# asarigun/mma

Hardware: AMD Instinct MI355X
Metric: aggregated edges/sec (fwd+bwd) MultiMaskConv (higher is better)
Workload: dtype f32

## Files before the change

include/mma_amd.h:

```cpp
#ifndef MMA_AMD_H
#define MMA_AMD_H

#include <stdint.h>

#ifdef __cplusplus
extern "C" {
#endif

#define MMA_ABI_VERSION 36
#define MMA_MAX_K 8

enum {
  MMA_KIND_SUM = 0,
  MMA_KIND_MEAN = 1,
  MMA_KIND_MAX = 2,
  MMA_KIND_MIN = 3,
  MMA_KIND_SOFTMAX = 4,
  MMA_KIND_SOFTMIN = 5
};
enum { MMA_ACT_SIGMOID = 0, MMA_ACT_RAW = 1 };

enum { MMA_DROP_NONE = 0, MMA_DROP_HASH = 1, MMA_DROP_EXPLICIT = 2 };

int mma_abi_version(void);
const char* mma_last_error(void);
const char* mma_build_stamp(void);

int mma_nc_fused_fwd(
    const float* x, int64_t ldx,
    const float* P, int64_t ldp,
    const float* Q, int64_t ldq,
    const int32_t* rowptr,
    const int32_t* col,
    const int32_t* items, int64_t n_items,
    int64_t n_wave_items,
    const int32_t* hubs, int64_t n_hubs,
    float* partial, int64_t n_slots,
    float* m,
    float* m_sum, int64_t ldms,
    float* T, uint8_t* sel, int64_t ldt,
    float* crow, int64_t ldc,
    int64_t N, int64_t E, int32_t H, int32_t K,
    const uint8_t* kind_host, const uint8_t* act_host,
    int32_t drop_mode, uint32_t drop_thr, uint64_t seed,
    const uint64_t* seed_dev,
    int64_t drop_edge_base,
    const uint8_t* keep,
    int32_t* sync,
    void* stream);

int mma_nc_bwd_node(
    const float* g, int64_t g_kstride, int64_t ldgr,
    const uint8_t* sel, const float* T, int64_t ldt, const int32_t* rowptr,
    float* gs, int64_t ldgs,
    const float* crow, int64_t ldc,
    float* gP, int64_t ldgp, float* gxs, int64_t ldgx,
    float* row_max,
    int64_t N, int32_t H, int32_t K, const uint8_t* kind_host, void* stream);
int64_t mma_nc_crow_floats(int32_t H, int32_t K, const uint8_t* kind_host);

int mma_nc_fused_bwd(
    const float* x, int64_t ldx, const float* P, int64_t ldp, const float* Q, int64_t ldq,
    const float* gs, int64_t ldg,
    const float* g, int64_t ldgg,
    const float* crow, int64_t ldc,
    const uint8_t* kind_host,
    const float* gxs, int64_t ldgx,
    const float* T, int64_t ldt,
    float* gP, int64_t ldgp, int64_t n_targets,
    const int32_t* t_col, const int32_t* t_eid,
    const int32_t* items, int64_t n_items, int64_t n_wave_items, const int32_t* hubs, int64_t n_hubs,
    float* partial, int64_t n_slots,
    float* gQ, int64_t ldgq, float* gx, int64_t ldgxo,
    float* row_max,
    int64_t N, int64_t E, int32_t H, int32_t K,
    const uint8_t* act_host,
    int32_t drop_mode, uint32_t drop_thr, uint64_t seed, const uint64_t* seed_dev, int64_t drop_edge_base, const uint8_t* keep,
    int32_t* sync,
    void* stream);

int mma_csr_spmm(
    const int32_t* rowptr, const int32_t* col, const float* val,
    const float* B, int64_t ldb, int64_t rows_per_block, int32_t K,
    const float* bias, float* out, int64_t ldo,
    int64_t n_rows, int32_t C, void* stream);
int mma_csr_spmm_rm(
    const int32_t* rowptr, const int32_t* col, const float* val,
    const float* B, int64_t ldb, int64_t rows_per_block, int32_t K,
    const float* bias, float* out, int64_t ldo,
    int64_t n_rows, int32_t C, float* row_max, void* stream);

int mma_csr_spmm_items(
    const int32_t* col, const float* val, const float* B, int64_t ldb, const float* bias, float* out, int64_t ldo,
    const int32_t* items, int64_t n_items,
    int64_t n_wave_items,
    const int32_t* hubs, int64_t n_hubs, float* partial, int64_t n_slots,
    int32_t C, void* stream);

int mma_split_bf16x3(const float* in, int64_t n, void* out_3n_bf16, void* stream);
int mma_gemm_bf16x3(const float* A, int64_t lda, const void* Bt3, float* C, int64_t ldc,
                    int64_t M, int32_t N, int32_t K, int32_t accumulate , void* stream);
int mma_row_absmax(const float* A, int64_t lda, int64_t M, int32_t cols, float* out, void* stream);
int mma_split_f16x2(const float* w, int64_t stride_k, int64_t stride_n, int32_t K, int32_t N, void* bt2, float* col_unscale,
                    int32_t plain_lo, void* stream);
int mma_gemm_f16x2(const float* A, int64_t lda, const void* Bt2, const float* col_unscale, float* C, int64_t ldc,
                   float* a_row_max,
                   int64_t M, int32_t N, void* stream);
int mma_gemm_f16x2_k(const float* A, int64_t lda, const void* Bt2, const float* col_unscale, float* C, int64_t ldc,
                     float* a_row_max, int64_t M, int32_t N, int32_t K, void* stream);
int mma_gemm_f16x2_k256(const float* A, int64_t lda, const float* row_max, const void* Bt2, const float* col_unscale, float* C,
                        int64_t ldc, int64_t M, int32_t N, void* stream);
int64_t mma_pack_f16x2_k256_bytes(int64_t M);
int mma_pack_f16x2_k256(const float* A, int64_t lda, int64_t M, void* Ap, int32_t* sce, float* row_max, void* stream);
int mma_gemm_f16x2_k256p(const void* Ap, const int32_t* sce, const void* Bt2, const float* col_unscale, float* C, int64_t ldc,
                         int64_t M, int32_t N, void* stream);
int mma_gemm_f16x2_n128(const float* A, int64_t lda, const float* row_max, const void* Bt2, const float* col_unscale,
                        float* C, int64_t ldc, int64_t M, int32_t K, int32_t accumulate, void* stream);
int mma_gemm_f16x2_nlp(const float* A, int64_t lda, const float* row_max, const void* Bt2, const float* col_unscale,
                       float* C, int64_t ldc, int64_t M, int32_t N, int32_t K, int32_t accumulate, void* stream);
int64_t mma_gemm_bf16x3_tn_workspace_floats(int64_t M, int32_t KA, int32_t NC);
int mma_gemm_bf16x3_tn(const float* X, int64_t ldx, const float* G, int64_t ldg, float* C, float* ws, int64_t ws_floats,
                       int64_t M, int32_t KA, int32_t NC, void* stream);
int64_t mma_gemm_bf16x3_tn_batched_workspace_floats(int64_t M, int32_t KA, int32_t NC, int32_t B);
int mma_gemm_bf16x3_tn_batched(const float* X, int64_t ldx, int64_t xb, const float* G, int64_t ldg, int64_t gb, float* C, float* ws,
                               int64_t ws_floats, int64_t M, int32_t KA, int32_t NC, int32_t B, void* stream);
int64_t mma_gemm_f16x2_tn_workspace_floats(int64_t M, int32_t KA, int32_t NC);
int mma_gemm_f16x2_tn(const float* X, int64_t ldx, const float* G, int64_t ldg, const float* x_row_max, const float* g_row_max,
                      float* C, float* ws, int64_t ws_floats, int64_t M, int32_t KA, int32_t NC, void* stream);

int mma_pack_rows(const float* src, int64_t lds, const int32_t* idx, int64_t n_idx,
                  float* dst, int64_t ldd, int32_t width, void* stream);
int mma_unpack_add_rows(const float* src, int64_t lds, const int32_t* idx, int64_t n_idx,
                        float* dst, int64_t ldd, int32_t width, void* stream);
int mma_unpack_add_rows_csr(const float* src, int64_t lds, const int32_t* rows, const int32_t* segptr, const int32_t* pos,
                            int64_t n_rows, float* dst, int64_t ldd, int32_t width, void* stream);

int64_t mma_col_sum_workspace_floats(int64_t R, int32_t C);
int mma_col_sum(const float* g, int64_t ldg, int64_t R, int32_t C, float* out, float* ws, int64_t ws_floats,
                void* stream);

int64_t mma_tower_linear_bwd_blocks(int64_t N);
int mma_tower_linear_bwd(const float* gy, const float* a, const float* W, float* ga, float* part, int64_t n_blocks,
                         int64_t N, int32_t T, int32_t O, int32_t C, void* stream);

int64_t mma_tower_post_kfp(int32_t KF);
int mma_tower_post_weights(const float* Wo, int32_t T, int32_t O, int32_t S, int32_t KF, float* Wa, float* Wb, void* stream);
int mma_skinny_linear_weights(const float* W, int32_t O, int32_t K, float* Wa, float* Wb, void* stream);
int mma_tower_post_gw_reduce(const float* part, int64_t n_chunks, int32_t T, int32_t S, int32_t O, int32_t KF, float* gWo, void* stream);
int mma_tower_post_fits(int32_t KF, int32_t S);
int mma_tower_post_pre(const int32_t* rowptr, float* pre, int64_t N, int32_t S, const uint8_t* scaler_host, float avg_log, float avg_lin,
                       void* stream);
int mma_tower_post_fwd(const float* agg, int64_t lda, const float* pre, const float* Wa, float* y, int64_t ldy,
                       int64_t N, int32_t T, int32_t KF, int32_t S, int32_t O, const uint8_t* scaler_host, float avg_log, float avg_lin,
                       void* stream);
int mma_tower_post_bwd(const float* gy, int64_t ldg, const float* pre, const float* Wb, float* gagg, int64_t lda,
                       float* gys, int64_t ldgs,
                       int64_t N, int32_t T, int32_t KF, int32_t S, int32_t O,
                       const uint8_t* scaler_host, float avg_log, float avg_lin, void* stream);
int64_t mma_tower_post_gw_chunks(int64_t N, int32_t T);
int mma_tower_post_gw(const float* gy, int64_t ldg, const float* agg, int64_t lda,
                      const float* pre,
                      float* part, int64_t n_chunks,
// ... 84 lines not shown
```

mma_amd/_abi.py:

```python
ABI_VERSION = 36
FUNCTIONS = {
    "mma_abi_version": ("int", []),
    "mma_last_error": ("const char*", []),
    "mma_build_stamp": ("const char*", []),
    "mma_nc_fused_fwd": ("int", [("T", "T", "x"), ("i", "i64", "ldx"), ("T", "T", "P"), ("i", "i64", "ldp"), ("T", "T", "Q"), ("i", "i64", "ldq"), ("T", "T", "rowptr"), ("T", "T", "col"), ("T", "T", "items"), ("i", "i64", "n_items"), ("i", "i64", "n_wave_items"), ("T", "T", "hubs"), ("i", "i64", "n_hubs"), ("T", "T", "partial"), ("i", "i64", "n_slots"), ("T", "T", "m"), ("T", "T", "m_sum"), ("i", "i64", "ldms"), ("T", "T", "T"), ("T", "T", "sel"), ("i", "i64", "ldt"), ("T", "T", "crow"), ("i", "i64", "ldc"), ("i", "i64", "N"), ("i", "i64", "E"), ("i", "i32", "H"), ("i", "i32", "K"), ("H", "H", "kind_host"), ("H", "H", "act_host"), ("i", "i32", "drop_mode"), ("i", "u32", "drop_thr"), ("i", "u64", "seed"), ("T", "T", "seed_dev"), ("i", "i64", "drop_edge_base"), ("T", "T", "keep"), ("T", "T", "sync"), ("S", "S", "stream")]),
    "mma_nc_bwd_node": ("int", [("T", "T", "g"), ("i", "i64", "g_kstride"), ("i", "i64", "ldgr"), ("T", "T", "sel"), ("T", "T", "T"), ("i", "i64", "ldt"), ("T", "T", "rowptr"), ("T", "T", "gs"), ("i", "i64", "ldgs"), ("T", "T", "crow"), ("i", "i64", "ldc"), ("T", "T", "gP"), ("i", "i64", "ldgp"), ("T", "T", "gxs"), ("i", "i64", "ldgx"), ("T", "T", "row_max"), ("i", "i64", "N"), ("i", "i32", "H"), ("i", "i32", "K"), ("H", "H", "kind_host"), ("S", "S", "stream")]),
    "mma_nc_crow_floats": ("int64_t", [("i", "i32", "H"), ("i", "i32", "K"), ("H", "H", "kind_host")]),
    "mma_nc_fused_bwd": ("int", [("T", "T", "x"), ("i", "i64", "ldx"), ("T", "T", "P"), ("i", "i64", "ldp"), ("T", "T", "Q"), ("i", "i64", "ldq"), ("T", "T", "gs"), ("i", "i64", "ldg"), ("T", "T", "g"), ("i", "i64", "ldgg"), ("T", "T", "crow"), ("i", "i64", "ldc"), ("H", "H", "kind_host"), ("T", "T", "gxs"), ("i", "i64", "ldgx"), ("T", "T", "T"), ("i", "i64", "ldt"), ("T", "T", "gP"), ("i", "i64", "ldgp"), ("i", "i64", "n_targets"), ("T", "T", "t_col"), ("T", "T", "t_eid"), ("T", "T", "items"), ("i", "i64", "n_items"), ("i", "i64", "n_wave_items"), ("T", "T", "hubs"), ("i", "i64", "n_hubs"), ("T", "T", "partial"), ("i", "i64", "n_slots"), ("T", "T", "gQ"), ("i", "i64", "ldgq"), ("T", "T", "gx"), ("i", "i64", "ldgxo"), ("T", "T", "row_max"), ("i", "i64", "N"), ("i", "i64", "E"), ("i", "i32", "H"), ("i", "i32", "K"), ("H", "H", "act_host"), ("i", "i32", "drop_mode"), ("i", "u32", "drop_thr"), ("i", "u64", "seed"), ("T", "T", "seed_dev"), ("i", "i64", "drop_edge_base"), ("T", "T", "keep"), ("T", "T", "sync"), ("S", "S", "stream")]),
    "mma_csr_spmm": ("int", [("T", "T", "rowptr"), ("T", "T", "col"), ("T", "T", "val"), ("T", "T", "B"), ("i", "i64", "ldb"), ("i", "i64", "rows_per_block"), ("i", "i32", "K"), ("T", "T", "bias"), ("T", "T", "out"), ("i", "i64", "ldo"), ("i", "i64", "n_rows"), ("i", "i32", "C"), ("S", "S", "stream")]),
    "mma_csr_spmm_rm": ("int", [("T", "T", "rowptr"), ("T", "T", "col"), ("T", "T", "val"), ("T", "T", "B"), ("i", "i64", "ldb"), ("i", "i64", "rows_per_block"), ("i", "i32", "K"), ("T", "T", "bias"), ("T", "T", "out"), ("i", "i64", "ldo"), ("i", "i64", "n_rows"), ("i", "i32", "C"), ("T", "T", "row_max"), ("S", "S", "stream")]),
    "mma_csr_spmm_items": ("int", [("T", "T", "col"), ("T", "T", "val"), ("T", "T", "B"), ("i", "i64", "ldb"), ("T", "T", "bias"), ("T", "T", "out"), ("i", "i64", "ldo"), ("T", "T", "items"), ("i", "i64", "n_items"), ("i", "i64", "n_wave_items"), ("T", "T", "hubs"), ("i", "i64", "n_hubs"), ("T", "T", "partial"), ("i", "i64", "n_slots"), ("i", "i32", "C"), ("S", "S", "stream")]),
    "mma_split_bf16x3": ("int", [("T", "T", "in"), ("i", "i64", "n"), ("T", "T", "out_3n_bf16"), ("S", "S", "stream")]),
    "mma_gemm_bf16x3": ("int", [("T", "T", "A"), ("i", "i64", "lda"), ("T", "T", "Bt3"), ("T", "T", "C"), ("i", "i64", "ldc"), ("i", "i64", "M"), ("i", "i32", "N"), ("i", "i32", "K"), ("i", "i32", "accumulate"), ("S", "S", "stream")]),
    "mma_row_absmax": ("int", [("T", "T", "A"), ("i", "i64", "lda"), ("i", "i64", "M"), ("i", "i32", "cols"), ("T", "T", "out"), ("S", "S", "stream")]),
    "mma_split_f16x2": ("int", [("T", "T", "w"), ("i", "i64", "stride_k"), ("i", "i64", "stride_n"), ("i", "i32", "K"), ("i", "i32", "N"), ("T", "T", "bt2"), ("T", "T", "col_unscale"), ("i", "i32", "plain_lo"), ("S", "S", "stream")]),
    "mma_gemm_f16x2": ("int", [("T", "T", "A"), ("i", "i64", "lda"), ("T", "T", "Bt2"), ("T", "T", "col_unscale"), ("T", "T", "C"), ("i", "i64", "ldc"), ("T", "T", "a_row_max"), ("i", "i64", "M"), ("i", "i32", "N"), ("S", "S", "stream")]),
    "mma_gemm_f16x2_k": ("int", [("T", "T", "A"), ("i", "i64", "lda"), ("T", "T", "Bt2"), ("T", "T", "col_unscale"), ("T", "T", "C"), ("i", "i64", "ldc"), ("T", "T", "a_row_max"), ("i", "i64", "M"), ("i", "i32", "N"), ("i", "i32", "K"), ("S", "S", "stream")]),
    "mma_gemm_f16x2_k256": ("int", [("T", "T", "A"), ("i", "i64", "lda"), ("T", "T", "row_max"), ("T", "T", "Bt2"), ("T", "T", "col_unscale"), ("T", "T", "C"), ("i", "i64", "ldc"), ("i", "i64", "M"), ("i", "i32", "N"), ("S", "S", "stream")]),
    "mma_pack_f16x2_k256_bytes": ("int64_t", [("i", "i64", "M")]),
    "mma_pack_f16x2_k256": ("int", [("T", "T", "A"), ("i", "i64", "lda"), ("i", "i64", "M"), ("T", "T", "Ap"), ("T", "T", "sce"), ("T", "T", "row_max"), ("S", "S", "stream")]),
    "mma_gemm_f16x2_k256p": ("int", [("T", "T", "Ap"), ("T", "T", "sce"), ("T", "T", "Bt2"), ("T", "T", "col_unscale"), ("T", "T", "C"), ("i", "i64", "ldc"), ("i", "i64", "M"), ("i", "i32", "N"), ("S", "S", "stream")]),
    "mma_gemm_f16x2_n128": ("int", [("T", "T", "A"), ("i", "i64", "lda"), ("T", "T", "row_max"), ("T", "T", "Bt2"), ("T", "T", "col_unscale"), ("T", "T", "C"), ("i", "i64", "ldc"), ("i", "i64", "M"), ("i", "i32", "K"), ("i", "i32", "accumulate"), ("S", "S", "stream")]),
    "mma_gemm_f16x2_nlp": ("int", [("T", "T", "A"), ("i", "i64", "lda"), ("T", "T", "row_max"), ("T", "T", "Bt2"), ("T", "T", "col_unscale"), ("T", "T", "C"), ("i", "i64", "ldc"), ("i", "i64", "M"), ("i", "i32", "N"), ("i", "i32", "K"), ("i", "i32", "accumulate"), ("S", "S", "stream")]),
    "mma_gemm_bf16x3_tn_workspace_floats": ("int64_t", [("i", "i64", "M"), ("i", "i32", "KA"), ("i", "i32", "NC")]),
    "mma_gemm_bf16x3_tn": ("int", [("T", "T", "X"), ("i", "i64", "ldx"), ("T", "T", "G"), ("i", "i64", "ldg"), ("T", "T", "C"), ("T", "T", "ws"), ("i", "i64", "ws_floats"), ("i", "i64", "M"), ("i", "i32", "KA"), ("i", "i32", "NC"), ("S", "S", "stream")]),
    "mma_gemm_bf16x3_tn_batched_workspace_floats": ("int64_t", [("i", "i64", "M"), ("i", "i32", "KA"), ("i", "i32", "NC"), ("i", "i32", "B")]),
    "mma_gemm_bf16x3_tn_batched": ("int", [("T", "T", "X"), ("i", "i64", "ldx"), ("i", "i64", "xb"), ("T", "T", "G"), ("i", "i64", "ldg"), ("i", "i64", "gb"), ("T", "T", "C"), ("T", "T", "ws"), ("i", "i64", "ws_floats"), ("i", "i64", "M"), ("i", "i32", "KA"), ("i", "i32", "NC"), ("i", "i32", "B"), ("S", "S", "stream")]),
    "mma_gemm_f16x2_tn_workspace_floats": ("int64_t", [("i", "i64", "M"), ("i", "i32", "KA"), ("i", "i32", "NC")]),
    "mma_gemm_f16x2_tn": ("int", [("T", "T", "X"), ("i", "i64", "ldx"), ("T", "T", "G"), ("i", "i64", "ldg"), ("T", "T", "x_row_max"), ("T", "T", "g_row_max"), ("T", "T", "C"), ("T", "T", "ws"), ("i", "i64", "ws_floats"), ("i", "i64", "M"), ("i", "i32", "KA"), ("i", "i32", "NC"), ("S", "S", "stream")]),
    "mma_pack_rows": ("int", [("T", "T", "src"), ("i", "i64", "lds"), ("T", "T", "idx"), ("i", "i64", "n_idx"), ("T", "T", "dst"), ("i", "i64", "ldd"), ("i", "i32", "width"), ("S", "S", "stream")]),
    "mma_unpack_add_rows": ("int", [("T", "T", "src"), ("i", "i64", "lds"), ("T", "T", "idx"), ("i", "i64", "n_idx"), ("T", "T", "dst"), ("i", "i64", "ldd"), ("i", "i32", "width"), ("S", "S", "stream")]),
    "mma_unpack_add_rows_csr": ("int", [("T", "T", "src"), ("i", "i64", "lds"), ("T", "T", "rows"), ("T", "T", "segptr"), ("T", "T", "pos"), ("i", "i64", "n_rows"), ("T", "T", "dst"), ("i", "i64", "ldd"), ("i", "i32", "width"), ("S", "S", "stream")]),
    "mma_col_sum_workspace_floats": ("int64_t", [("i", "i64", "R"), ("i", "i32", "C")]),
    "mma_col_sum": ("int", [("T", "T", "g"), ("i", "i64", "ldg"), ("i", "i64", "R"), ("i", "i32", "C"), ("T", "T", "out"), ("T", "T", "ws"), ("i", "i64", "ws_floats"), ("S", "S", "stream")]),
    "mma_tower_linear_bwd_blocks": ("int64_t", [("i", "i64", "N")]),
    "mma_tower_linear_bwd": ("int", [("T", "T", "gy"), ("T", "T", "a"), ("T", "T", "W"), ("T", "T", "ga"), ("T", "T", "part"), ("i", "i64", "n_blocks"), ("i", "i64", "N"), ("i", "i32", "T"), ("i", "i32", "O"), ("i", "i32", "C"), ("S", "S", "stream")]),
    "mma_tower_post_kfp": ("int64_t", [("i", "i32", "KF")]),
    "mma_tower_post_weights": ("int", [("T", "T", "Wo"), ("i", "i32", "T"), ("i", "i32", "O"), ("i", "i32", "S"), ("i", "i32", "KF"), ("T", "T", "Wa"), ("T", "T", "Wb"), ("S", "S", "stream")]),
    "mma_skinny_linear_weights": ("int", [("T", "T", "W"), ("i", "i32", "O"), ("i", "i32", "K"), ("T", "T", "Wa"), ("T", "T", "Wb"), ("S", "S", "stream")]),
    "mma_tower_post_gw_reduce": ("int", [("T", "T", "part"), ("i", "i64", "n_chunks"), ("i", "i32", "T"), ("i", "i32", "S"), ("i", "i32", "O"), ("i", "i32", "KF"), ("T", "T", "gWo"), ("S", "S", "stream")]),
    "mma_tower_post_fits": ("int", [("i", "i32", "KF"), ("i", "i32", "S")]),
    "mma_tower_post_pre": ("int", [("T", "T", "rowptr"), ("T", "T", "pre"), ("i", "i64", "N"), ("i", "i32", "S"), ("H", "H", "scaler_host"), ("f", "f32", "avg_log"), ("f", "f32", "avg_lin"), ("S", "S", "stream")]),
    "mma_tower_post_fwd": ("int", [("T", "T", "agg"), ("i", "i64", "lda"), ("T", "T", "pre"), ("T", "T", "Wa"), ("T", "T", "y"), ("i", "i64", "ldy"), ("i", "i64", "N"), ("i", "i32", "T"), ("i", "i32", "KF"), ("i", "i32", "S"), ("i", "i32", "O"), ("H", "H", "scaler_host"), ("f", "f32", "avg_log"), ("f", "f32", "avg_lin"), ("S", "S", "stream")]),
    "mma_tower_post_bwd": ("int", [("T", "T", "gy"), ("i", "i64", "ldg"), ("T", "T", "pre"), ("T", "T", "Wb"), ("T", "T", "gagg"), ("i", "i64", "lda"), ("T", "T", "gys"), ("i", "i64", "ldgs"), ("i", "i64", "N"), ("i", "i32", "T"), ("i", "i32", "KF"), ("i", "i32", "S"), ("i", "i32", "O"), ("H", "H", "scaler_host"), ("f", "f32", "avg_log"), ("f", "f32", "avg_lin"), ("S", "S", "stream")]),
    "mma_tower_post_gw_chunks": ("int64_t", [("i", "i64", "N"), ("i", "i32", "T")]),
    "mma_tower_post_gw": ("int", [("T", "T", "gy"), ("i", "i64", "ldg"), ("T", "T", "agg"), ("i", "i64", "lda"), ("T", "T", "pre"), ("T", "T", "part"), ("i", "i64", "n_chunks"), ("i", "i64", "N"), ("i", "i32", "T"), ("i", "i32", "KF"), ("i", "i32", "S"), ("i", "i32", "O"), ("H", "H", "scaler_host"), ("f", "f32", "avg_log"), ("f", "f32", "avg_lin"), ("S", "S", "stream")]),
    "mma_skinny_linear_fwd": ("int", [("T", "T", "x"), ("i", "i64", "ldx"), ("T", "T", "Wa"), ("T", "T", "bias"), ("T", "T", "addend"), ("i", "i64", "ldadd"), ("T", "T", "y"), ("i", "i64", "ldy"), ("i", "i64", "N"), ("i", "i32", "K"), ("i", "i32", "O"), ("S", "S", "stream")]),
    "mma_skinny_linear_bwd_dx": ("int", [("T", "T", "gy"), ("i", "i64", "ldg"), ("T", "T", "Wb"), ("T", "T", "gx"), ("i", "i64", "ldx"), ("i", "i64", "N"), ("i", "i32", "K"), ("i", "i32", "O"), ("S", "S", "stream")]),
    "mma_skinny_linear_gw_part": ("int64_t", [("i", "i64", "N"), ("i", "i32", "K"), ("i", "i32", "O")]),
    "mma_skinny_linear_gw": ("int", [("T", "T", "gy"), ("i", "i64", "ldg"), ("T", "T", "x"), ("i", "i64", "ldx"), ("T", "T", "part"), ("i", "i64", "n_part"), ("T", "T", "gw"), ("T", "T", "gb"), ("i", "i64", "N"), ("i", "i32", "K"), ("i", "i32", "O"), ("S", "S", "stream")]),
    "mma_logsoftmax_nll_fwd": ("int", [("T", "T", "x"), ("i", "i64", "ldx"), ("T", "T", "idx"), ("T", "T", "labels"), ("i", "i64", "n_idx"), ("T", "T", "logp"), ("i", "i64", "ldo"), ("T", "T", "loss"), ("i", "i64", "N"), ("i", "i32", "C"), ("S", "S", "stream")]),
    "mma_logsoftmax_nll_bwd": ("int", [("T", "T", "logp"), ("i", "i64", "ldo"), ("T", "T", "idx"), ("T", "T", "labels"), ("i", "i64", "n_idx"), ("T", "T", "gloss"), ("T", "T", "gx"), ("i", "i64", "ldg"), ("i", "i64", "N"), ("i", "i32", "C"), ("S", "S", "stream")]),
    "mma_masked_bn_relu_fwd": ("int", [("T", "T", "x"), ("i", "i64", "ldx"), ("T", "T", "n_valid"), ("T", "T", "gamma"), ("T", "T", "beta"), ("T", "T", "y"), ("i", "i64", "ldy"), ("T", "T", "mean_out"), ("T", "T", "rstd_out"), ("T", "T", "running_mean"), ("T", "T", "running_var"), ("T", "T", "n_tracked"), ("f", "f32", "momentum"), ("f", "f32", "eps"), ("i", "i64", "N"), ("i", "i32", "C"), ("i", "i32", "relu"), ("S", "S", "stream")]),
    "mma_masked_bn_relu_bwd": ("int", [("T", "T", "gy"), ("i", "i64", "ldg"), ("T", "T", "y"), ("i", "i64", "ldy"), ("T", "T", "x"), ("i", "i64", "ldx"), ("T", "T", "mean"), ("T", "T", "rstd"), ("T", "T", "gamma"), ("T", "T", "n_valid"), ("T", "T", "gx"), ("i", "i64", "ldgx"), ("T", "T", "ggamma"), ("T", "T", "gbeta"), ("i", "i64", "N"), ("i", "i32", "C"), ("i", "i32", "relu"), ("S", "S", "stream")]),
    "mma_pad_rows": ("int", [("T", "T", "x"), ("i", "i64", "ldx"), ("i", "i64", "M"), ("i", "i32", "fin"), ("T", "T", "col"), ("T", "T", "row_index"), ("T", "T", "out"), ("i", "i64", "ldo"), ("i", "i32", "width"), ("i", "i64", "M_out"), ("S", "S", "stream")]),
    "mma_pack_blocks": ("int", [("T", "T", "table"), ("i", "i64", "n_blocks"), ("T", "T", "a_base"), ("T", "T", "b0"), ("T", "T", "b1"), ("T", "T", "b2"), ("T", "T", "b3"), ("T", "T", "b4"), ("T", "T", "b5"), ("T", "T", "b6"), ("T", "T", "b7"), ("i", "i32", "unpack"), ("S", "S", "stream")]),
    "mma_edge_fold_fwd": ("int", [("T", "T", "We"), ("i", "i64", "ldw"), ("T", "T", "Wenc"), ("T", "T", "benc"), ("T", "T", "wz"), ("T", "T", "bz"), ("i", "i64", "TF"), ("i", "i32", "F"), ("i", "i32", "ED"), ("S", "S", "stream")]),
    "mma_edge_fold_bwd": ("int", [("T", "T", "We"), ("i", "i64", "ldw"), ("T", "T", "Wenc"), ("T", "T", "benc"), ("T", "T", "gwz"), ("T", "T", "gbz"), ("T", "T", "gWe"), ("T", "T", "gWenc"), ("T", "T", "gbenc"), ("i", "i64", "TF"), ("i", "i32", "F"), ("i", "i32", "ED"), ("S", "S", "stream")]),
    "mma_seed_advance": ("int", [("T", "T", "seeds"), ("i", "i32", "n"), ("S", "S", "stream")]),
    "mma_l1_loss_fwd": ("int", [("T", "T", "pred"), ("T", "T", "target"), ("i", "i64", "n"), ("T", "T", "loss"), ("S", "S", "stream")]),
    "mma_l1_loss_bwd": ("int", [("T", "T", "pred"), ("T", "T", "target"), ("i", "i64", "n"), ("T", "T", "gloss"), ("T", "T", "gpred"), ("S", "S", "stream")]),
    "mma_adam_table_bytes": ("int64_t", [("i", "i64", "n_tensors"), ("i", "i64", "total_chunks")]),
    "mma_adam_chunks": ("int64_t", [("i", "i64", "n_elements")]),
    "mma_adam_step": ("int", [("T", "T", "table"), ("i", "i64", "n_tensors"), ("i", "i64", "total_chunks"), ("T", "T", "step"), ("f", "f64", "lr"), ("f", "f64", "beta1"), ("f", "f64", "beta2"), ("f", "f32", "eps"), ("f", "f32", "weight_decay"), ("S", "S", "stream")]),
    "mma_adam_max_grads_by_value": ("int64_t", []),
    "mma_adam_step_grads": ("int", [("T", "T", "table"), ("i", "i64", "n_tensors"), ("i", "i64", "total_chunks"), ("T", "T", "step"), ("f", "f64", "lr"), ("f", "f64", "beta1"), ("f", "f64", "beta2"), ("f", "f32", "eps"), ("f", "f32", "weight_decay"), ("H", "H", "grad_ptrs_host"), ("S", "S", "stream")]),
    "mma_csr_workspace_bytes": ("int64_t", [("i", "i64", "E"), ("i", "i64", "N")]),
    "mma_gr_long_nodes_len": ("int64_t", [("i", "i64", "E")]),
    "mma_build_csr": ("int", [("T", "T", "key"), ("T", "T", "other"), ("i", "i64", "E"), ("i", "i64", "N"), ("T", "T", "rowptr"), ("T", "T", "perm"), ("T", "T", "other_sorted"), ("T", "T", "long_nodes"), ("T", "T", "workspace"), ("i", "i64", "workspace_bytes"), ("S", "S", "stream")]),
    "mma_gr_arg_side_rows": ("int64_t", [("i", "i64", "E")]),
    "mma_gr_fused_fwd": ("int", [("T", "T", "rowptr"), ("T", "T", "src"), ("T", "T", "perm"), ("T", "T", "U"), ("T", "T", "V"), ("i", "i64", "lduv"), ("T", "T", "Z"), ("i", "i64", "ldz"), ("i", "i32", "by_pos"), ("T", "T", "z_index"), ("T", "T", "inputs"), ("i", "i64", "ldi"), ("T", "T", "out"), ("T", "T", "amin8"), ("T", "T", "amax8"), ("T", "T", "amin_side"), ("T", "T", "amax_side"), ("T", "T", "mean"), ("T", "T", "var"), ("i", "i64", "ldsave"), ("T", "T", "long_nodes"), ("i", "i64", "N"), ("i", "i64", "E"), ("i", "i32", "T"), ("i", "i32", "F"), ("H", "H", "aggr_host"), ("i", "i32", "K"), ("H", "H", "scaler_host"), ("i", "i32", "S"), ("f", "f32", "avg_log"), ("f", "f32", "avg_lin"), ("i", "i32", "drop_mode"), ("i", "u32", "drop_thr"), ("i", "u64", "seed"), ("T", "T", "seed_dev"), ("S", "S", "stream")]),
    "mma_gr_fused_bwd": ("int", [("T", "T", "rowptr"), ("T", "T", "src"), ("T", "T", "perm"), ("T", "T", "U"), ("T", "T", "V"), ("i", "i64", "lduv"), ("T", "T", "Z"), ("i", "i64", "ldz"), ("i", "i32", "by_pos"), ("T", "T", "z_index"), ("T", "T", "inputs"), ("i", "i64", "ldi"), ("T", "T", "gout"), ("T", "T", "amin8"), ("T", "T", "amax8"), ("T", "T", "amin_side"), ("T", "T", "amax_side"), ("T", "T", "mean"), ("T", "T", "var"), ("i", "i64", "ldsave"), ("T", "T", "long_nodes"), ("T", "T", "gmsg"), ("i", "i64", "ldg"), ("T", "T", "gU"), ("i", "i64", "ldgu"), ("T", "T", "gmsg_row_max"), ("T", "T", "gu_row_max"), ("i", "i64", "N"), ("i", "i64", "E"), ("i", "i32", "T"), ("i", "i32", "F"), ("H", "H", "aggr_host"), ("i", "i32", "K"), ("H", "H", "scaler_host"), ("i", "i32", "S"), ("f", "f32", "avg_log"), ("f", "f32", "avg_lin"), ("i", "i32", "drop_mode"), ("i", "u32", "drop_thr"), ("i", "u64", "seed"), ("T", "T", "seed_dev"), ("S", "S", "stream")]),
}
```

mma_amd/csrc/nc_fused.hip:

```cpp
#include <cstdlib>
#include "common.h"

#ifndef NC_FWD_UNROLL
#define NC_FWD_UNROLL(K) ((K) >= 3 ? 1 : 2)
#endif
#ifndef NC_BWD_UNROLL
#define NC_BWD_UNROLL(K) ((K) >= 3 ? 1 : 2)
#endif
#ifndef MMA_MIN_WAVES
#define MMA_MIN_WAVES 2
#endif
namespace mma {

struct NcFwdParams {
  const float* x; int64_t ldx;
  const float* P; int64_t ldp; const float* Q; int64_t ldq;
  const int32_t* rowptr; const int32_t* col;
  const int4* items; int64_t n_items;
  float* partial; int64_t pstride;
  float* m; int64_t m_kstride;
  float* msum; int64_t ldms;
  float* T; uint8_t* sel; int64_t ldt;
  float* crow; int64_t ldc; uint32_t sel_slots;
  int H, HQ, K_total, k_base, lpr_log;
// ... 306 lines not shown
    default: fs = tf == 255u ? __builtin_nanf("") : 1.f; fx = 0.f; break;
  }
}

template <int VEC>
__global__ __launch_bounds__(kBlock) void nc_bwd_node_kernel(const NcBwdNodeParams p) {
  const int per_row = (p.H + VEC - 1) / VEC;
  const int64_t total = p.N * per_row;
  for (int64_t idx = (int64_t)blockIdx.x * blockDim.x + threadIdx.x; idx < total; idx += (int64_t)gridDim.x * blockDim.x) {
    const int64_t node = idx / per_row;
    const int c = (int)(idx % per_row) * VEC;
    const float deg = (float)max(p.rowptr[node + 1] - p.rowptr[node], 1);
    const float inv_deg = 1.f / deg;
    Vec<VEC> gk[MMA_MAX_K], tk[MMA_MAX_K];
    uint32_t ck[MMA_MAX_K];
    const bool shared_g = p.g_kstride == 0;
#pragma unroll
    for (int k = 0; k < MMA_MAX_K; ++k) {
      if (k < p.K) {
        const size_t o = (size_t)node * p.ldt + (size_t)k * p.H + c;
        if (k == 0 || !shared_g) gk[k] = ldv_nt<VEC>(p.g + (size_t)k * p.g_kstride + (size_t)node * p.ldgr + c);
        tk[k] = ldv_nt<VEC>(p.T + o);
        if (p.crow) {
          ck[k] = sel_slot_of(p.sel_slots, k) != 0xFu
              ? ldb<VEC>(reinterpret_cast<const uint8_t*>(p.crow + (size_t)node * p.ldc + 4 + (size_t)sel_slot_of(p.sel_slots, k) * p.HQ) + c) : 0u;
        } else {
          ck[k] = ldb_nt<VEC>(p.sel + o);
        }
      }
    }
    Vec<VEC> gx = vzero<VEC>();
    float mxp = 0.f;
#pragma unroll
    for (int k = 0; k < MMA_MAX_K; ++k) {
      if (k < p.K) {
        const int kind = kind_of(p.kinds, k);
        const Vec<VEC> g = shared_g ? gk[0] : gk[k];
        const Vec<VEC> t = tk[k];
        const uint32_t codes = ck[k];
        Vec<VEC> gsv, gpv;
#pragma unroll
        for (int i = 0; i < VEC; ++i) {
          uint32_t tf = (codes >> (8 * i)) & 0xFFu;
          if (!p.crow) tf = tf == 1u ? 2u : (tf == 2u ? 1u : (tf == 3u ? 255u : 0u));
          float fs, fx;
          combine_grad_tf(kind, tf, inv_deg, fs, fx);
          gsv.v[i] = g.v[i] * fs;
          gpv.v[i] = gsv.v[i] * t.v[i];
          gx.v[i] = fmaf(g.v[i], fx, gx.v[i]);
          mxp = fmaxf(mxp, fabsf(gpv.v[i]));
        }
        if (p.gs) stv<VEC>(p.gs + (size_t)node * p.ldgs + (size_t)k * p.H + c, gsv);
        stv_nt<VEC>(p.gP + (size_t)node * p.ldgp + (size_t)k * p.H + c, gpv);
      }
    }
    stv_nt<VEC>(p.gxs + (size_t)node * p.ldgx + c, gx);
    if (p.rowmax) {
      if ((per_row & (per_row - 1)) == 0 && per_row <= kWave) {
        for (int off = per_row >> 1; off > 0; off >>= 1) mxp = fmaxf(mxp, __shfl_xor(mxp, off, kWave));
        if ((idx & (per_row - 1)) == 0 && mxp > 0.f) atomicMax(p.rowmax + node, __float_as_uint(mxp));
      } else if (mxp > 0.f) {
        atomicMax(p.rowmax + node, __float_as_uint(mxp));
      }
    }
  }
}

struct NcBwdParams {
  const float* x; int64_t ldx;
  const float* P; int64_t ldp; const float* Q; int64_t ldq;
  const float* gs; int64_t ldg; const float* gxs; int64_t ldgx;
  const float* g; int64_t ldgg; const float* crow; int64_t ldc; uint32_t sel_slots; uint32_t kinds;
  const float* T; int64_t ldt; float* gP; int64_t ldgp; int64_t n_targets;
  const int32_t* t_col; const int32_t* t_eid;
  const int4* items; int64_t n_items;
  float* partial; int64_t pstride;
  float* gQ; int64_t ldgq; float* gx; int64_t ldgxo;
  int H, HQ, K_total, k_base, lpr_log;
  uint32_t acts;
  DropParams drop;
  int first_pass;
  uint32_t* rowmax;
  const int4* hubs; int64_t n_hubs; unsigned* sync; unsigned n_slots;
};

template <int VEC>
__device__ __forceinline__ Vec<VEC> nc_bwd_epilogue(const NcBwdParams& p, int node, int c, int k0, int nk, float& mx) {
  const Vec<VEC> g = ldv_nt<VEC>(p.g + row_off(node, p.ldgg) + c);
  const float* crow = p.crow + row_off(node, p.ldc);
  const float inv_deg = crow[0];
  Vec<VEC> gxd = vzero<VEC>();
  Vec<VEC> tk[MMA_MAX_K]; uint32_t ck[MMA_MAX_K];
#pragma unroll
  for (int k = 0; k < MMA_MAX_K; ++k) {
    if (k < nk) {
      tk[k] = ldv_nt<VEC>(p.T + row_off(node, p.ldt) + (size_t)(k0 + k) * p.H + c);
      const uint32_t sslot = sel_slot_of(p.sel_slots, k0 + k);
      ck[k] = sslot != 0xFu ? ldb<VEC>(reinterpret_cast<const uint8_t*>(crow + 4 + (size_t)sslot * p.HQ) + c) : 0u;
    }
  }
#pragma unroll
  for (int k = 0; k < MMA_MAX_K; ++k) {
    if (k < nk) {
      const int kind = kind_of(p.kinds, k0 + k);
      Vec<VEC> gpv;
#pragma unroll
      for (int i = 0; i < VEC; ++i) {
        float fs, fx;
        combine_grad_tf(kind, (ck[k] >> (8 * i)) & 0xFFu, inv_deg, fs, fx);
        gpv.v[i] = (g.v[i] * fs) * tk[k].v[i];
        gxd.v[i] = fmaf(g.v[i], fx, gxd.v[i]);
        mx = fmaxf(mx, fabsf(gpv.v[i]));
      }
      stv_nt<VEC>(p.gP + row_off(node, p.ldgp) + (size_t)(k0 + k) * p.H + c, gpv);
    }
  }
  return gxd;
}

template <int VEC>
__device__ __forceinline__ void nc_bwd_finalize_body(const NcBwdParams& p, const int4* hubs, int64_t n_hubs, const int64_t first, const int64_t step);

template <int K, int VEC, int DM, bool SHARED, bool MULTI, bool EPI, bool ONE = false>
__device__ __forceinline__ void nc_bwd_body(const NcBwdParams& p, const int bx, const int nbx) {
  constexpr bool DROP = DM != MMA_DROP_NONE;
  const DropParams dp = (DM == MMA_DROP_HASH || DM == MMA_DROP_HASH16) ? drop_resolve(p.drop) : p.drop;
  uint32_t mult[K], mult2[K];
#pragma unroll
  for (int k = 0; k < K; ++k) { mult[k] = drop_mask_mult(p.k_base + k); mult2[k] = drop_mask_mult2(p.k_base + k); }
  constexpr int U = NC_BWD_UNROLL(K);
  const int lane = threadIdx.x & (kWave - 1);
  const int lpr = 1 << p.lpr_log;
  const int G = MULTI ? lpr : kWave;
  const int epg = G >> p.lpr_log;
  const int gpw = kWave / G;
  const int grp = MULTI ? lane / G : 0;
  const int gl = lane & (G - 1);
  const int gbase = grp * G;
  const int sub = gl >> p.lpr_log;
  const int c = ((int)blockIdx.y * lpr + (lane & (lpr - 1))) * VEC;
  const bool fvalid = c < p.H;
  const int cc = fvalid ? c : 0;
  const int waves_per_block = kBlock / kWave;
  const int64_t stride = (int64_t)nbx * waves_per_block;
  const int64_t n_witems = (p.n_items + gpw - 1) / gpw;

  for (int64_t it0 = (int64_t)bx * waves_per_block + (threadIdx.x >> 6); it0 < n_witems; it0 += stride) {
    int node, ebeg, eend, slot;
    bool ivalid = true;
    if (MULTI) {
      const int64_t idx = it0 * gpw + grp;
      ivalid = idx < p.n_items;
      const int4 item = p.items[ivalid ? idx : 0];
      node = item.x; ebeg = item.y; eend = ivalid ? item.z : item.y; slot = item.w;
    } else {
      const int4 item = p.items[__builtin_amdgcn_readfirstlane((int)it0)];
      node = __builtin_amdgcn_readfirstlane(item.x);
      ebeg = __builtin_amdgcn_readfirstlane(item.y);
      eend = __builtin_amdgcn_readfirstlane(item.z);
      slot = __builtin_amdgcn_readfirstlane(item.w);
    }
    const int len = eend - ebeg;
    int maxlen = len;
    if (MULTI) {
      for (int off = G; off < kWave; off <<= 1) maxlen = max(maxlen, __shfl_xor(maxlen, off, kWave));
      maxlen = __builtin_amdgcn_readfirstlane(maxlen);
    }

    const Vec<VEC> xj = ldv_nt<VEC>(p.x + row_off(node, p.ldx) + cc);
    Vec<VEC> qk[K], aq[K];
    Vec<VEC> ax = vzero<VEC>();
#pragma unroll
    for (int k = 0; k < K; ++k) {
      qk[k] = ldv_nt<VEC>(p.Q + row_off(node, p.ldq) + (size_t)(p.k_base + k) * p.H + cc);
      aq[k] = vzero<VEC>();
    }

    for (int base = 0; base < maxlen; base += G) {
      const int cnt = min(G, max(len - base, 0));
      const int ucnt = min(G, maxlen - base);
      const int myi = (gl < cnt) ? p.t_col[ebeg + base + gl] : ((gl == 0 && len > 0) ? p.t_col[ebeg] : 0);
      const int mye = (DROP && gl < cnt) ? p.t_eid[ebeg + base + gl] : 0;
      for (int t0 = 0; t0 < ucnt; t0 += U * epg) {
        int tt[U]; bool ev[U]; uint32_t eid[U]; Vec<VEC> gv[U][SHARED ? 1 : K]; Vec<VEC> pv[U][K];
        uint32_t codes[U][K]; float idg[U];
#pragma unroll
        for (int u = 0; u < U; ++u) {
          tt[u] = t0 + u * epg + sub;
          ev[u] = tt[u] < cnt;
          const int tl = min(tt[u], max(cnt - 1, 0));
          const int ii = __shfl(myi, gbase + (tl & (G - 1)), kWave);
          eid[u] = DROP ? (uint32_t)__shfl(mye, gbase + (tl & (G - 1)), kWave) : 0u;
          if (SHARED) {
            gv[u][0] = ldv<VEC>(p.g + row_off(ii, p.ldgg) + cc);
            const float* crow = p.crow + row_off(ii, p.ldc);
            idg[u] = crow[0];
#pragma unroll
            for (int k = 0; k < K; ++k) {
              const uint32_t sslot = sel_slot_of(p.sel_slots, p.k_base + k);
              codes[u][k] = (sslot != 0xFu) ? ldb<VEC>(reinterpret_cast<const uint8_t*>(crow + 4 + (size_t)sslot * p.HQ) + cc)
                                             : 0x02020202u;
            }
          }
          const float* prow = p.P + row_off(ii, p.ldp) + cc;
          const float* grow = SHARED ? nullptr : p.gs + row_off(ii, p.ldg) + cc;
#pragma unroll
          for (int k = 0; k < K; ++k) {
            const size_t o = (size_t)(p.k_base + k) * p.H;
            if (!SHARED) gv[u][k] = ldv<VEC>(grow + o);
            pv[u][k] = ldv<VEC>(prow + o);
          }
        }
#pragma unroll
        for (int u = 0; u < U; ++u) {
          const bool live = ev[u];
#pragma unroll
          for (int kk = 0; kk < (SHARED ? 1 : K); ++kk)
#pragma unroll
            for (int i = 0; i < VEC; ++i) gv[u][kk].v[i] = live ? gv[u][kk].v[i] : 0.f;
          const uint32_t hw = (DM == MMA_DROP_HASH || DM == MMA_DROP_HASH16) ? drop_base_word(dp, eid[u], cc >> 2) : 0u;
#pragma unroll
          for (int k = 0; k < K; ++k) {
            const bool raw = (p.acts >> (p.k_base + k)) & 1u;
            const int kind = SHARED ? kind_of(p.kinds, p.k_base + k) : 0;
            const float kscale = 0.5f * (kind == MMA_KIND_MEAN ? idg[u] : 1.f);
            float f[VEC];
            if (DM == MMA_DROP_HASH) {
              drop_unpack<VEC>(dp, drop_mask_word(hw, k == 0 ? p.k_base : 1, mult[k]), cc, f);
            } else if (DM == MMA_DROP_HASH16) {
              drop_unpack16<VEC>(dp, drop_mask_word(hw, k == 0 ? p.k_base : 1, mult[k]), drop_low_word(hw, mult2[k]), cc, f);
            } else if (DM == MMA_DROP_EXPLICIT) {
              drop_explicit<VEC>(dp, eid[u], p.k_base + k, cc, p.H, f);
            } else {
#pragma unroll
              for (int i = 0; i < VEC; ++i) f[i] = 1.f;
            }
#pragma unroll
            for (int i = 0; i < VEC; ++i) {
              const float z = pv[u][k].v[i] + qk[k].v[i];
              float a, da;
              if (raw) { a = z; da = 1.f; }
              else { a = sigmoid_fast(z); da = a - a * a; }
              float gsv;
              if (SHARED) {
                const uint32_t tf = (codes[u][k] >> (8 * i)) & 0xFFu;
                float cf = (float)tf;
                if (kind >= MMA_KIND_SOFTMAX && tf == 255u) cf = __builtin_nanf("");
                gsv = gv[u][0].v[i] * (cf * kscale);
              } else {
                gsv = gv[u][k].v[i];
              }
              const float w = f[i] * gsv;
              aq[k].v[i] = fmaf(da, w, aq[k].v[i]);
              ax.v[i] = fmaf(a, w, ax.v[i]);
            }
          }
        }
      }
    }

    const bool writer = sub == 0 && fvalid && ivalid;
    const bool tgt = EPI && writer && slot < 0 && (int64_t)node < p.n_targets;
    Vec<VEC> gxd = vzero<VEC>();
    float mxp = 0.f;
    if (EPI) { if (tgt) gxd = nc_bwd_epilogue<VEC>(p, node, c, p.k_base, K, mxp); }

    for (int off = G / 2; off >= lpr; off >>= 1) {
#pragma unroll
      for (int i = 0; i < VEC; ++i) {
        ax.v[i] += __shfl_xor(ax.v[i], off, kWave);
#pragma unroll
        for (int k = 0; k < K; ++k) aq[k].v[i] += __shfl_xor(aq[k].v[i], off, kWave);
      }
    }
    if (len == 0) {
      ax = vzero<VEC>();
#pragma unroll
      for (int k = 0; k < K; ++k) aq[k] = vzero<VEC>();
    }

    if (p.rowmax) {
      float mxq = mxp;
      if (writer && slot < 0) {
#pragma unroll
        for (int k = 0; k < K; ++k)
#pragma unroll
          for (int i = 0; i < VEC; ++i) mxq = fmaxf(mxq, fabsf(xj.v[i] * aq[k].v[i]));
      }
      for (int off = lpr >> 1; off > 0; off >>= 1) mxq = fmaxf(mxq, __shfl_xor(mxq, off, kWave));
      if (sub == 0 && (lane & (lpr - 1)) == 0 && ivalid && slot < 0 && mxq > 0.f) atomicMax(p.rowmax + node, __float_as_uint(mxq));
    }
    if (writer) {
      if (slot < 0) {
#pragma unroll
        for (int k = 0; k < K; ++k) {
          Vec<VEC> o;
#pragma unroll
          for (int i = 0; i < VEC; ++i) o.v[i] = xj.v[i] * aq[k].v[i];
          stv_nt<VEC>(p.gQ + row_off(node, p.ldgq) + (size_t)(p.k_base + k) * p.H + c, o);
        }
        Vec<VEC> g0;
        if (EPI) {
          g0 = gxd;
          if (!p.first_pass) {
            const Vec<VEC> prev = ldv<VEC>(p.gx + row_off(node, p.ldgxo) + c);
#pragma unroll
            for (int i = 0; i < VEC; ++i) g0.v[i] += prev.v[i];
          }
        } else {
          g0 = p.first_pass ? ldv_nt<VEC>(p.gxs + row_off(node, p.ldgx) + c) : ldv<VEC>(p.gx + row_off(node, p.ldgxo) + c);
        }
        Vec<VEC> o;
#pragma unroll
        for (int i = 0; i < VEC; ++i) o.v[i] = g0.v[i] + ax.v[i];
        stv_nt<VEC>(p.gx + row_off(node, p.ldgxo) + c, o);
      } else {
        float* ps = p.partial + (size_t)slot * p.pstride;
#pragma unroll
        for (int k = 0; k < K; ++k) stv<VEC>(ps + (size_t)(p.k_base + k) * p.H + c, aq[k]);
        float* px = ps + (size_t)p.K_total * p.H + c;
        if (p.first_pass) stv<VEC>(px, ax);
        else {
          const Vec<VEC> prev = ldv<VEC>(px);
          Vec<VEC> o;
#pragma unroll
          for (int i = 0; i < VEC; ++i) o.v[i] = prev.v[i] + ax.v[i];
          stv<VEC>(px, o);
        }
      }
    }
    if (ONE) {
      const bool wrote = ivalid && slot >= 0;
      if (__builtin_amdgcn_ballot_w64(wrote) != 0) {
        __builtin_amdgcn_fence(__ATOMIC_RELEASE, "agent");
        unsigned ticket = 0u;
        if (wrote && gl == 0) ticket = atomicAdd(p.sync, 1u) + 1u;
        if (__builtin_amdgcn_ballot_w64(ticket == p.n_slots) != 0) {
          __builtin_amdgcn_fence(__ATOMIC_ACQUIRE, "agent");
          nc_bwd_finalize_body<VEC>(p, p.hubs, p.n_hubs, lane, kWave);
          if (lane == 0) *p.sync = 0u;
        }
      }
    }
  }
}

template <int K, int VEC, int DM, bool SHARED, bool MULTI, bool EPI>
__global__ __launch_bounds__(kBlock, (K <= 4 ? MMA_MIN_WAVES : 1)) void nc_bwd_kernel(const NcBwdParams p) {
  nc_bwd_body<K, VEC, DM, SHARED, MULTI, EPI>(p, (int)blockIdx.x, (int)gridDim.x);
}

template <int VEC>
__device__ __forceinline__ void nc_bwd_finalize_body(const NcBwdParams& p, const int4* hubs, int64_t n_hubs, const int64_t first, const int64_t step) {
  const int per_row = (p.H + VEC - 1) / VEC;
  const bool epi = p.T != nullptr;
  const int64_t total = n_hubs * (p.K_total + 1) * per_row;
  for (int64_t idx = first; idx < total; idx += step) {
    const int c = (int)(idx % per_row) * VEC;
    const int k = (int)((idx / per_row) % (p.K_total + 1));
    const int4 hub = hubs[idx / ((int64_t)per_row * (p.K_total + 1))];
    Vec<VEC> s = vzero<VEC>();
    constexpr int kAhead = 8;
    for (int sl0 = hub.y; sl0 < hub.z; sl0 += kAhead) {
      Vec<VEC> a[kAhead];
#pragma unroll
      for (int u = 0; u < kAhead; ++u) a[u] = ldv<VEC>(p.partial + (size_t)min(sl0 + u, hub.z - 1) * p.pstride + (size_t)k * p.H + c);
#pragma unroll
      for (int u = 0; u < kAhead; ++u) {
        if (sl0 + u < hub.z) {
#pragma unroll
          for (int i = 0; i < VEC; ++i) s.v[i] += a[u].v[i];
        }
      }
    }
    const int node = hub.x;
    const bool tgt = epi && (int64_t)node < p.n_targets;
    Vec<VEC> o;
    if (k < p.K_total) {
      const Vec<VEC> xj = ldv<VEC>(p.x + (size_t)node * p.ldx + c);
      float mxq = 0.f;
      if (tgt) nc_bwd_epilogue<VEC>(p, node, c, k, 1, mxq);
#pragma unroll
      for (int i = 0; i < VEC; ++i) o.v[i] = xj.v[i] * s.v[i];
      stv_nt<VEC>(p.gQ + (size_t)node * p.ldgq + (size_t)k * p.H + c, o);
      if (p.rowmax) {
#pragma unroll
        for (int i = 0; i < VEC; ++i) mxq = fmaxf(mxq, fabsf(o.v[i]));
        if (mxq > 0.f) atomicMax(p.rowmax + node, __float_as_uint(mxq));
      }
    } else {
      Vec<VEC> g0 = vzero<VEC>();
      if (tgt) {
        const Vec<VEC> g = ldv<VEC>(p.g + row_off(node, p.ldgg) + c);
        const float* crow = p.crow + row_off(node, p.ldc);
        const float inv_deg = crow[0];
        for (int kk = 0; kk < p.K_total; ++kk) {
          const uint32_t sslot = sel_slot_of(p.sel_slots, kk);
          const uint32_t ck = sslot != 0xFu ? ldb<VEC>(reinterpret_cast<const uint8_t*>(crow + 4 + (size_t)sslot * p.HQ) + c) : 0u;
#pragma unroll
          for (int i = 0; i < VEC; ++i) {
            float fs, fx;
            combine_grad_tf(kind_of(p.kinds, kk), (ck >> (8 * i)) & 0xFFu, inv_deg, fs, fx);
            g0.v[i] = fmaf(g.v[i], fx, g0.v[i]);
          }
        }
      } else if (!epi) {
        g0 = ldv<VEC>(p.gxs + (size_t)node * p.ldgx + c);
      }
#pragma unroll
      for (int i = 0; i < VEC; ++i) o.v[i] = g0.v[i] + s.v[i];
      stv<VEC>(p.gx + (size_t)node * p.ldgxo + c, o);
    }
  }
}
template <int VEC>
__global__ __launch_bounds__(kBlock) void nc_bwd_finalize_kernel(const NcBwdParams p, const int4* hubs, int64_t n_hubs) {
  nc_bwd_finalize_body<VEC>(p, hubs, n_hubs, (int64_t)blockIdx.x * blockDim.x + threadIdx.x, (int64_t)gridDim.x * blockDim.x);
}

template <int K, int VEC, int DM, bool EPI>
__global__ __launch_bounds__(kBlock, (K <= 4 ? MMA_MIN_WAVES : 1)) void nc_bwd_small_kernel(const NcBwdParams p, const NcSmallPlan sp) {
  if ((int)blockIdx.x < sp.blocks_a) {
    NcBwdParams q = p;
    q.n_items = sp.n_wave_items;
    nc_bwd_body<K, VEC, DM, true, false, EPI, true>(q, (int)blockIdx.x, sp.blocks_a);
  } else {
    NcBwdParams q = p;
    q.items = p.items + sp.n_wave_items; q.n_items = p.n_items - sp.n_wave_items;
    nc_bwd_body<K, VEC, DM, true, true, EPI, true>(q, (int)blockIdx.x - sp.blocks_a, (int)gridDim.x - sp.blocks_a);
  }
}

static bool aligned16(const void* p) { return (reinterpret_cast<uintptr_t>(p) & 15u) == 0; }

static int pack_codes(const uint8_t* kind_host, const uint8_t* act_host, int K, uint32_t* kinds, uint32_t* acts) {
  *kinds = 0; *acts = 0;
  for (int k = 0; k < K; ++k) {
    if (kind_host) {
      if (kind_host[k] > MMA_KIND_SOFTMIN) return fail(1, "kind[%d]=%d is not an MMA_KIND_* code", k, (int)kind_host[k]);
      *kinds |= (uint32_t)kind_host[k] << (4 * k);
    }
    if (act_host) {
      if (act_host[k] > MMA_ACT_RAW) return fail(1, "act[%d]=%d is not an MMA_ACT_* code", k, (int)act_host[k]);
      *acts |= (uint32_t)act_host[k] << k;
    }
  }
  return 0;
}

static int64_t fill_sel_slots(const uint8_t* kind_host, int K, int H, uint32_t* slots) {
  int n = 0;
  *slots = 0xFFFFFFFFu;
  for (int k = 0; k < K; ++k)
    if (kind_host[k] >= MMA_KIND_MAX) { *slots = (*slots & ~(0xFu << (4 * k))) | ((uint32_t)n << (4 * k)); ++n; }
  return ((4 + (int64_t)n * (((int64_t)H + 3) / 4)) + 3) & ~(int64_t)3;
}

static int make_drop(int32_t mode, uint32_t thr, uint64_t seed, const uint64_t* seed_dev, int64_t edge_base, const uint8_t* keep,
                     int64_t E, DropParams* d) {
  d->seed_dev = seed_dev;
  MMA_REQUIRE(edge_base >= 0 && edge_base + E < (1LL << 32), "drop_edge_base %lld out of range", (long long)edge_base);
  d->edge_base = (uint32_t)edge_base;
  MMA_REQUIRE(mode >= MMA_DROP_NONE && mode <= MMA_DROP_EXPLICIT, "drop_mode %d unknown", mode);
  MMA_REQUIRE(mode == MMA_DROP_NONE || thr < 65536, "drop_thr %u out of range (0..65535: P(drop) = thr / 65536)", thr);
  MMA_REQUIRE(mode != MMA_DROP_EXPLICIT || keep != nullptr, "drop_mode EXPLICIT needs a keep mask");
  drop_set_threshold(d, mode, thr);
  d->seed_lo = (uint32_t)seed; d->seed_hi = (uint32_t)(seed >> 32); d->keep = keep; d->E = E;
  return 0;
}

struct Geometry { int vec, lpr_log, chunks; };
static Geometry geometry(int H, bool vec4_ok) {
  Geometry g;
  g.vec = vec4_ok ? 4 : 1;
  const int per_row = (H + g.vec - 1) / g.vec;
  g.lpr_log = min(ilog2_ceil(per_row), 6);
  g.chunks = (per_row + (1 << g.lpr_log) - 1) >> g.lpr_log;
  return g;
}

static dim3 item_grid(int64_t n_items, int chunks, int items_per_wave = 1) {
  const int64_t per_block = (int64_t)(kBlock / kWave) * items_per_wave;
  int64_t blocks = (n_items + per_block - 1) / per_block;
  if (blocks > kMaxGrid) blocks = kMaxGrid;
  if (blocks < 1) blocks = 1;
  return dim3((unsigned)blocks, (unsigned)chunks, 1);
}

template <int K, int VEC, bool MULTI>
static void launch_fwd(const NcFwdParams& p, dim3 grid, bool save, int dm, hipStream_t st) {
#define MMA_FWD(SAVE, DM) hipLaunchKernelGGL((nc_fwd_kernel<K, VEC, SAVE, DM, MULTI>), grid, dim3(kBlock), 0, st, p)
  if (save) {
    if (dm == MMA_DROP_HASH) MMA_FWD(true, MMA_DROP_HASH); else if (dm == MMA_DROP_HASH16) MMA_FWD(true, MMA_DROP_HASH16); else if (dm == MMA_DROP_EXPLICIT) MMA_FWD(true, MMA_DROP_EXPLICIT); else MMA_FWD(true, MMA_DROP_NONE);
  } else {
    if (dm == MMA_DROP_HASH) MMA_FWD(false, MMA_DROP_HASH); else if (dm == MMA_DROP_HASH16) MMA_FWD(false, MMA_DROP_HASH16); else if (dm == MMA_DROP_EXPLICIT) MMA_FWD(false, MMA_DROP_EXPLICIT); else MMA_FWD(false, MMA_DROP_NONE);
  }
#undef MMA_FWD
}
template <int VEC, bool MULTI>
static void launch_fwd_k(int Ks, const NcFwdParams& p, dim3 grid, bool save, int dm, hipStream_t st) {
  switch (Ks) {
    case 1: launch_fwd<1, VEC, MULTI>(p, grid, save, dm, st); break;
    case 2: launch_fwd<2, VEC, MULTI>(p, grid, save, dm, st); break;
    case 3: launch_fwd<3, VEC, MULTI>(p, grid, save, dm, st); break;
    case 4: launch_fwd<4, VEC, MULTI>(p, grid, save, dm, st); break;
    default: launch_fwd<8, VEC, MULTI>(p, grid, save, dm, st); break;
  }
}
template <int K, int VEC, bool MULTI>
static void launch_bwd(const NcBwdParams& p, dim3 grid, int dm, hipStream_t st) {
  const bool shared = p.gs == nullptr;
  const bool epi = p.T != nullptr;
#define MMA_BWD(DM, SHARED, EPI) hipLaunchKernelGGL((nc_bwd_kernel<K, VEC, DM, SHARED, MULTI, EPI>), grid, dim3(kBlock), 0, st, p)
#define MMA_BWD_DM(SHARED, EPI) \
  do { if (dm == MMA_DROP_HASH) MMA_BWD(MMA_DROP_HASH, SHARED, EPI); else if (dm == MMA_DROP_HASH16) MMA_BWD(MMA_DROP_HASH16, SHARED, EPI); else if (dm == MMA_DROP_EXPLICIT) MMA_BWD(MMA_DROP_EXPLICIT, SHARED, EPI); \
       else MMA_BWD(MMA_DROP_NONE, SHARED, EPI); } while (0)
  if (shared) { if (epi) MMA_BWD_DM(true, true); else MMA_BWD_DM(true, false); }
  else MMA_BWD_DM(false, false);
#undef MMA_BWD_DM
#undef MMA_BWD
}
template <int VEC, bool MULTI>
static void launch_bwd_k(int Ks, const NcBwdParams& p, dim3 grid, int dm, hipStream_t st) {
  switch (Ks) {
    case 1: launch_bwd<1, VEC, MULTI>(p, grid, dm, st); break;
    case 2: launch_bwd<2, VEC, MULTI>(p, grid, dm, st); break;
    case 3: launch_bwd<3, VEC, MULTI>(p, grid, dm, st); break;
    case 4: launch_bwd<4, VEC, MULTI>(p, grid, dm, st); break;
    default: launch_bwd<8, VEC, MULTI>(p, grid, dm, st); break;
  }
}

template <int K>
static void launch_fwd_small(const NcFwdParams& p, const NcSmallPlan& sp, dim3 grid, bool save, int dm, hipStream_t st) {
#define MMA_FWD_S(SAVE, DM) hipLaunchKernelGGL((nc_fwd_small_kernel<K, 4, SAVE, DM>), grid, dim3(kBlock), 0, st, p, sp)
  if (save) { if (dm == MMA_DROP_HASH) MMA_FWD_S(true, MMA_DROP_HASH); else if (dm == MMA_DROP_HASH16) MMA_FWD_S(true, MMA_DROP_HASH16); else MMA_FWD_S(true, MMA_DROP_NONE); }
  else { if (dm == MMA_DROP_HASH) MMA_FWD_S(false, MMA_DROP_HASH); else if (dm == MMA_DROP_HASH16) MMA_FWD_S(false, MMA_DROP_HASH16); else MMA_FWD_S(false, MMA_DROP_NONE); }
#undef MMA_FWD_S
}
template <int K>
static void launch_bwd_small(const NcBwdParams& p, const NcSmallPlan& sp, dim3 grid, int dm, hipStream_t st) {
  const bool epi = p.T != nullptr;
#define MMA_BWD_S(DM, EPI) hipLaunchKernelGGL((nc_bwd_small_kernel<K, 4, DM, EPI>), grid, dim3(kBlock), 0, st, p, sp)
  if (epi) { if (dm == MMA_DROP_HASH) MMA_BWD_S(MMA_DROP_HASH, true); else if (dm == MMA_DROP_HASH16) MMA_BWD_S(MMA_DROP_HASH16, true); else MMA_BWD_S(MMA_DROP_NONE, true); }
  else { if (dm == MMA_DROP_HASH) MMA_BWD_S(MMA_DROP_HASH, false); else if (dm == MMA_DROP_HASH16) MMA_BWD_S(MMA_DROP_HASH16, false); else MMA_BWD_S(MMA_DROP_NONE, false); }
#undef MMA_BWD_S
}
static bool small_plan(int32_t* sync, int K, const Geometry& g, int dm, int64_t n_items, int64_t n_wave_items, int64_t n_hubs, int64_t n_slots,
                       int64_t finalize_elems, NcSmallPlan* sp, dim3* grid) {
  const bool one_slice = K <= 4 || K == 8;
  if (!sync || !one_slice || g.vec != 4 || g.chunks != 1 || dm == MMA_DROP_EXPLICIT || finalize_elems > 4096 || n_slots >= (1LL << 31)) return false;
  const int64_t n_group = n_items - n_wave_items;
  if (n_hubs == 0 && (n_wave_items == 0 || n_group == 0)) return false;
  const int ipw = kWave >> g.lpr_log;
  const unsigned ba = n_wave_items > 0 ? item_grid(n_wave_items, 1, 1).x : 0u;
  const unsigned bb = n_group > 0 ? item_grid(n_group, 1, ipw).x : 0u;
  *sp = NcSmallPlan{n_wave_items, (int)ba};
  *grid = dim3(ba + bb, 1, 1);
  return true;
}

static int next_slice(int remaining) { return remaining >= 8 ? 8 : (remaining >= 4 ? 4 : remaining); }

static int64_t elementwise_grid(int64_t total) {
  int64_t b = (total + kBlock - 1) / kBlock;
  return b < 1 ? 1 : (b > kMaxGrid * 4 ? kMaxGrid * 4 : b);
}

}

using namespace mma;

extern "C" int mma_nc_fused_fwd(
    const float* x, int64_t ldx, const float* P, int64_t ldp, const float* Q, int64_t ldq,
    const int32_t* rowptr, const int32_t* col,
    const int32_t* items, int64_t n_items, int64_t n_wave_items, const int32_t* hubs, int64_t n_hubs,
    float* partial, int64_t n_slots, float* m, float* m_sum, int64_t ldms, float* T, uint8_t* sel, int64_t ldt,
    float* crow, int64_t ldc,
    int64_t N, int64_t E, int32_t H, int32_t K, const uint8_t* kind_host, const uint8_t* act_host,
    int32_t drop_mode, uint32_t drop_thr, uint64_t seed, const uint64_t* seed_dev, int64_t drop_edge_base, const uint8_t* keep,
    int32_t* sync, void* stream) {
  MMA_REQUIRE(N >= 0 && E >= 0 && N < (1LL << 31) && E < (1LL << 31), "N=%lld E=%lld out of int32 range", (long long)N, (long long)E);
  MMA_REQUIRE(H >= 1 && K >= 1 && K <= MMA_MAX_K, "H=%d K=%d unsupported (1<=K<=%d)", H, K, MMA_MAX_K);
  MMA_REQUIRE(ldx >= H && ldp >= (int64_t)K * H && ldq >= (int64_t)K * H, "row pitch too small: ldx=%lld ldp=%lld ldq=%lld",
              (long long)ldx, (long long)ldp, (long long)ldq);
  MMA_REQUIRE(T != nullptr || (sel == nullptr && crow == nullptr), "sel / crow are saved next to T: give T too");
  MMA_REQUIRE(T == nullptr || sel != nullptr || crow != nullptr, "T needs the selection state beside it: sel (N,K*H), crow (N,ldc), or both");
  MMA_REQUIRE(T == nullptr || ldt >= (int64_t)K * H, "ldt=%lld too small", (long long)ldt);
  MMA_REQUIRE(ldx < (1LL << 31) && ldp < (1LL << 31) && ldq < (1LL << 31) && ldt < (1LL << 31) && ldc < (1LL << 31), "row pitch out of range");
  MMA_REQUIRE(n_items >= 0 && n_hubs >= 0 && n_slots >= 0 && n_items < (1LL << 31) && n_wave_items >= 0, "negative or oversize item counts");
  MMA_REQUIRE(n_slots == 0 || (partial != nullptr && hubs != nullptr && n_hubs > 0), "hub slots without partial/hubs buffers");
  if (N == 0 || n_items == 0) return 0;
  MMA_REQUIRE(x && P && Q && rowptr && items && kind_host && act_host, "NULL argument");
  MMA_REQUIRE(m != nullptr || m_sum != nullptr, "give m (K,N,H), m_sum (N,H), or both");
  MMA_REQUIRE(m_sum == nullptr || ldms >= H, "ldms=%lld too small", (long long)ldms);
  MMA_REQUIRE(E == 0 || col != nullptr, "NULL col");
  MMA_REQUIRE(aligned16(items) && (hubs == nullptr || aligned16(hubs)), "items/hubs must be 16-byte aligned int32 quadruples");
  uint32_t kinds, acts;
  if (int rc = pack_codes(kind_host, act_host, K, &kinds, &acts)) return rc;
  NcFwdParams p{};
  if (int rc = make_drop(drop_mode, drop_thr, seed, seed_dev, drop_edge_base, keep, E, &p.drop)) return rc;
  const int dm = (drop_mode == MMA_DROP_HASH && drop_thr == 0) ? MMA_DROP_NONE : p.drop.mode;
  const bool save = T != nullptr;
  if (crow) {
    const int64_t crow_len = fill_sel_slots(kind_host, K, H, &p.sel_slots);
    MMA_REQUIRE(ldc >= crow_len && ldc % 4 == 0 && aligned16(crow), "crow needs a 16-byte aligned pitch >= %lld floats (mma_nc_crow_floats)",
                (long long)crow_len);
  }
  const bool v4 = (H % 4 == 0) && (ldx % 4 == 0) && (ldp % 4 == 0) && (ldq % 4 == 0) && (!save || ldt % 4 == 0) && aligned16(x) &&
                  aligned16(P) && aligned16(Q) && (!m || aligned16(m)) && (!m_sum || (aligned16(m_sum) && ldms % 4 == 0)) &&
                  (!save || (aligned16(T) && (!sel || aligned16(sel)))) && (partial == nullptr || aligned16(partial));
  const Geometry g = geometry(H, v4);
  p.x = x; p.ldx = ldx; p.P = P; p.ldp = ldp; p.Q = Q; p.ldq = ldq; p.rowptr = rowptr; p.col = col;
  static const bool ablate_p = getenv("MMA_NC_ABLATE_P") && atoi(getenv("MMA_NC_ABLATE_P")) != 0;
  if (ablate_p) p.ldp = 0;
  p.items = reinterpret_cast<const int4*>(items); p.n_items = n_items;
  p.partial = partial; p.pstride = 2LL * K * H;
  p.m = m; p.m_kstride = N * (int64_t)H; p.msum = m_sum; p.ldms = ldms; p.T = T; p.sel = sel; p.ldt = ldt;
  p.crow = crow; p.ldc = ldc;
  p.H = H; p.HQ = (H + 3) / 4; p.K_total = K; p.lpr_log = g.lpr_log; p.kinds = kinds; p.acts = acts;
  hipStream_t st = static_cast<hipStream_t>(stream);
  const int ipw = kWave >> g.lpr_log;
  if (ipw == 1 || n_wave_items > n_items) n_wave_items = n_items;
  const int4* all_items = p.items;
  {
    NcSmallPlan sp; dim3 sgrid;
    if (small_plan(sync, K, g, dm, n_items, n_wave_items, n_hubs, n_slots, n_hubs * ((H + 3) / 4), &sp, &sgrid)) {
      p.k_base = 0;
      p.hubs = reinterpret_cast<const int4*>(hubs); p.n_hubs = n_hubs; p.sync = reinterpret_cast<unsigned*>(sync); p.n_slots = (unsigned)n_slots;
      switch (K) {
        case 1: launch_fwd_small<1>(p, sp, sgrid, save, dm, st); break;
        case 2: launch_fwd_small<2>(p, sp, sgrid, save, dm, st); break;
        case 3: launch_fwd_small<3>(p, sp, sgrid, save, dm, st); break;
        case 4: launch_fwd_small<4>(p, sp, sgrid, save, dm, st); break;
        default: launch_fwd_small<8>(p, sp, sgrid, save, dm, st); break;
      }
      return check_launch("nc_fwd_small_kernel");
    }
  }
  for (int part = 0; part < 2; ++part) {
    const int64_t cnt = part == 0 ? n_wave_items : n_items - n_wave_items;
    if (cnt <= 0) continue;
    p.items = all_items + (part == 0 ? 0 : n_wave_items);
    p.n_items = cnt;
    const dim3 grid = item_grid(cnt, g.chunks, part == 0 ? 1 : ipw);
    for (int k0 = 0; k0 < K;) {
      const int ks = next_slice(K - k0);
      p.k_base = k0;
      if (g.vec == 4) { if (part == 0) launch_fwd_k<4, false>(ks, p, grid, save, dm, st); else launch_fwd_k<4, true>(ks, p, grid, save, dm, st); }
      else { if (part == 0) launch_fwd_k<1, false>(ks, p, grid, save, dm, st); else launch_fwd_k<1, true>(ks, p, grid, save, dm, st); }
      k0 += ks;
    }
  }
  if (int rc = check_launch("nc_fwd_kernel")) return rc;
  if (n_hubs > 0) {
    const int per_row = (H + g.vec - 1) / g.vec;
    const dim3 fg((unsigned)elementwise_grid(n_hubs * per_row));
    const int4* hb = reinterpret_cast<const int4*>(hubs);
    if (g.vec == 4) {
      if (save) hipLaunchKernelGGL((nc_fwd_finalize_kernel<4, true>), fg, dim3(kBlock), 0, st, p, hb, n_hubs);
      else hipLaunchKernelGGL((nc_fwd_finalize_kernel<4, false>), fg, dim3(kBlock), 0, st, p, hb, n_hubs);
    } else {
      if (save) hipLaunchKernelGGL((nc_fwd_finalize_kernel<1, true>), fg, dim3(kBlock), 0, st, p, hb, n_hubs);
      else hipLaunchKernelGGL((nc_fwd_finalize_kernel<1, false>), fg, dim3(kBlock), 0, st, p, hb, n_hubs);
    }
    if (int rc = check_launch("nc_fwd_finalize_kernel")) return rc;
  }
  return 0;
}

extern "C" int64_t mma_nc_crow_floats(int32_t H, int32_t K, const uint8_t* kind_host) {
  if (H < 1 || K < 1 || K > MMA_MAX_K || !kind_host) return -1;
  for (int k = 0; k < K; ++k) if (kind_host[k] > MMA_KIND_SOFTMIN) return -1;
  uint32_t slots;
  return fill_sel_slots(kind_host, K, H, &slots);
}

extern "C" int mma_nc_bwd_node(
    const float* g, int64_t g_kstride, int64_t ldgr, const uint8_t* sel, const float* T, int64_t ldt, const int32_t* rowptr,
    float* gs, int64_t ldgs, const float* crow, int64_t ldc, float* gP, int64_t ldgp, float* gxs, int64_t ldgx, float* row_max,
    int64_t N, int32_t H, int32_t K, const uint8_t* kind_host, void* stream) {
  MMA_REQUIRE(N >= 0 && N < (1LL << 31) && H >= 1 && K >= 1 && K <= MMA_MAX_K, "N=%lld H=%d K=%d unsupported", (long long)N, H, K);
  MMA_REQUIRE(ldt >= (int64_t)K * H && (!gs || ldgs >= (int64_t)K * H) && ldgp >= (int64_t)K * H && ldgx >= H && ldgr >= H &&
              g_kstride >= 0, "row pitch too small");
  if (N == 0) return 0;
  MMA_REQUIRE(g && (sel || crow) && T && rowptr && gP && gxs && kind_host, "NULL argument (the selection state is sel or crow)");
  uint32_t kinds, acts;
  if (int rc = pack_codes(kind_host, nullptr, K, &kinds, &acts)) return rc;
  NcBwdNodeParams p{g, g_kstride, ldgr, sel, T, ldt, rowptr, gs, ldgs, gP, ldgp, gxs, ldgx, N, H, K, kinds};
  p.rowmax = reinterpret_cast<uint32_t*>(row_max);
  p.crow = crow; p.ldc = ldc; p.HQ = (H + 3) / 4;
  const int64_t crow_len = fill_sel_slots(kind_host, K, H, &p.sel_slots);
  MMA_REQUIRE(!crow || (ldc >= crow_len && ldc % 4 == 0 && aligned16(crow)),
              "crow needs a 16-byte aligned pitch >= %lld floats (mma_nc_crow_floats)", (long long)crow_len);
  const bool v4 = (H % 4 == 0) && (ldt % 4 == 0) && (!gs || ldgs % 4 == 0) && (ldgp % 4 == 0) && (ldgx % 4 == 0) &&
                  (ldgr % 4 == 0) && (g_kstride % 4 == 0) && aligned16(g) && (crow || aligned16(sel)) &&
                  aligned16(T) && (!gs || aligned16(gs)) && aligned16(gP) && aligned16(gxs);
  hipStream_t st = static_cast<hipStream_t>(stream);
  const int per_row = v4 ? H / 4 : H;
  int64_t nblk = (N * per_row + kBlock - 1) / kBlock;
  if (nblk > (1LL << 30)) nblk = 1LL << 30;
  const dim3 grid((unsigned)nblk);
  if (v4) hipLaunchKernelGGL((nc_bwd_node_kernel<4>), grid, dim3(kBlock), 0, st, p);
  else hipLaunchKernelGGL((nc_bwd_node_kernel<1>), grid, dim3(kBlock), 0, st, p);
  return check_launch("nc_bwd_node_kernel");
}

extern "C" int mma_nc_fused_bwd(
    const float* x, int64_t ldx, const float* P, int64_t ldp, const float* Q, int64_t ldq,
    const float* gs, int64_t ldg, const float* g, int64_t ldgg, const float* crow, int64_t ldc, const uint8_t* kind_host,
    const float* gxs, int64_t ldgx, const float* T, int64_t ldt, float* gP, int64_t ldgp, int64_t n_targets,
    const int32_t* t_col, const int32_t* t_eid,
    const int32_t* items, int64_t n_items, int64_t n_wave_items, const int32_t* hubs, int64_t n_hubs,
    float* partial, int64_t n_slots, float* gQ, int64_t ldgq, float* gx, int64_t ldgxo, float* row_max,
    int64_t N, int64_t E, int32_t H, int32_t K, const uint8_t* act_host,
    int32_t drop_mode, uint32_t drop_thr, uint64_t seed, const uint64_t* seed_dev, int64_t drop_edge_base, const uint8_t* keep,
    int32_t* sync, void* stream) {
  MMA_REQUIRE(N >= 0 && E >= 0 && N < (1LL << 31) && E < (1LL << 31), "N=%lld E=%lld out of int32 range", (long long)N, (long long)E);
  MMA_REQUIRE(H >= 1 && K >= 1 && K <= MMA_MAX_K, "H=%d K=%d unsupported (1<=K<=%d)", H, K, MMA_MAX_K);
  MMA_REQUIRE(ldx >= H && ldp >= (int64_t)K * H && ldq >= (int64_t)K * H && (!gs || ldg >= (int64_t)K * H) && ldgq >= (int64_t)K * H &&
              ldgxo >= H, "row pitch too small");
  MMA_REQUIRE(ldx < (1LL << 31) && ldp < (1LL << 31) && ldq < (1LL << 31) && ldg < (1LL << 31) && ldgg < (1LL << 31) && ldc < (1LL << 31) &&
              ldt < (1LL << 31) && ldgp < (1LL << 31) && ldgq < (1LL << 31) && ldgx < (1LL << 31) && ldgxo < (1LL << 31), "row pitch out of range");
  MMA_REQUIRE(n_items >= 0 && n_hubs >= 0 && n_slots >= 0 && n_items < (1LL << 31) && n_wave_items >= 0, "negative or oversize item counts");
  MMA_REQUIRE(n_slots == 0 || (partial != nullptr && hubs != nullptr && n_hubs > 0), "hub slots without partial/hubs buffers");
  if (N == 0 || n_items == 0) return 0;
  const bool shared = gs == nullptr;
  const bool epi = T != nullptr;
  MMA_REQUIRE(!shared || (g && crow && kind_host && ldgg >= H),
              "give gs (n_targets,K*H), or the shared-gradient form: g (n_targets,H), the code rows crow K1 wrote, and kinds");
  MMA_REQUIRE(!epi || (shared && gP && ldt >= (int64_t)K * H && ldgp >= (int64_t)K * H && n_targets >= 0 && n_targets <= N),
              "the fused node-level epilogue (T given) needs the shared-gradient form, gP and 0 <= n_targets <= N");
  MMA_REQUIRE(epi || (gxs && ldgx >= H), "gxs (N,H) from mma_nc_bwd_node is needed unless the epilogue is fused (T given)");
  MMA_REQUIRE(x && P && Q && items && gQ && gx && act_host, "NULL argument");
  MMA_REQUIRE(E == 0 || (t_col != nullptr && t_eid != nullptr), "NULL transposed CSR");
  MMA_REQUIRE(aligned16(items) && (hubs == nullptr || aligned16(hubs)), "items/hubs must be 16-byte aligned int32 quadruples");
  uint32_t kinds, acts;
  if (int rc = pack_codes(shared ? kind_host : nullptr, act_host, K, &kinds, &acts)) return rc;
  NcBwdParams p{};
  if (int rc = make_drop(drop_mode, drop_thr, seed, seed_dev, drop_edge_base, keep, E, &p.drop)) return rc;
  const int dm = (drop_mode == MMA_DROP_HASH && drop_thr == 0) ? MMA_DROP_NONE : p.drop.mode;
  const bool v4 = (H % 4 == 0) && (ldx % 4 == 0) && (ldp % 4 == 0) && (ldq % 4 == 0) && (epi || (ldgx % 4 == 0 && aligned16(gxs))) && (ldgq % 4 == 0) &&
                  (shared ? (ldgg % 4 == 0 && aligned16(g) && ldc % 4 == 0 && aligned16(crow)) : (ldg % 4 == 0 && aligned16(gs))) &&
                  (!epi || (ldt % 4 == 0 && aligned16(T) && ldgp % 4 == 0 && aligned16(gP))) &&
                  (ldgxo % 4 == 0) && aligned16(x) && aligned16(P) && aligned16(Q) &&
                  aligned16(gQ) && aligned16(gx) && (partial == nullptr || aligned16(partial));
  const Geometry geo = geometry(H, v4);
  p.x = x; p.ldx = ldx; p.P = P; p.ldp = ldp; p.Q = Q; p.ldq = ldq; p.gs = gs; p.ldg = ldg; p.gxs = gxs; p.ldgx = ldgx;
  p.g = g; p.ldgg = ldgg; p.crow = crow; p.ldc = ldc; p.kinds = kinds;
  p.T = T; p.ldt = ldt; p.gP = gP; p.ldgp = ldgp; p.n_targets = n_targets;
  if (shared) {
    const int64_t crow_len = fill_sel_slots(kind_host, K, H, &p.sel_slots);
    MMA_REQUIRE(ldc >= crow_len, "ldc=%lld < %lld", (long long)ldc, (long long)crow_len);
  }
  p.t_col = t_col; p.t_eid = t_eid; p.items = reinterpret_cast<const int4*>(items); p.n_items = n_items;
  p.partial = partial; p.pstride = (int64_t)(K + 1) * H; p.gQ = gQ; p.ldgq = ldgq; p.gx = gx; p.ldgxo = ldgxo;
  p.rowmax = reinterpret_cast<uint32_t*>(row_max);
  p.H = H; p.HQ = (H + 3) / 4; p.K_total = K; p.lpr_log = geo.lpr_log; p.acts = acts;
  hipStream_t st = static_cast<hipStream_t>(stream);
  const int ipw = kWave >> geo.lpr_log;
  if (ipw == 1 || n_wave_items > n_items) n_wave_items = n_items;
  const int4* all_items = p.items;
  {
    NcSmallPlan sp; dim3 sgrid;
    if (shared && small_plan(sync, K, geo, dm, n_items, n_wave_items, n_hubs, n_slots, n_hubs * (K + 1) * ((H + 3) / 4), &sp, &sgrid)) {
      p.k_base = 0; p.first_pass = 1;
      p.hubs = reinterpret_cast<const int4*>(hubs); p.n_hubs = n_hubs; p.sync = reinterpret_cast<unsigned*>(sync); p.n_slots = (unsigned)n_slots;
      switch (K) {
        case 1: launch_bwd_small<1>(p, sp, sgrid, dm, st); break;
        case 2: launch_bwd_small<2>(p, sp, sgrid, dm, st); break;
        case 3: launch_bwd_small<3>(p, sp, sgrid, dm, st); break;
        case 4: launch_bwd_small<4>(p, sp, sgrid, dm, st); break;
        default: launch_bwd_small<8>(p, sp, sgrid, dm, st); break;
      }
      return check_launch("nc_bwd_small_kernel");
    }
  }
  for (int part = 0; part < 2; ++part) {
    const int64_t cnt = part == 0 ? n_wave_items : n_items - n_wave_items;
    if (cnt <= 0) continue;
    p.items = all_items + (part == 0 ? 0 : n_wave_items);
    p.n_items = cnt;
    const dim3 grid = item_grid(cnt, geo.chunks, part == 0 ? 1 : ipw);
    for (int k0 = 0; k0 < K;) {
      const int ks = next_slice(K - k0);
      p.k_base = k0; p.first_pass = (k0 == 0);
      if (geo.vec == 4) { if (part == 0) launch_bwd_k<4, false>(ks, p, grid, dm, st); else launch_bwd_k<4, true>(ks, p, grid, dm, st); }
      else { if (part == 0) launch_bwd_k<1, false>(ks, p, grid, dm, st); else launch_bwd_k<1, true>(ks, p, grid, dm, st); }
      k0 += ks;
    }
  }
  if (int rc = check_launch("nc_bwd_kernel")) return rc;
  if (n_hubs > 0) {
    const int per_row = (H + geo.vec - 1) / geo.vec;
    const dim3 fg((unsigned)elementwise_grid(n_hubs * (K + 1) * per_row));
    const int4* hb = reinterpret_cast<const int4*>(hubs);
    if (geo.vec == 4) hipLaunchKernelGGL((nc_bwd_finalize_kernel<4>), fg, dim3(kBlock), 0, st, p, hb, n_hubs);
    else hipLaunchKernelGGL((nc_bwd_finalize_kernel<1>), fg, dim3(kBlock), 0, st, p, hb, n_hubs);
    if (int rc = check_launch("nc_bwd_finalize_kernel")) return rc;
  }
  return 0;
}
```

mma_amd/csrc/torch_ops.cpp:

```cpp
#include <torch/library.h>
#include <ATen/ATen.h>
#include <c10/hip/HIPStream.h>
#include <array>
#include <optional>
#include "../../include/mma_amd.h"

namespace {
using OptT = std::optional<at::Tensor>;
template <typename T> T* dptr(const OptT& t) { return t.has_value() && t->defined() ? static_cast<T*>(t->data_ptr()) : nullptr; }
struct Codes { std::array<uint8_t, 1024> v{}; bool has = false; };
Codes codes(const std::optional<at::IntArrayRef>& a, int64_t expected, const char* what) {
  Codes c;
  if (a.has_value()) {
    TORCH_CHECK(a->size() <= c.v.size(), "mma_amd: ", what, " is too long");
    TORCH_CHECK(expected < 0 || static_cast<int64_t>(a->size()) == expected, "mma_amd: ", what, " has ", a->size(),
                " entries, the call says ", expected);
    for (size_t i = 0; i < a->size(); ++i) c.v[i] = static_cast<uint8_t>((*a)[i]);
    c.has = true;
  }
  return c;
}
void check(int rc, const char* name) { TORCH_CHECK(rc == 0, name, " failed (code ", rc, "): ", mma_last_error()); }
void* stream() { return c10::hip::device_count() > 0 ? static_cast<void*>(c10::hip::getCurrentHIPStream().stream()) : nullptr; }

void op_mma_nc_fused_fwd(const OptT& x, int64_t ldx, const OptT& P, int64_t ldp, const OptT& Q, int64_t ldq, const OptT& rowptr, const OptT& col, const OptT& items, int64_t n_items, int64_t n_wave_items, const OptT& hubs, int64_t n_hubs, const OptT& partial, int64_t n_slots, const OptT& m, const OptT& m_sum, int64_t ldms, const OptT& T, const OptT& sel, int64_t ldt, const OptT& crow, int64_t ldc, int64_t N, int64_t E, int64_t H, int64_t K, std::optional<at::IntArrayRef> kind_host, std::optional<at::IntArrayRef> act_host, int64_t drop_mode, int64_t drop_thr, int64_t seed, const OptT& seed_dev, int64_t drop_edge_base, const OptT& keep, const OptT& sync) {
  const Codes c_kind_host = codes(kind_host, static_cast<int64_t>(K), "kind_host");
  const Codes c_act_host = codes(act_host, static_cast<int64_t>(K), "act_host");
  check(mma_nc_fused_fwd(dptr<float>(x), static_cast<int64_t>(ldx), dptr<float>(P), static_cast<int64_t>(ldp), dptr<float>(Q), static_cast<int64_t>(ldq), dptr<int32_t>(rowptr), dptr<int32_t>(col), dptr<int32_t>(items), static_cast<int64_t>(n_items), static_cast<int64_t>(n_wave_items), dptr<int32_t>(hubs), static_cast<int64_t>(n_hubs), dptr<float>(partial), static_cast<int64_t>(n_slots), dptr<float>(m), dptr<float>(m_sum), static_cast<int64_t>(ldms), dptr<float>(T), dptr<uint8_t>(sel), static_cast<int64_t>(ldt), dptr<float>(crow), static_cast<int64_t>(ldc), static_cast<int64_t>(N), static_cast<int64_t>(E), static_cast<int32_t>(H), static_cast<int32_t>(K), (c_kind_host.has ? c_kind_host.v.data() : nullptr), (c_act_host.has ? c_act_host.v.data() : nullptr), static_cast<int32_t>(drop_mode), static_cast<uint32_t>(drop_thr), static_cast<uint64_t>(seed), dptr<uint64_t>(seed_dev), static_cast<int64_t>(drop_edge_base), dptr<uint8_t>(keep), dptr<int32_t>(sync), stream()), "mma_nc_fused_fwd");
}

void op_mma_nc_bwd_node(const OptT& g, int64_t g_kstride, int64_t ldgr, const OptT& sel, const OptT& T, int64_t ldt, const OptT& rowptr, const OptT& gs, int64_t ldgs, const OptT& crow, int64_t ldc, const OptT& gP, int64_t ldgp, const OptT& gxs, int64_t ldgx, const OptT& row_max, int64_t N, int64_t H, int64_t K, std::optional<at::IntArrayRef> kind_host) {
  const Codes c_kind_host = codes(kind_host, static_cast<int64_t>(K), "kind_host");
  check(mma_nc_bwd_node(dptr<float>(g), static_cast<int64_t>(g_kstride), static_cast<int64_t>(ldgr), dptr<uint8_t>(sel), dptr<float>(T), static_cast<int64_t>(ldt), dptr<int32_t>(rowptr), dptr<float>(gs), static_cast<int64_t>(ldgs), dptr<float>(crow), static_cast<int64_t>(ldc), dptr<float>(gP), static_cast<int64_t>(ldgp), dptr<float>(gxs), static_cast<int64_t>(ldgx), dptr<float>(row_max), static_cast<int64_t>(N), static_cast<int32_t>(H), static_cast<int32_t>(K), (c_kind_host.has ? c_kind_host.v.data() : nullptr), stream()), "mma_nc_bwd_node");
}

void op_mma_nc_fused_bwd(const OptT& x, int64_t ldx, const OptT& P, int64_t ldp, const OptT& Q, int64_t ldq, const OptT& gs, int64_t ldg, const OptT& g, int64_t ldgg, const OptT& crow, int64_t ldc, std::optional<at::IntArrayRef> kind_host, const OptT& gxs, int64_t ldgx, const OptT& T, int64_t ldt, const OptT& gP, int64_t ldgp, int64_t n_targets, const OptT& t_col, const OptT& t_eid, const OptT& items, int64_t n_items, int64_t n_wave_items, const OptT& hubs, int64_t n_hubs, const OptT& partial, int64_t n_slots, const OptT& gQ, int64_t ldgq, const OptT& gx, int64_t ldgxo, const OptT& row_max, int64_t N, int64_t E, int64_t H, int64_t K, std::optional<at::IntArrayRef> act_host, int64_t drop_mode, int64_t drop_thr, int64_t seed, const OptT& seed_dev, int64_t drop_edge_base, const OptT& keep, const OptT& sync) {
  const Codes c_kind_host = codes(kind_host, static_cast<int64_t>(K), "kind_host");
  const Codes c_act_host = codes(act_host, static_cast<int64_t>(K), "act_host");
  check(mma_nc_fused_bwd(dptr<float>(x), static_cast<int64_t>(ldx), dptr<float>(P), static_cast<int64_t>(ldp), dptr<float>(Q), static_cast<int64_t>(ldq), dptr<float>(gs), static_cast<int64_t>(ldg), dptr<float>(g), static_cast<int64_t>(ldgg), dptr<float>(crow), static_cast<int64_t>(ldc), (c_kind_host.has ? c_kind_host.v.data() : nullptr), dptr<float>(gxs), static_cast<int64_t>(ldgx), dptr<float>(T), static_cast<int64_t>(ldt), dptr<float>(gP), static_cast<int64_t>(ldgp), static_cast<int64_t>(n_targets), dptr<int32_t>(t_col), dptr<int32_t>(t_eid), dptr<int32_t>(items), static_cast<int64_t>(n_items), static_cast<int64_t>(n_wave_items), dptr<int32_t>(hubs), static_cast<int64_t>(n_hubs), dptr<float>(partial), static_cast<int64_t>(n_slots), dptr<float>(gQ), static_cast<int64_t>(ldgq), dptr<float>(gx), static_cast<int64_t>(ldgxo), dptr<float>(row_max), static_cast<int64_t>(N), static_cast<int64_t>(E), static_cast<int32_t>(H), static_cast<int32_t>(K), (c_act_host.has ? c_act_host.v.data() : nullptr), static_cast<int32_t>(drop_mode), static_cast<uint32_t>(drop_thr), static_cast<uint64_t>(seed), dptr<uint64_t>(seed_dev), static_cast<int64_t>(drop_edge_base), dptr<uint8_t>(keep), dptr<int32_t>(sync), stream()), "mma_nc_fused_bwd");
}

void op_mma_csr_spmm(const OptT& rowptr, const OptT& col, const OptT& val, const OptT& B, int64_t ldb, int64_t rows_per_block, int64_t K, const OptT& bias, const OptT& out, int64_t ldo, int64_t n_rows, int64_t C) {
  check(mma_csr_spmm(dptr<int32_t>(rowptr), dptr<int32_t>(col), dptr<float>(val), dptr<float>(B), static_cast<int64_t>(ldb), static_cast<int64_t>(rows_per_block), static_cast<int32_t>(K), dptr<float>(bias), dptr<float>(out), static_cast<int64_t>(ldo), static_cast<int64_t>(n_rows), static_cast<int32_t>(C), stream()), "mma_csr_spmm");
}

void op_mma_csr_spmm_rm(const OptT& rowptr, const OptT& col, const OptT& val, const OptT& B, int64_t ldb, int64_t rows_per_block, int64_t K, const OptT& bias, const OptT& out, int64_t ldo, int64_t n_rows, int64_t C, const OptT& row_max) {
  check(mma_csr_spmm_rm(dptr<int32_t>(rowptr), dptr<int32_t>(col), dptr<float>(val), dptr<float>(B), static_cast<int64_t>(ldb), static_cast<int64_t>(rows_per_block), static_cast<int32_t>(K), dptr<float>(bias), dptr<float>(out), static_cast<int64_t>(ldo), static_cast<int64_t>(n_rows), static_cast<int32_t>(C), dptr<float>(row_max), stream()), "mma_csr_spmm_rm");
}

void op_mma_csr_spmm_items(const OptT& col, const OptT& val, const OptT& B, int64_t ldb, const OptT& bias, const OptT& out, int64_t ldo, const OptT& items, int64_t n_items, int64_t n_wave_items, const OptT& hubs, int64_t n_hubs, const OptT& partial, int64_t n_slots, int64_t C) {
  check(mma_csr_spmm_items(dptr<int32_t>(col), dptr<float>(val), dptr<float>(B), static_cast<int64_t>(ldb), dptr<float>(bias), dptr<float>(out), static_cast<int64_t>(ldo), dptr<int32_t>(items), static_cast<int64_t>(n_items), static_cast<int64_t>(n_wave_items), dptr<int32_t>(hubs), static_cast<int64_t>(n_hubs), dptr<float>(partial), static_cast<int64_t>(n_slots), static_cast<int32_t>(C), stream()), "mma_csr_spmm_items");
}

void op_mma_split_bf16x3(const OptT& in_, int64_t n, const OptT& out_3n_bf16) {
  check(mma_split_bf16x3(dptr<float>(in_), static_cast<int64_t>(n), dptr<void>(out_3n_bf16), stream()), "mma_split_bf16x3");
}

void op_mma_gemm_bf16x3(const OptT& A, int64_t lda, const OptT& Bt3, const OptT& C, int64_t ldc, int64_t M, int64_t N, int64_t K, int64_t accumulate) {
  check(mma_gemm_bf16x3(dptr<float>(A), static_cast<int64_t>(lda), dptr<void>(Bt3), dptr<float>(C), static_cast<int64_t>(ldc), static_cast<int64_t>(M), static_cast<int32_t>(N), static_cast<int32_t>(K), static_cast<int32_t>(accumulate), stream()), "mma_gemm_bf16x3");
}

void op_mma_row_absmax(const OptT& A, int64_t lda, int64_t M, int64_t cols, const OptT& out) {
  check(mma_row_absmax(dptr<float>(A), static_cast<int64_t>(lda), static_cast<int64_t>(M), static_cast<int32_t>(cols), dptr<float>(out), stream()), "mma_row_absmax");
}

void op_mma_split_f16x2(const OptT& w, int64_t stride_k, int64_t stride_n, int64_t K, int64_t N, const OptT& bt2, const OptT& col_unscale, int64_t plain_lo) {
  check(mma_split_f16x2(dptr<float>(w), static_cast<int64_t>(stride_k), static_cast<int64_t>(stride_n), static_cast<int32_t>(K), static_cast<int32_t>(N), dptr<void>(bt2), dptr<float>(col_unscale), static_cast<int32_t>(plain_lo), stream()), "mma_split_f16x2");
}

void op_mma_gemm_f16x2(const OptT& A, int64_t lda, const OptT& Bt2, const OptT& col_unscale, const OptT& C, int64_t ldc, const OptT& a_row_max, int64_t M, int64_t N) {
  check(mma_gemm_f16x2(dptr<float>(A), static_cast<int64_t>(lda), dptr<void>(Bt2), dptr<float>(col_unscale), dptr<float>(C), static_cast<int64_t>(ldc), dptr<float>(a_row_max), static_cast<int64_t>(M), static_cast<int32_t>(N), stream()), "mma_gemm_f16x2");
}

void op_mma_gemm_f16x2_k(const OptT& A, int64_t lda, const OptT& Bt2, const OptT& col_unscale, const OptT& C, int64_t ldc, const OptT& a_row_max, int64_t M, int64_t N, int64_t K) {
  check(mma_gemm_f16x2_k(dptr<float>(A), static_cast<int64_t>(lda), dptr<void>(Bt2), dptr<float>(col_unscale), dptr<float>(C), static_cast<int64_t>(ldc), dptr<float>(a_row_max), static_cast<int64_t>(M), static_cast<int32_t>(N), static_cast<int32_t>(K), stream()), "mma_gemm_f16x2_k");
}

void op_mma_gemm_f16x2_k256(const OptT& A, int64_t lda, const OptT& row_max, const OptT& Bt2, const OptT& col_unscale, const OptT& C, int64_t ldc, int64_t M, int64_t N) {
  check(mma_gemm_f16x2_k256(dptr<float>(A), static_cast<int64_t>(lda), dptr<float>(row_max), dptr<void>(Bt2), dptr<float>(col_unscale), dptr<float>(C), static_cast<int64_t>(ldc), static_cast<int64_t>(M), static_cast<int32_t>(N), stream()), "mma_gemm_f16x2_k256");
}

void op_mma_pack_f16x2_k256(const OptT& A, int64_t lda, int64_t M, const OptT& Ap, const OptT& sce, const OptT& row_max) {
  check(mma_pack_f16x2_k256(dptr<float>(A), static_cast<int64_t>(lda), static_cast<int64_t>(M), dptr<void>(Ap), dptr<int32_t>(sce), dptr<float>(row_max), stream()), "mma_pack_f16x2_k256");
}

void op_mma_gemm_f16x2_k256p(const OptT& Ap, const OptT& sce, const OptT& Bt2, const OptT& col_unscale, const OptT& C, int64_t ldc, int64_t M, int64_t N) {
  check(mma_gemm_f16x2_k256p(dptr<void>(Ap), dptr<int32_t>(sce), dptr<void>(Bt2), dptr<float>(col_unscale), dptr<float>(C), static_cast<int64_t>(ldc), static_cast<int64_t>(M), static_cast<int32_t>(N), stream()), "mma_gemm_f16x2_k256p");
}

void op_mma_gemm_f16x2_n128(const OptT& A, int64_t lda, const OptT& row_max, const OptT& Bt2, const OptT& col_unscale, const OptT& C, int64_t ldc, int64_t M, int64_t K, int64_t accumulate) {
  check(mma_gemm_f16x2_n128(dptr<float>(A), static_cast<int64_t>(lda), dptr<float>(row_max), dptr<void>(Bt2), dptr<float>(col_unscale), dptr<float>(C), static_cast<int64_t>(ldc), static_cast<int64_t>(M), static_cast<int32_t>(K), static_cast<int32_t>(accumulate), stream()), "mma_gemm_f16x2_n128");
}

void op_mma_gemm_f16x2_nlp(const OptT& A, int64_t lda, const OptT& row_max, const OptT& Bt2, const OptT& col_unscale, const OptT& C, int64_t ldc, int64_t M, int64_t N, int64_t K, int64_t accumulate) {
  check(mma_gemm_f16x2_nlp(dptr<float>(A), static_cast<int64_t>(lda), dptr<float>(row_max), dptr<void>(Bt2), dptr<float>(col_unscale), dptr<float>(C), static_cast<int64_t>(ldc), static_cast<int64_t>(M), static_cast<int32_t>(N), static_cast<int32_t>(K), static_cast<int32_t>(accumulate), stream()), "mma_gemm_f16x2_nlp");
}

void op_mma_gemm_bf16x3_tn(const OptT& X, int64_t ldx, const OptT& G, int64_t ldg, const OptT& C, const OptT& ws, int64_t ws_floats, int64_t M, int64_t KA, int64_t NC) {
  check(mma_gemm_bf16x3_tn(dptr<float>(X), static_cast<int64_t>(ldx), dptr<float>(G), static_cast<int64_t>(ldg), dptr<float>(C), dptr<float>(ws), static_cast<int64_t>(ws_floats), static_cast<int64_t>(M), static_cast<int32_t>(KA), static_cast<int32_t>(NC), stream()), "mma_gemm_bf16x3_tn");
}

void op_mma_gemm_bf16x3_tn_batched(const OptT& X, int64_t ldx, int64_t xb, const OptT& G, int64_t ldg, int64_t gb, const OptT& C, const OptT& ws, int64_t ws_floats, int64_t M, int64_t KA, int64_t NC, int64_t B) {
  check(mma_gemm_bf16x3_tn_batched(dptr<float>(X), static_cast<int64_t>(ldx), static_cast<int64_t>(xb), dptr<float>(G), static_cast<int64_t>(ldg), static_cast<int64_t>(gb), dptr<float>(C), dptr<float>(ws), static_cast<int64_t>(ws_floats), static_cast<int64_t>(M), static_cast<int32_t>(KA), static_cast<int32_t>(NC), static_cast<int32_t>(B), stream()), "mma_gemm_bf16x3_tn_batched");
}

void op_mma_gemm_f16x2_tn(const OptT& X, int64_t ldx, const OptT& G, int64_t ldg, const OptT& x_row_max, const OptT& g_row_max, const OptT& C, const OptT& ws, int64_t ws_floats, int64_t M, int64_t KA, int64_t NC) {
  check(mma_gemm_f16x2_tn(dptr<float>(X), static_cast<int64_t>(ldx), dptr<float>(G), static_cast<int64_t>(ldg), dptr<float>(x_row_max), dptr<float>(g_row_max), dptr<float>(C), dptr<float>(ws), static_cast<int64_t>(ws_floats), static_cast<int64_t>(M), static_cast<int32_t>(KA), static_cast<int32_t>(NC), stream()), "mma_gemm_f16x2_tn");
}

void op_mma_pack_rows(const OptT& src, int64_t lds, const OptT& idx, int64_t n_idx, const OptT& dst, int64_t ldd, int64_t width) {
  check(mma_pack_rows(dptr<float>(src), static_cast<int64_t>(lds), dptr<int32_t>(idx), static_cast<int64_t>(n_idx), dptr<float>(dst), static_cast<int64_t>(ldd), static_cast<int32_t>(width), stream()), "mma_pack_rows");
}

void op_mma_unpack_add_rows(const OptT& src, int64_t lds, const OptT& idx, int64_t n_idx, const OptT& dst, int64_t ldd, int64_t width) {
  check(mma_unpack_add_rows(dptr<float>(src), static_cast<int64_t>(lds), dptr<int32_t>(idx), static_cast<int64_t>(n_idx), dptr<float>(dst), static_cast<int64_t>(ldd), static_cast<int32_t>(width), stream()), "mma_unpack_add_rows");
}

void op_mma_unpack_add_rows_csr(const OptT& src, int64_t lds, const OptT& rows, const OptT& segptr, const OptT& pos, int64_t n_rows, const OptT& dst, int64_t ldd, int64_t width) {
  check(mma_unpack_add_rows_csr(dptr<float>(src), static_cast<int64_t>(lds), dptr<int32_t>(rows), dptr<int32_t>(segptr), dptr<int32_t>(pos), static_cast<int64_t>(n_rows), dptr<float>(dst), static_cast<int64_t>(ldd), static_cast<int32_t>(width), stream()), "mma_unpack_add_rows_csr");
}

void op_mma_col_sum(const OptT& g, int64_t ldg, int64_t R, int64_t C, const OptT& out, const OptT& ws, int64_t ws_floats) {
  check(mma_col_sum(dptr<float>(g), static_cast<int64_t>(ldg), static_cast<int64_t>(R), static_cast<int32_t>(C), dptr<float>(out), dptr<float>(ws), static_cast<int64_t>(ws_floats), stream()), "mma_col_sum");
}
// ... 41 lines not shown
void op_mma_skinny_linear_bwd_dx(const OptT& gy, int64_t ldg, const OptT& Wb, const OptT& gx, int64_t ldx, int64_t N, int64_t K, int64_t O) {
  check(mma_skinny_linear_bwd_dx(dptr<float>(gy), static_cast<int64_t>(ldg), dptr<float>(Wb), dptr<float>(gx), static_cast<int64_t>(ldx), static_cast<int64_t>(N), static_cast<int32_t>(K), static_cast<int32_t>(O), stream()), "mma_skinny_linear_bwd_dx");
}

void op_mma_skinny_linear_gw(const OptT& gy, int64_t ldg, const OptT& x, int64_t ldx, const OptT& part, int64_t n_part, const OptT& gw, const OptT& gb, int64_t N, int64_t K, int64_t O) {
  check(mma_skinny_linear_gw(dptr<float>(gy), static_cast<int64_t>(ldg), dptr<float>(x), static_cast<int64_t>(ldx), dptr<float>(part), static_cast<int64_t>(n_part), dptr<float>(gw), dptr<float>(gb), static_cast<int64_t>(N), static_cast<int32_t>(K), static_cast<int32_t>(O), stream()), "mma_skinny_linear_gw");
}

void op_mma_logsoftmax_nll_fwd(const OptT& x, int64_t ldx, const OptT& idx, const OptT& labels, int64_t n_idx, const OptT& logp, int64_t ldo, const OptT& loss, int64_t N, int64_t C) {
  check(mma_logsoftmax_nll_fwd(dptr<float>(x), static_cast<int64_t>(ldx), dptr<int64_t>(idx), dptr<int64_t>(labels), static_cast<int64_t>(n_idx), dptr<float>(logp), static_cast<int64_t>(ldo), dptr<float>(loss), static_cast<int64_t>(N), static_cast<int32_t>(C), stream()), "mma_logsoftmax_nll_fwd");
}

void op_mma_logsoftmax_nll_bwd(const OptT& logp, int64_t ldo, const OptT& idx, const OptT& labels, int64_t n_idx, const OptT& gloss, const OptT& gx, int64_t ldg, int64_t N, int64_t C) {
  check(mma_logsoftmax_nll_bwd(dptr<float>(logp), static_cast<int64_t>(ldo), dptr<int64_t>(idx), dptr<int64_t>(labels), static_cast<int64_t>(n_idx), dptr<float>(gloss), dptr<float>(gx), static_cast<int64_t>(ldg), static_cast<int64_t>(N), static_cast<int32_t>(C), stream()), "mma_logsoftmax_nll_bwd");
}

void op_mma_masked_bn_relu_fwd(const OptT& x, int64_t ldx, const OptT& n_valid, const OptT& gamma, const OptT& beta, const OptT& y, int64_t ldy, const OptT& mean_out, const OptT& rstd_out, const OptT& running_mean, const OptT& running_var, const OptT& n_tracked, double momentum, double eps, int64_t N, int64_t C, int64_t relu) {
  check(mma_masked_bn_relu_fwd(dptr<float>(x), static_cast<int64_t>(ldx), dptr<int64_t>(n_valid), dptr<float>(gamma), dptr<float>(beta), dptr<float>(y), static_cast<int64_t>(ldy), dptr<float>(mean_out), dptr<float>(rstd_out), dptr<float>(running_mean), dptr<float>(running_var), dptr<int64_t>(n_tracked), static_cast<float>(momentum), static_cast<float>(eps), static_cast<int64_t>(N), static_cast<int32_t>(C), static_cast<int32_t>(relu), stream()), "mma_masked_bn_relu_fwd");
}

void op_mma_masked_bn_relu_bwd(const OptT& gy, int64_t ldg, const OptT& y, int64_t ldy, const OptT& x, int64_t ldx, const OptT& mean, const OptT& rstd, const OptT& gamma, const OptT& n_valid, const OptT& gx, int64_t ldgx, const OptT& ggamma, const OptT& gbeta, int64_t N, int64_t C, int64_t relu) {
  check(mma_masked_bn_relu_bwd(dptr<float>(gy), static_cast<int64_t>(ldg), dptr<float>(y), static_cast<int64_t>(ldy), dptr<float>(x), static_cast<int64_t>(ldx), dptr<float>(mean), dptr<float>(rstd), dptr<float>(gamma), dptr<int64_t>(n_valid), dptr<float>(gx), static_cast<int64_t>(ldgx), dptr<float>(ggamma), dptr<float>(gbeta), static_cast<int64_t>(N), static_cast<int32_t>(C), static_cast<int32_t>(relu), stream()), "mma_masked_bn_relu_bwd");
}

void op_mma_pad_rows(const OptT& x, int64_t ldx, int64_t M, int64_t fin, const OptT& col, const OptT& row_index, const OptT& out, int64_t ldo, int64_t width, int64_t M_out) {
  check(mma_pad_rows(dptr<float>(x), static_cast<int64_t>(ldx), static_cast<int64_t>(M), static_cast<int32_t>(fin), dptr<float>(col), dptr<int32_t>(row_index), dptr<float>(out), static_cast<int64_t>(ldo), static_cast<int32_t>(width), static_cast<int64_t>(M_out), stream()), "mma_pad_rows");
}

void op_mma_pack_blocks(const OptT& table, int64_t n_blocks, const OptT& a_base, const OptT& b0, const OptT& b1, const OptT& b2, const OptT& b3, const OptT& b4, const OptT& b5, const OptT& b6, const OptT& b7, int64_t unpack) {
  check(mma_pack_blocks(dptr<int64_t>(table), static_cast<int64_t>(n_blocks), dptr<float>(a_base), dptr<float>(b0), dptr<float>(b1), dptr<float>(b2), dptr<float>(b3), dptr<float>(b4), dptr<float>(b5), dptr<float>(b6), dptr<float>(b7), static_cast<int32_t>(unpack), stream()), "mma_pack_blocks");
}

void op_mma_edge_fold_fwd(const OptT& We, int64_t ldw, const OptT& Wenc, const OptT& benc, const OptT& wz, const OptT& bz, int64_t TF, int64_t F, int64_t ED) {
  check(mma_edge_fold_fwd(dptr<float>(We), static_cast<int64_t>(ldw), dptr<float>(Wenc), dptr<float>(benc), dptr<float>(wz), dptr<float>(bz), static_cast<int64_t>(TF), static_cast<int32_t>(F), static_cast<int32_t>(ED), stream()), "mma_edge_fold_fwd");
}

void op_mma_edge_fold_bwd(const OptT& We, int64_t ldw, const OptT& Wenc, const OptT& benc, const OptT& gwz, const OptT& gbz, const OptT& gWe, const OptT& gWenc, const OptT& gbenc, int64_t TF, int64_t F, int64_t ED) {
  check(mma_edge_fold_bwd(dptr<float>(We), static_cast<int64_t>(ldw), dptr<float>(Wenc), dptr<float>(benc), dptr<float>(gwz), dptr<float>(gbz), dptr<float>(gWe), dptr<float>(gWenc), dptr<float>(gbenc), static_cast<int64_t>(TF), static_cast<int32_t>(F), static_cast<int32_t>(ED), stream()), "mma_edge_fold_bwd");
}

void op_mma_seed_advance(const OptT& seeds, int64_t n) {
  check(mma_seed_advance(dptr<uint64_t>(seeds), static_cast<int32_t>(n), stream()), "mma_seed_advance");
}

void op_mma_l1_loss_fwd(const OptT& pred, const OptT& target, int64_t n, const OptT& loss) {
  check(mma_l1_loss_fwd(dptr<float>(pred), dptr<float>(target), static_cast<int64_t>(n), dptr<float>(loss), stream()), "mma_l1_loss_fwd");
}

void op_mma_l1_loss_bwd(const OptT& pred, const OptT& target, int64_t n, const OptT& gloss, const OptT& gpred) {
  check(mma_l1_loss_bwd(dptr<float>(pred), dptr<float>(target), static_cast<int64_t>(n), dptr<float>(gloss), dptr<float>(gpred), stream()), "mma_l1_loss_bwd");
}

void op_mma_adam_step(const OptT& table, int64_t n_tensors, int64_t total_chunks, const OptT& step, double lr, double beta1, double beta2, double eps, double weight_decay) {
  check(mma_adam_step(dptr<void>(table), static_cast<int64_t>(n_tensors), static_cast<int64_t>(total_chunks), dptr<float>(step), lr, beta1, beta2, static_cast<float>(eps), static_cast<float>(weight_decay), stream()), "mma_adam_step");
}

void op_mma_adam_step_grads(const OptT& table, int64_t n_tensors, int64_t total_chunks, const OptT& step, double lr, double beta1, double beta2, double eps, double weight_decay, std::optional<at::IntArrayRef> grad_ptrs_host) {
  const Codes c_grad_ptrs_host = codes(grad_ptrs_host, static_cast<int64_t>(8 * n_tensors), "grad_ptrs_host");
  check(mma_adam_step_grads(dptr<void>(table), static_cast<int64_t>(n_tensors), static_cast<int64_t>(total_chunks), dptr<float>(step), lr, beta1, beta2, static_cast<float>(eps), static_cast<float>(weight_decay), (c_grad_ptrs_host.has ? c_grad_ptrs_host.v.data() : nullptr), stream()), "mma_adam_step_grads");
}

void op_mma_build_csr(const OptT& key, const OptT& other, int64_t E, int64_t N, const OptT& rowptr, const OptT& perm, const OptT& other_sorted, const OptT& long_nodes, const OptT& workspace, int64_t workspace_bytes) {
  check(mma_build_csr(dptr<int64_t>(key), dptr<int64_t>(other), static_cast<int64_t>(E), static_cast<int64_t>(N), dptr<int32_t>(rowptr), dptr<int32_t>(perm), dptr<int32_t>(other_sorted), dptr<int32_t>(long_nodes), dptr<void>(workspace), static_cast<int64_t>(workspace_bytes), stream()), "mma_build_csr");
}

void op_mma_gr_fused_fwd(const OptT& rowptr, const OptT& src, const OptT& perm, const OptT& U, const OptT& V, int64_t lduv, const OptT& Z, int64_t ldz, int64_t by_pos, const OptT& z_index, const OptT& inputs, int64_t ldi, const OptT& out, const OptT& amin8, const OptT& amax8, const OptT& amin_side, const OptT& amax_side, const OptT& mean, const OptT& var, int64_t ldsave, const OptT& long_nodes, int64_t N, int64_t E, int64_t T, int64_t F, std::optional<at::IntArrayRef> aggr_host, int64_t K, std::optional<at::IntArrayRef> scaler_host, int64_t S, double avg_log, double avg_lin, int64_t drop_mode, int64_t drop_thr, int64_t seed, const OptT& seed_dev) {
  const Codes c_aggr_host = codes(aggr_host, static_cast<int64_t>(K), "aggr_host");
  const Codes c_scaler_host = codes(scaler_host, static_cast<int64_t>(S), "scaler_host");
  check(mma_gr_fused_fwd(dptr<int32_t>(rowptr), dptr<int32_t>(src), dptr<int32_t>(perm), dptr<float>(U), dptr<float>(V), static_cast<int64_t>(lduv), dptr<float>(Z), static_cast<int64_t>(ldz), static_cast<int32_t>(by_pos), dptr<uint8_t>(z_index), dptr<float>(inputs), static_cast<int64_t>(ldi), dptr<float>(out), dptr<uint8_t>(amin8), dptr<uint8_t>(amax8), dptr<int32_t>(amin_side), dptr<int32_t>(amax_side), dptr<float>(mean), dptr<float>(var), static_cast<int64_t>(ldsave), dptr<int32_t>(long_nodes), static_cast<int64_t>(N), static_cast<int64_t>(E), static_cast<int32_t>(T), static_cast<int32_t>(F), (c_aggr_host.has ? c_aggr_host.v.data() : nullptr), static_cast<int32_t>(K), (c_scaler_host.has ? c_scaler_host.v.data() : nullptr), static_cast<int32_t>(S), static_cast<float>(avg_log), static_cast<float>(avg_lin), static_cast<int32_t>(drop_mode), static_cast<uint32_t>(drop_thr), static_cast<uint64_t>(seed), dptr<uint64_t>(seed_dev), stream()), "mma_gr_fused_fwd");
}

void op_mma_gr_fused_bwd(const OptT& rowptr, const OptT& src, const OptT& perm, const OptT& U, const OptT& V, int64_t lduv, const OptT& Z, int64_t ldz, int64_t by_pos, const OptT& z_index, const OptT& inputs, int64_t ldi, const OptT& gout, const OptT& amin8, const OptT& amax8, const OptT& amin_side, const OptT& amax_side, const OptT& mean, const OptT& var, int64_t ldsave, const OptT& long_nodes, const OptT& gmsg, int64_t ldg, const OptT& gU, int64_t ldgu, const OptT& gmsg_row_max, const OptT& gu_row_max, int64_t N, int64_t E, int64_t T, int64_t F, std::optional<at::IntArrayRef> aggr_host, int64_t K, std::optional<at::IntArrayRef> scaler_host, int64_t S, double avg_log, double avg_lin, int64_t drop_mode, int64_t drop_thr, int64_t seed, const OptT& seed_dev) {
  const Codes c_aggr_host = codes(aggr_host, static_cast<int64_t>(K), "aggr_host");
  const Codes c_scaler_host = codes(scaler_host, static_cast<int64_t>(S), "scaler_host");
  check(mma_gr_fused_bwd(dptr<int32_t>(rowptr), dptr<int32_t>(src), dptr<int32_t>(perm), dptr<float>(U), dptr<float>(V), static_cast<int64_t>(lduv), dptr<float>(Z), static_cast<int64_t>(ldz), static_cast<int32_t>(by_pos), dptr<uint8_t>(z_index), dptr<float>(inputs), static_cast<int64_t>(ldi), dptr<float>(gout), dptr<uint8_t>(amin8), dptr<uint8_t>(amax8), dptr<int32_t>(amin_side), dptr<int32_t>(amax_side), dptr<float>(mean), dptr<float>(var), static_cast<int64_t>(ldsave), dptr<int32_t>(long_nodes), dptr<float>(gmsg), static_cast<int64_t>(ldg), dptr<float>(gU), static_cast<int64_t>(ldgu), dptr<float>(gmsg_row_max), dptr<float>(gu_row_max), static_cast<int64_t>(N), static_cast<int64_t>(E), static_cast<int32_t>(T), static_cast<int32_t>(F), (c_aggr_host.has ? c_aggr_host.v.data() : nullptr), static_cast<int32_t>(K), (c_scaler_host.has ? c_scaler_host.v.data() : nullptr), static_cast<int32_t>(S), static_cast<float>(avg_log), static_cast<float>(avg_lin), static_cast<int32_t>(drop_mode), static_cast<uint32_t>(drop_thr), static_cast<uint64_t>(seed), dptr<uint64_t>(seed_dev), stream()), "mma_gr_fused_bwd");
}

}

TORCH_LIBRARY(mma_amd, m) {
  m.def("mma_nc_fused_fwd(Tensor? x, int ldx, Tensor? P, int ldp, Tensor? Q, int ldq, Tensor? rowptr, Tensor? col, Tensor? items, int n_items, int n_wave_items, Tensor? hubs, int n_hubs, Tensor(a!)? partial, int n_slots, Tensor(b!)? m, Tensor(c!)? m_sum, int ldms, Tensor(d!)? T, Tensor(e!)? sel, int ldt, Tensor(f!)? crow, int ldc, int N, int E, int H, int K, int[]? kind_host, int[]? act_host, int drop_mode, int drop_thr, int seed, Tensor? seed_dev, int drop_edge_base, Tensor? keep, Tensor(g!)? sync) -> ()");
  m.def("mma_nc_bwd_node(Tensor? g, int g_kstride, int ldgr, Tensor? sel, Tensor? T, int ldt, Tensor? rowptr, Tensor(a!)? gs, int ldgs, Tensor? crow, int ldc, Tensor(b!)? gP, int ldgp, Tensor(c!)? gxs, int ldgx, Tensor(d!)? row_max, int N, int H, int K, int[]? kind_host) -> ()");
  m.def("mma_nc_fused_bwd(Tensor? x, int ldx, Tensor? P, int ldp, Tensor? Q, int ldq, Tensor? gs, int ldg, Tensor? g, int ldgg, Tensor? crow, int ldc, int[]? kind_host, Tensor? gxs, int ldgx, Tensor? T, int ldt, Tensor(a!)? gP, int ldgp, int n_targets, Tensor? t_col, Tensor? t_eid, Tensor? items, int n_items, int n_wave_items, Tensor? hubs, int n_hubs, Tensor(b!)? partial, int n_slots, Tensor(c!)? gQ, int ldgq, Tensor(d!)? gx, int ldgxo, Tensor(e!)? row_max, int N, int E, int H, int K, int[]? act_host, int drop_mode, int drop_thr, int seed, Tensor? seed_dev, int drop_edge_base, Tensor? keep, Tensor(f!)? sync) -> ()");
  m.def("mma_csr_spmm(Tensor? rowptr, Tensor? col, Tensor? val, Tensor? B, int ldb, int rows_per_block, int K, Tensor? bias, Tensor(a!)? out, int ldo, int n_rows, int C) -> ()");
  m.def("mma_csr_spmm_rm(Tensor? rowptr, Tensor? col, Tensor? val, Tensor? B, int ldb, int rows_per_block, int K, Tensor? bias, Tensor(a!)? out, int ldo, int n_rows, int C, Tensor(b!)? row_max) -> ()");
  m.def("mma_csr_spmm_items(Tensor? col, Tensor? val, Tensor? B, int ldb, Tensor? bias, Tensor(a!)? out, int ldo, Tensor? items, int n_items, int n_wave_items, Tensor? hubs, int n_hubs, Tensor(b!)? partial, int n_slots, int C) -> ()");
  m.def("mma_split_bf16x3(Tensor? in_, int n, Tensor(a!)? out_3n_bf16) -> ()");
  m.def("mma_gemm_bf16x3(Tensor? A, int lda, Tensor? Bt3, Tensor(a!)? C, int ldc, int M, int N, int K, int accumulate) -> ()");
  m.def("mma_row_absmax(Tensor? A, int lda, int M, int cols, Tensor(a!)? out) -> ()");
  m.def("mma_split_f16x2(Tensor? w, int stride_k, int stride_n, int K, int N, Tensor(a!)? bt2, Tensor(b!)? col_unscale, int plain_lo) -> ()");
  m.def("mma_gemm_f16x2(Tensor? A, int lda, Tensor? Bt2, Tensor? col_unscale, Tensor(a!)? C, int ldc, Tensor(b!)? a_row_max, int M, int N) -> ()");
  m.def("mma_gemm_f16x2_k(Tensor? A, int lda, Tensor? Bt2, Tensor? col_unscale, Tensor(a!)? C, int ldc, Tensor(b!)? a_row_max, int M, int N, int K) -> ()");
  m.def("mma_gemm_f16x2_k256(Tensor? A, int lda, Tensor? row_max, Tensor? Bt2, Tensor? col_unscale, Tensor(a!)? C, int ldc, int M, int N) -> ()");
  m.def("mma_pack_f16x2_k256(Tensor? A, int lda, int M, Tensor(a!)? Ap, Tensor(b!)? sce, Tensor(c!)? row_max) -> ()");
  m.def("mma_gemm_f16x2_k256p(Tensor? Ap, Tensor? sce, Tensor? Bt2, Tensor? col_unscale, Tensor(a!)? C, int ldc, int M, int N) -> ()");
  m.def("mma_gemm_f16x2_n128(Tensor? A, int lda, Tensor? row_max, Tensor? Bt2, Tensor? col_unscale, Tensor(a!)? C, int ldc, int M, int K, int accumulate) -> ()");
  m.def("mma_gemm_f16x2_nlp(Tensor? A, int lda, Tensor? row_max, Tensor? Bt2, Tensor? col_unscale, Tensor(a!)? C, int ldc, int M, int N, int K, int accumulate) -> ()");
  m.def("mma_gemm_bf16x3_tn(Tensor? X, int ldx, Tensor? G, int ldg, Tensor(a!)? C, Tensor(b!)? ws, int ws_floats, int M, int KA, int NC) -> ()");
  m.def("mma_gemm_bf16x3_tn_batched(Tensor? X, int ldx, int xb, Tensor? G, int ldg, int gb, Tensor(a!)? C, Tensor(b!)? ws, int ws_floats, int M, int KA, int NC, int B) -> ()");
  m.def("mma_gemm_f16x2_tn(Tensor? X, int ldx, Tensor? G, int ldg, Tensor? x_row_max, Tensor? g_row_max, Tensor(a!)? C, Tensor(b!)? ws, int ws_floats, int M, int KA, int NC) -> ()");
  m.def("mma_pack_rows(Tensor? src, int lds, Tensor? idx, int n_idx, Tensor(a!)? dst, int ldd, int width) -> ()");
  m.def("mma_unpack_add_rows(Tensor? src, int lds, Tensor? idx, int n_idx, Tensor(a!)? dst, int ldd, int width) -> ()");
  m.def("mma_unpack_add_rows_csr(Tensor? src, int lds, Tensor? rows, Tensor? segptr, Tensor? pos, int n_rows, Tensor(a!)? dst, int ldd, int width) -> ()");
  m.def("mma_col_sum(Tensor? g, int ldg, int R, int C, Tensor(a!)? out, Tensor(b!)? ws, int ws_floats) -> ()");
  m.def("mma_tower_linear_bwd(Tensor? gy, Tensor? a, Tensor? W, Tensor(a!)? ga, Tensor(b!)? part, int n_blocks, int N, int T, int O, int C) -> ()");
  m.def("mma_tower_post_weights(Tensor? Wo, int T, int O, int S, int KF, Tensor(a!)? Wa, Tensor(b!)? Wb) -> ()");
  m.def("mma_skinny_linear_weights(Tensor? W, int O, int K, Tensor(a!)? Wa, Tensor(b!)? Wb) -> ()");
  m.def("mma_tower_post_gw_reduce(Tensor? part, int n_chunks, int T, int S, int O, int KF, Tensor(a!)? gWo) -> ()");
  m.def("mma_tower_post_pre(Tensor? rowptr, Tensor(a!)? pre, int N, int S, int[]? scaler_host, float avg_log, float avg_lin) -> ()");
  m.def("mma_tower_post_fwd(Tensor? agg, int lda, Tensor? pre, Tensor? Wa, Tensor(a!)? y, int ldy, int N, int T, int KF, int S, int O, int[]? scaler_host, float avg_log, float avg_lin) -> ()");
  m.def("mma_tower_post_bwd(Tensor? gy, int ldg, Tensor? pre, Tensor? Wb, Tensor(a!)? gagg, int lda, Tensor(b!)? gys, int ldgs, int N, int T, int KF, int S, int O, int[]? scaler_host, float avg_log, float avg_lin) -> ()");
  m.def("mma_tower_post_gw(Tensor? gy, int ldg, Tensor? agg, int lda, Tensor? pre, Tensor(a!)? part, int n_chunks, int N, int T, int KF, int S, int O, int[]? scaler_host, float avg_log, float avg_lin) -> ()");
  m.def("mma_skinny_linear_fwd(Tensor? x, int ldx, Tensor? Wa, Tensor? bias, Tensor? addend, int ldadd, Tensor(a!)? y, int ldy, int N, int K, int O) -> ()");
  m.def("mma_skinny_linear_bwd_dx(Tensor? gy, int ldg, Tensor? Wb, Tensor(a!)? gx, int ldx, int N, int K, int O) -> ()");
  m.def("mma_skinny_linear_gw(Tensor? gy, int ldg, Tensor? x, int ldx, Tensor(a!)? part, int n_part, Tensor(b!)? gw, Tensor(c!)? gb, int N, int K, int O) -> ()");
  m.def("mma_logsoftmax_nll_fwd(Tensor? x, int ldx, Tensor? idx, Tensor? labels, int n_idx, Tensor(a!)? logp, int ldo, Tensor(b!)? loss, int N, int C) -> ()");
  m.def("mma_logsoftmax_nll_bwd(Tensor? logp, int ldo, Tensor? idx, Tensor? labels, int n_idx, Tensor? gloss, Tensor(a!)? gx, int ldg, int N, int C) -> ()");
  m.def("mma_masked_bn_relu_fwd(Tensor? x, int ldx, Tensor? n_valid, Tensor? gamma, Tensor? beta, Tensor(a!)? y, int ldy, Tensor(b!)? mean_out, Tensor(c!)? rstd_out, Tensor(d!)? running_mean, Tensor(e!)? running_var, Tensor(f!)? n_tracked, float momentum, float eps, int N, int C, int relu) -> ()");
  m.def("mma_masked_bn_relu_bwd(Tensor? gy, int ldg, Tensor? y, int ldy, Tensor? x, int ldx, Tensor? mean, Tensor? rstd, Tensor? gamma, Tensor? n_valid, Tensor(a!)? gx, int ldgx, Tensor(b!)? ggamma, Tensor(c!)? gbeta, int N, int C, int relu) -> ()");
  m.def("mma_pad_rows(Tensor? x, int ldx, int M, int fin, Tensor? col, Tensor? row_index, Tensor(a!)? out, int ldo, int width, int M_out) -> ()");
  m.def("mma_pack_blocks(Tensor? table, int n_blocks, Tensor(a!)? a_base, Tensor(b!)? b0, Tensor(c!)? b1, Tensor(d!)? b2, Tensor(e!)? b3, Tensor(f!)? b4, Tensor(g!)? b5, Tensor(h!)? b6, Tensor(i!)? b7, int unpack) -> ()");
  m.def("mma_edge_fold_fwd(Tensor? We, int ldw, Tensor? Wenc, Tensor? benc, Tensor(a!)? wz, Tensor(b!)? bz, int TF, int F, int ED) -> ()");
  m.def("mma_edge_fold_bwd(Tensor? We, int ldw, Tensor? Wenc, Tensor? benc, Tensor? gwz, Tensor? gbz, Tensor(a!)? gWe, Tensor(b!)? gWenc, Tensor(c!)? gbenc, int TF, int F, int ED) -> ()");
  m.def("mma_seed_advance(Tensor(a!)? seeds, int n) -> ()");
  m.def("mma_l1_loss_fwd(Tensor? pred, Tensor? target, int n, Tensor(a!)? loss) -> ()");
  m.def("mma_l1_loss_bwd(Tensor? pred, Tensor? target, int n, Tensor? gloss, Tensor(a!)? gpred) -> ()");
  m.def("mma_adam_step(Tensor? table, int n_tensors, int total_chunks, Tensor(a!)? step, float lr, float beta1, float beta2, float eps, float weight_decay) -> ()");
  m.def("mma_adam_step_grads(Tensor? table, int n_tensors, int total_chunks, Tensor(a!)? step, float lr, float beta1, float beta2, float eps, float weight_decay, int[]? grad_ptrs_host) -> ()");
  m.def("mma_build_csr(Tensor? key, Tensor? other, int E, int N, Tensor(a!)? rowptr, Tensor(b!)? perm, Tensor(c!)? other_sorted, Tensor(d!)? long_nodes, Tensor(e!)? workspace, int workspace_bytes) -> ()");
  m.def("mma_gr_fused_fwd(Tensor? rowptr, Tensor? src, Tensor? perm, Tensor? U, Tensor? V, int lduv, Tensor? Z, int ldz, int by_pos, Tensor? z_index, Tensor? inputs, int ldi, Tensor(a!)? out, Tensor(b!)? amin8, Tensor(c!)? amax8, Tensor(d!)? amin_side, Tensor(e!)? amax_side, Tensor(f!)? mean, Tensor(g!)? var, int ldsave, Tensor? long_nodes, int N, int E, int T, int F, int[]? aggr_host, int K, int[]? scaler_host, int S, float avg_log, float avg_lin, int drop_mode, int drop_thr, int seed, Tensor? seed_dev) -> ()");
  m.def("mma_gr_fused_bwd(Tensor? rowptr, Tensor? src, Tensor? perm, Tensor? U, Tensor? V, int lduv, Tensor? Z, int ldz, int by_pos, Tensor? z_index, Tensor? inputs, int ldi, Tensor? gout, Tensor? amin8, Tensor? amax8, Tensor? amin_side, Tensor? amax_side, Tensor? mean, Tensor? var, int ldsave, Tensor? long_nodes, Tensor(a!)? gmsg, int ldg, Tensor(b!)? gU, int ldgu, Tensor(c!)? gmsg_row_max, Tensor(d!)? gu_row_max, int N, int E, int T, int F, int[]? aggr_host, int K, int[]? scaler_host, int S, float avg_log, float avg_lin, int drop_mode, int drop_thr, int seed, Tensor? seed_dev) -> ()");
}

TORCH_LIBRARY_IMPL(mma_amd, CompositeExplicitAutograd, m) {
  m.impl("mma_nc_fused_fwd", &op_mma_nc_fused_fwd);
  m.impl("mma_nc_bwd_node", &op_mma_nc_bwd_node);
  m.impl("mma_nc_fused_bwd", &op_mma_nc_fused_bwd);
  m.impl("mma_csr_spmm", &op_mma_csr_spmm);
  m.impl("mma_csr_spmm_rm", &op_mma_csr_spmm_rm);
  m.impl("mma_csr_spmm_items", &op_mma_csr_spmm_items);
  m.impl("mma_split_bf16x3", &op_mma_split_bf16x3);
  m.impl("mma_gemm_bf16x3", &op_mma_gemm_bf16x3);
  m.impl("mma_row_absmax", &op_mma_row_absmax);
  m.impl("mma_split_f16x2", &op_mma_split_f16x2);
  m.impl("mma_gemm_f16x2", &op_mma_gemm_f16x2);
  m.impl("mma_gemm_f16x2_k", &op_mma_gemm_f16x2_k);
  m.impl("mma_gemm_f16x2_k256", &op_mma_gemm_f16x2_k256);
  m.impl("mma_pack_f16x2_k256", &op_mma_pack_f16x2_k256);
  m.impl("mma_gemm_f16x2_k256p", &op_mma_gemm_f16x2_k256p);
  m.impl("mma_gemm_f16x2_n128", &op_mma_gemm_f16x2_n128);
  m.impl("mma_gemm_f16x2_nlp", &op_mma_gemm_f16x2_nlp);
  m.impl("mma_gemm_bf16x3_tn", &op_mma_gemm_bf16x3_tn);
  m.impl("mma_gemm_bf16x3_tn_batched", &op_mma_gemm_bf16x3_tn_batched);
  m.impl("mma_gemm_f16x2_tn", &op_mma_gemm_f16x2_tn);
  m.impl("mma_pack_rows", &op_mma_pack_rows);
  m.impl("mma_unpack_add_rows", &op_mma_unpack_add_rows);
  m.impl("mma_unpack_add_rows_csr", &op_mma_unpack_add_rows_csr);
  m.impl("mma_col_sum", &op_mma_col_sum);
  m.impl("mma_tower_linear_bwd", &op_mma_tower_linear_bwd);
  m.impl("mma_tower_post_weights", &op_mma_tower_post_weights);
  m.impl("mma_skinny_linear_weights", &op_mma_skinny_linear_weights);
  m.impl("mma_tower_post_gw_reduce", &op_mma_tower_post_gw_reduce);
  m.impl("mma_tower_post_pre", &op_mma_tower_post_pre);
  m.impl("mma_tower_post_fwd", &op_mma_tower_post_fwd);
  m.impl("mma_tower_post_bwd", &op_mma_tower_post_bwd);
  m.impl("mma_tower_post_gw", &op_mma_tower_post_gw);
  m.impl("mma_skinny_linear_fwd", &op_mma_skinny_linear_fwd);
  m.impl("mma_skinny_linear_bwd_dx", &op_mma_skinny_linear_bwd_dx);
  m.impl("mma_skinny_linear_gw", &op_mma_skinny_linear_gw);
  m.impl("mma_logsoftmax_nll_fwd", &op_mma_logsoftmax_nll_fwd);
  m.impl("mma_logsoftmax_nll_bwd", &op_mma_logsoftmax_nll_bwd);
  m.impl("mma_masked_bn_relu_fwd", &op_mma_masked_bn_relu_fwd);
  m.impl("mma_masked_bn_relu_bwd", &op_mma_masked_bn_relu_bwd);
  m.impl("mma_pad_rows", &op_mma_pad_rows);
  m.impl("mma_pack_blocks", &op_mma_pack_blocks);
  m.impl("mma_edge_fold_fwd", &op_mma_edge_fold_fwd);
  m.impl("mma_edge_fold_bwd", &op_mma_edge_fold_bwd);
  m.impl("mma_seed_advance", &op_mma_seed_advance);
  m.impl("mma_l1_loss_fwd", &op_mma_l1_loss_fwd);
  m.impl("mma_l1_loss_bwd", &op_mma_l1_loss_bwd);
  m.impl("mma_adam_step", &op_mma_adam_step);
  m.impl("mma_adam_step_grads", &op_mma_adam_step_grads);
  m.impl("mma_build_csr", &op_mma_build_csr);
  m.impl("mma_gr_fused_fwd", &op_mma_gr_fused_fwd);
  m.impl("mma_gr_fused_bwd", &op_mma_gr_fused_bwd);
}
```

mma_amd/functional.py:

```python


import torch

from . import _lib
from ._env import flag
from ._lib import call, host_codes, ptr, require_gpu, stream_ptr

SHARED_GRAD_BWD = True
FUSE_NODE_BWD = flag("MMA_FUSE_NODE_BWD")
TIMER = None


class _NoSpan:
    def __enter__(self):
        return self

    def __exit__(self, *a):
        return False


def _span(name, nbytes=0, flops=0, mfma=None):
    return TIMER.span(name, nbytes, flops, mfma) if TIMER is not None else _NoSpan()


KIND = {"sum": 0, "mean": 1, "max": 2, "min": 3, "softmax": 4, "softmin": 5}
ACT_SIGMOID, ACT_RAW = 0, 1
DROP_NONE, DROP_HASH, DROP_EXPLICIT = 0, 1, 2


class DropoutSpec:

    def __init__(self, p=0.0, seed=None, keep=None, seed_tensor=None):
        self.p = float(p)
        if not (0.0 <= self.p < 1.0):
            raise ValueError("dropout probability has to be in [0, 1), but got %r" % p)
        self.keep = keep
        self.seed_tensor = seed_tensor
        if keep is not None:
            self.mode, self.thr = DROP_EXPLICIT, int(round(self.p * 65536))
            if self.thr / 65536.0 != self.p:
                raise ValueError("explicit keep masks need p = i/65536 so that 1/(1-p) is reproduced exactly")
        elif self.p == 0.0:
            self.mode, self.thr = DROP_NONE, 0
        else:
            self.mode, self.thr = DROP_HASH, min(65535, max(1, int(round(self.p * 65536))))
        self.p_applied = self.thr / 65536.0 if self.mode != DROP_NONE else 0.0
        if seed is None:
            seed = int(torch.empty((), dtype=torch.int64).random_().item()) if (self.mode == DROP_HASH and seed_tensor is None) else 0
        self.seed = seed & 0xFFFFFFFFFFFFFFFF

    def args(self):
        return self.mode, self.thr, self.seed, ptr(self.seed_tensor), ptr(self.keep)


def crow_floats(H, kinds):
    return _lib.query("mma_nc_crow_floats", H, len(kinds), host_codes(kinds))


def nc_fwd_launch(x_src, P, Q, graph, kinds, acts, drop, reduce_k, save, shared=None):
    K = len(kinds)
    S, H = x_src.shape
    N = graph.N
    shared = (reduce_k and SHARED_GRAD_BWD) if shared is None else shared
    assert x_src.dtype == torch.float32 and P.dtype == torch.float32 and Q.dtype == torch.float32
    assert S == graph.n_src and P.shape == (N, K * H) and Q.shape == (S, K * H) and 1 <= K <= 8
    assert x_src.is_contiguous() and P.stride(1) == 1 and Q.stride(1) == 1
    dev = x_src.device
    m = None if reduce_k else torch.empty((K, N, H), device=dev, dtype=torch.float32)
    msum = torch.empty((N, H), device=dev, dtype=torch.float32) if reduce_k else None
    T = torch.empty((N, K * H), device=dev, dtype=torch.float32) if save else None
    sel = torch.empty((N, K * H), device=dev, dtype=torch.uint8) if save and not shared else None
    crow = None
    if save and shared:
        ldc = crow_floats(H, kinds)
        crow = (torch.zeros if H % 4 else torch.empty)((N, ldc), device=dev, dtype=torch.float32)
    partial = torch.empty((graph.n_slots, 2 * K * H), device=dev, dtype=torch.float32) if graph.n_slots else None
    if drop.keep is not None:
        assert drop.keep.dtype == torch.uint8 and drop.keep.is_contiguous() and drop.keep.is_cuda and \
            tuple(drop.keep.shape) == (K, graph.E, H), "explicit keep mask must be a contiguous (K,E,H) uint8 GPU tensor"
    mode, thr, seed, seed_dev, keep = drop.args()
    with _span("nc_fused_fwd"):
        call("mma_nc_fused_fwd", ptr(x_src), x_src.stride(0), ptr(P), P.stride(0), ptr(Q), Q.stride(0),
             ptr(graph.rowptr), ptr(graph.col), ptr(graph.items), graph.items.shape[0], graph.n_wave_items,
             ptr(graph.hubs) if graph.n_slots else None, graph.hubs.shape[0], ptr(partial), graph.n_slots,
             ptr(m), ptr(msum), H, ptr(T), ptr(sel), K * H, ptr(crow), crow.stride(0) if crow is not None else 0,
             N, graph.E, H, K, host_codes(kinds), host_codes(acts),
             mode, thr, seed, seed_dev, graph.edge_base, keep, ptr(graph.sync(0)), stream_ptr())
    return (msum if reduce_k else m), T, sel, crow


def nc_bwd_node_launch(g, reduce_k, sel, crow, T, graph, kinds, H, shared, gP=None, row_max=None):
    K, N, S = len(kinds), graph.N, graph.n_src
    dev = g.device
    gs = None if shared else torch.empty((N, K * H), device=dev, dtype=torch.float32)
    if gP is None:
        gP = torch.empty((N, K * H), device=dev, dtype=torch.float32)
    gxs = torch.empty((S, H), device=dev, dtype=torch.float32)
    if S > N:
        gxs[N:].zero_()
    with _span("nc_bwd_node"):
        call("mma_nc_bwd_node", ptr(g), 0 if reduce_k else N * H, H, ptr(sel), ptr(T), K * H, ptr(graph.rowptr),
             ptr(gs), K * H, ptr(crow), crow.stride(0) if crow is not None else 0, ptr(gP), gP.stride(0), ptr(gxs), H, ptr(row_max),
             N, H, K, host_codes(kinds), stream_ptr())
    return gs, gP, gxs


def nc_bwd_edges_launch(x_src, P, Q, gs, g, crow, gxs, graph, kinds, acts, drop, gQ, gx, partial, part=None, row_max=None, T=None, gP=None):
    K = len(acts)
    S, H = x_src.shape
    items, n_wave, hubs = part if part is not None else (graph.t_items, graph.t_n_wave_items, graph.t_hubs)
    shared = gs is None
    mode, thr, seed, seed_dev, keep = drop.args()
    with _span("nc_fused_bwd"):
        call("mma_nc_fused_bwd", ptr(x_src), x_src.stride(0), ptr(P), P.stride(0), ptr(Q), Q.stride(0),
             ptr(gs), K * H, ptr(g) if shared else None, g.stride(0) if shared else 0,
             ptr(crow) if shared else None, crow.stride(0) if shared else 0, host_codes(kinds) if shared else None,
             ptr(gxs), H, ptr(T), K * H if T is not None else 0, ptr(gP), gP.stride(0) if gP is not None else 0, graph.N,
             ptr(graph.t_col), ptr(graph.t_eid), ptr(items), items.shape[0], n_wave,
             ptr(hubs) if hubs.shape[0] else None, hubs.shape[0], ptr(partial), graph.t_n_slots if hubs.shape[0] else 0,
             ptr(gQ), gQ.stride(0), ptr(gx), H, ptr(row_max), S, graph.E, H, K, host_codes(acts), mode, thr, seed, seed_dev, graph.edge_base,
             keep, ptr(graph.sync(1)) if part is None else None, stream_ptr())


class _NCFused(torch.autograd.Function):

    @staticmethod
    def forward(ctx, x_src, P, Q, graph, kinds, acts, drop, reduce_k):
        require_gpu(x_src, P, Q)
        x_src = x_src.contiguous()
        if P.stride(1) != 1:
            P = P.contiguous()
        if Q.stride(1) != 1:
            Q = Q.contiguous()
        out, T, sel, crow = nc_fwd_launch(x_src, P, Q, graph, kinds, acts, drop, reduce_k, any(ctx.needs_input_grad[:3]))
        ctx.graph, ctx.kinds, ctx.acts, ctx.drop, ctx.reduce_k = graph, kinds, acts, drop, reduce_k
        ctx.save_for_backward(x_src, P, Q, T, sel, crow)
        return out

    @staticmethod
    def backward(ctx, g):
        graph, kinds, acts, drop, reduce_k = ctx.graph, ctx.kinds, ctx.acts, ctx.drop, ctx.reduce_k
        x_src, P, Q, T, sel, crow = ctx.saved_tensors
        shared = crow is not None
        K = len(kinds)
        H, S = x_src.shape[1], graph.n_src
        g = g.contiguous()
        dev = g.device
        gQ = torch.empty((S, K * H), device=dev, dtype=torch.float32)
        gx = torch.empty((S, H), device=dev, dtype=torch.float32)
        partial = (torch.empty((graph.t_n_slots, (K + 1) * H), device=dev, dtype=torch.float32)
                   if graph.t_n_slots else None)
        if shared and FUSE_NODE_BWD:
            gP = torch.empty((graph.N, K * H), device=dev, dtype=torch.float32)
            nc_bwd_edges_launch(x_src, P, Q, None, g, crow, None, graph, kinds, acts, drop, gQ, gx, partial, T=T, gP=gP)
        else:
            gs, gP, gxs = nc_bwd_node_launch(g, reduce_k, sel, crow, T, graph, kinds, H, shared)
            nc_bwd_edges_launch(x_src, P, Q, gs, g, crow, gxs, graph, kinds, acts, drop, gQ, gx, partial)
        return gx, gP, gQ, None, None, None, None, None


class _NCLocalLayer(torch.autograd.Function):

    @staticmethod
    def forward(ctx, x, wtop, wbot, graph, kinds, acts, drop):
        from .dense import mm_into
        require_gpu(x)
        x = x.contiguous()
        N, H = x.shape
        K = len(kinds)
        KH = K * H
        PQ = torch.empty((N, 2 * KH), device=x.device, dtype=torch.float32)
        ctx.cat_given = wbot is None
        wcat = wtop if ctx.cat_given else torch.cat([wtop, wbot], 1)
        need = any(ctx.needs_input_grad[:3])
        box = [] if need else None
        mm_into(x, wcat, PQ, row_max_box=box)
        msum, T, sel, crow = nc_fwd_launch(x, PQ[:, :KH], PQ[:, KH:], graph, kinds, acts, drop, True, need)
        ctx.graph, ctx.kinds, ctx.acts, ctx.drop = graph, kinds, acts, drop
        ctx.save_for_backward(x, PQ, T, sel, crow, wcat, box[0] if box else None)
        return msum

    @staticmethod
    def backward(ctx, g):
        from .dense import f16x2_n128_ok, rows_mm_add_, xt_g
        graph, kinds, acts, drop = ctx.graph, ctx.kinds, ctx.acts, ctx.drop
        x, PQ, T, sel, crow, wcat, x_row_max = ctx.saved_tensors
        N, H = x.shape
        K = len(kinds)
        KH = K * H
        g = g.contiguous()
        gPQ = torch.empty((N, 2 * KH), device=g.device, dtype=torch.float32)
        row_max = torch.zeros((N,), device=g.device, dtype=torch.float32) if f16x2_n128_ok(N, 2 * KH, H) and K <= 8 else None
        gx = torch.empty((N, H), device=g.device, dtype=torch.float32)
        partial = (torch.empty((graph.t_n_slots, (K + 1) * H), device=g.device, dtype=torch.float32)
                   if graph.t_n_slots else None)
        shared = crow is not None
        if shared and FUSE_NODE_BWD:
            nc_bwd_edges_launch(x, PQ[:, :KH], PQ[:, KH:], None, g, crow, None, graph, kinds, acts, drop, gPQ[:, KH:], gx, partial,
                                row_max=row_max, T=T, gP=gPQ[:, :KH])
        else:
            gs, gP, gxs = nc_bwd_node_launch(g, True, sel, crow, T, graph, kinds, H, shared, gP=gPQ[:, :KH], row_max=row_max)
            nc_bwd_edges_launch(x, PQ[:, :KH], PQ[:, KH:], gs, g, crow, gxs, graph, kinds, acts, drop, gPQ[:, KH:], gx, partial,
                                row_max=row_max)
        rows_mm_add_(gx, gPQ, wcat.t(), row_max)
        gw = xt_g(x, gPQ, x_row_max, row_max) if (ctx.needs_input_grad[1] or ctx.needs_input_grad[2]) else None
        if ctx.cat_given:
            return gx, gw, None, None, None, None, None
        return gx, (gw[:, :KH] if gw is not None else None), (gw[:, KH:] if gw is not None else None), None, None, None, None


def nc_local_layer(x, wtop, wbot, graph, kinds, acts, drop=None):
    assert graph.n_src == graph.N
    return _NCLocalLayer.apply(x, wtop, wbot, graph, tuple(kinds), tuple(acts), drop or DropoutSpec(0.0))


class DeviceSeeds:

    def __init__(self, n, device):
        if torch.cuda.is_current_stream_capturing():
            raise _lib.MMALibraryError("mma_amd: run one warm-up step before capturing a graph (the dropout seed states are drawn on the first step)")
        self.n = n
        self.buf = torch.empty(2 * n, dtype=torch.int64, device=device)
        self.buf.random_()
        self.seeds = self.buf[:n]
        self.device = self.buf.device

    def advance(self):
        call("mma_seed_advance", ptr(self.buf), self.n, stream_ptr())
        return self.seeds


class SeedSlot:

    def __init__(self, shared, i):
        self.shared, self.i, self.n, self.device = shared, i, 1, shared.device
        self.seeds = shared.seeds[i:i + 1]

    def advance(self):
        if self.i == 0:
            self.shared.advance()
        return self.seeds


class _MaskWeights(torch.autograd.Function):

    @staticmethod
    def forward(ctx, *masks):
        K = len(masks)
        H = masks[0].shape[1]
        ctx.shape = (K, H)
        return torch.cat([w[:H] for w in masks] + [w[H:] for w in masks], 1)

    @staticmethod
    def backward(ctx, g):
        K, H = ctx.shape
        gm = g.view(H, 2, K, H).permute(2, 1, 0, 3).reshape(K, 2 * H, H)
        return tuple(gm[k] for k in range(K))


def mask_weights(masks):
    return _MaskWeights.apply(*masks)


def nc_fused_aggregate(x, P, Q, graph, kinds, acts, drop=None, reduce_k=False):
    return _NCFused.apply(x, P, Q, graph, tuple(kinds), tuple(acts), drop or DropoutSpec(0.0), bool(reduce_k))


def _spmm_call(rowptr, col, val, items, hubs, n_slots, B, rows_per_block, K, bias, out, n_rows, C, n_wave_items=None):
    if K == 1 and items is not None:
        partial = torch.empty((n_slots, C), device=B.device, dtype=torch.float32) if n_slots else None
        call("mma_csr_spmm_items", ptr(col), ptr(val), ptr(B), B.stride(0), ptr(bias), ptr(out), C, ptr(items), items.shape[0],
             items.shape[0] if n_wave_items is None else n_wave_items,
             ptr(hubs) if n_slots else None, hubs.shape[0], ptr(partial), n_slots, C, stream_ptr())
    else:
        call("mma_csr_spmm", ptr(rowptr), ptr(col), ptr(val), ptr(B), B.stride(0), rows_per_block, K,
             ptr(bias), ptr(out), C, n_rows, C, stream_ptr())


class _CsrSpmm(torch.autograd.Function):

    @staticmethod
    def forward(ctx, B, bias, sg, K):
        require_gpu(B, bias)
        B = B.contiguous()
        rows_per_block = B.shape[0] // K
        assert B.shape[0] == K * rows_per_block and rows_per_block == sg.n_cols
        C = B.shape[1]
        out = torch.empty((sg.n_rows, C), device=B.device, dtype=torch.float32)
        with _span("csr_spmm_fwd", nbytes=K * sg.col.numel() * (8 + 4 * C) + sg.n_rows * (16 + 4 * C), flops=2 * K * sg.col.numel() * C):
            _spmm_call(sg.rowptr, sg.col, sg.val, sg.items, sg.hubs, sg.n_slots, B, rows_per_block, K, bias, out, sg.n_rows, C,
                       sg.n_wave_items)
# ... 325 lines not shown
```

mma_amd/layers.py:

```python
import math

import torch
from torch.nn.modules.module import Module

from . import functional as Fn
from .dense import mm
from ._lib import require_gpu
from .graph import DEFAULT_CHUNK, NCGraph, SpmmGraph
from .scalers import SCALERS, scaler_row_factor, true_degree_row_factor

_AGG = {
    "sum": ("sum", False), "sum2": ("sum", False), "sum3": ("sum", False), "sum4": ("sum", False),
    "mean": ("mean", False), "mean2": ("mean", False), "mean3": ("mean", True), "mean4": ("mean", False),
    "max": ("max", True), "max2": ("max", False), "max3": ("max", False), "max4": ("max", False),
    "min": ("min", True), "min2": ("min", False), "min3": ("min", False), "min4": ("min", False),
    "softmax": ("softmax", True), "softmin": ("softmin", True),
}
_UNUSABLE = ("std", "normalized_mean", "moment_3")
_MASK_NAMES = ["moment_3", "sum", "sum2", "sum3", "sum4", "mean", "mean2", "mean3", "mean4", "max", "max2", "max3",
               "max4", "min", "min2", "min3", "min4", "softmax", "softmin", "std", "normalized_mean"]


class GraphConvolution(Module):

# ... 65 lines not shown
                 weight_mean3, weight_mean4, weight_max, weight_max2, weight_max3, weight_max4, weight_min,
                 weight_min2, weight_min3, weight_min4, weight_softmax, weight_softmin, weight_std,
                 weight_normalized_mean]
        for name, w in zip(_MASK_NAMES, masks):
            setattr(self, "mask_" + name, w)

        self.all_aggregators = {name: getattr(self, "learnable_" + name) for name in _MASK_NAMES}
        self.AGGREGATORS = dict()
        for aggr in aggregator_list:
            self.AGGREGATORS[aggr] = self.all_aggregators[aggr]
        self.aggregator_names = list(self.AGGREGATORS)
        self.aggregators = [self.AGGREGATORS[a] for a in self.AGGREGATORS]
        self.scalers = [SCALERS[s] for s in SCALERS]
        self.num_aggregators = len(self.aggregators)

        self.reset_parameters()
        self.avg_d = avg_d
        self.self_loop = None

        self.strict_reference = bool(strict_reference)
        self.scaler_names = list(scalers) if scalers is not None else list(SCALERS)
        self.compound_scalers = bool(compound_scalers)
        if self.strict_reference and (scalers is not None or compound_scalers):
            raise ValueError("scalers / compound_scalers are extensions: pass strict_reference=False to use them")
        self._row_factor = None

        self._chunk = chunk
        self._graph = add_all if isinstance(add_all, NCGraph) else None
        self._sg = None
        self._sg_scaled = None
        self.drop_override = None
        self.graph_capturable = False
        self._seeds = None
        self._seed_buf = None

    def reset_parameters(self):
        stdv = 1. / math.sqrt(self.weight.size(0))
        self.weight.data.uniform_(-stdv, stdv)
        for name in _MASK_NAMES:
            w = getattr(self, "mask_" + name)
            s = 1. / math.sqrt(w.size(1))
            setattr(self, "mask_stdv_" + name, s)
            w.data.uniform_(-s, s)
        if self.bias is not None:
            self.bias.data.uniform_(-stdv, stdv)

    def graph(self, device):
        if self._graph is None or self._graph.device != device:
            self._graph = NCGraph.from_add_all(self.add_all, device, chunk=self._chunk, H=self.in_features)
        return self._graph

    def _scaler_factor(self, N, device):
        if self.strict_reference:
            return scaler_row_factor(N, device)
        if self._row_factor is None or self._row_factor[0] != device:
            g = self.graph(device)
            deg = (g.rowptr[1:] - g.rowptr[:-1])
            self._row_factor = (device, true_degree_row_factor(deg, self.scaler_names, self.compound_scalers, self.avg_d))
        return self._row_factor[1]

    def _codes(self, names):
        kinds, acts = [], []
        for n in names:
            if n in _UNUSABLE:
                raise NotImplementedError(
                    "aggregator %r is unusable in the reference (layers.py:731-851: learnable_std calls the full-graph "
                    "mean inside the node loop, normalized_mean/moment_3 raise NameError); not implemented" % n)
            kind, rawq = _AGG[n]
            kinds.append(Fn.KIND[kind])
            acts.append(Fn.ACT_RAW if (rawq and self.activation == "new_sigmoid") else Fn.ACT_SIGMOID)
        return kinds, acts

    def _drop(self, names, device=None):
        if self.drop_override is not None:
            return self.drop_override
        if self.graph_capturable and self.dropout > 0 and device is not None:
            n_groups = -(-len(names) // 8)
            if self._seeds is None or self._seeds.device != device or self._seeds.n != n_groups:
                self._seeds = Fn.DeviceSeeds(n_groups, device)
                self._seed_buf = self._seeds.seeds
            return Fn.DropoutSpec(self.dropout, seed_tensor=self._seeds.advance())
        return Fn.DropoutSpec(self.dropout)

    def _aggregate(self, names, input, drop=None, reduce_k=False):
        require_gpu(input)
        H = input.shape[1]
        kinds, acts = self._codes(names)
        masks = [getattr(self, "mask_" + n) for n in names]
        graph = self.graph(input.device)
        if reduce_k:
            return Fn.nc_local_layer(input, Fn.mask_weights(masks), None, graph, kinds, acts, drop or self._drop(names, input.device))
        wtop, wbot = torch.cat([w[:H] for w in masks], 1), torch.cat([w[H:] for w in masks], 1)
        return Fn.nc_fused_aggregate(input, mm(input, wtop), mm(input, wbot), graph, kinds, acts,
                                     drop or self._drop(names, input.device))

    def _aggregate_all(self, names, input, reduce_k=False):
        outs = []
        base = self._drop(names, input.device)
        for g0 in range(0, len(names), 8):
            grp = names[g0:g0 + 8]
            drop = base
            if base.keep is not None:
                drop = Fn.DropoutSpec(base.p, keep=base.keep[g0:g0 + 8].contiguous())
            elif g0 and base.seed_tensor is not None and base.seed_tensor.numel() > g0 // 8:
                drop = Fn.DropoutSpec(base.p, seed_tensor=base.seed_tensor[g0 // 8:])
            elif g0 and base.seed_tensor is None:
                drop = Fn.DropoutSpec(base.p, seed=base.seed + g0)
            outs.append(self._aggregate(grp, input, drop, reduce_k))
        if reduce_k:
            return outs[0] if len(outs) == 1 else torch.stack(outs).sum(0)
        return outs[0] if len(outs) == 1 else torch.cat(outs, 0)

    def forward(self, input, adj):
        N = input.shape[0]
        msum = self._aggregate_all(self.aggregator_names, input, reduce_k=True)
        if self._sg is None or self._sg[0] is not adj:
            self._sg = (adj, adj if isinstance(adj, SpmmGraph) else SpmmGraph.from_torch_sparse(adj, input.device))
        factor = self._scaler_factor(N, input.device)
        if self._sg_scaled is None or self._sg_scaled[0] is not self._sg[1] or self._sg_scaled[1] is not factor:
            self._sg_scaled = (self._sg[1], factor, self._sg[1].scaled_by_source(factor))
        return Fn.csr_spmm(mm(msum, self.weight), self.bias, self._sg_scaled[2], 1)

    def __repr__(self):
        return self.__class__.__name__ + ' (' + str(self.in_features) + ' -> ' + str(self.out_features) + ')'


def _make_learnable(name):
    def run(self, input):
        return self._aggregate([name], input)[0]
    if name.startswith("max"):
        def learnable(self, input, adj, min_value=-math.inf):
            return run(self, input)
    elif name.startswith("min"):
        def learnable(self, input, adj, max_value=math.inf):
            return run(self, input)
    else:
        def learnable(self, input, adj):
            return run(self, input)
    learnable.__name__ = "learnable_" + name
    learnable.__doc__ = "Fused HIP form of layers.py learnable_%s(input, adj) -> (N, H)." % name
    return learnable


for _n in _MASK_NAMES:
    setattr(MMA, "learnable_" + _n, _make_learnable(_n))
```

Baseline: 752.6 million.

## Fuse output-weight backward projection into NC fused backward kernel

Adds a tail variant of the local layer. When the output width C is small, the backward kernel rebuilds the msum gradient on the fly from gt (N×C) and the tail weight held in LDS, instead of first materialising g = gt·Wᵀ (N×H) and then reading it. This removes a separate GEMM and an N×H gradient round trip through memory. The cost is extra per-edge FMA work to recompute the gradient for every neighbour, plus more template instantiations.

```diff
diff --git a/include/mma_amd.h b/include/mma_amd.h
--- a/include/mma_amd.h
+++ b/include/mma_amd.h
@@ -7,7 +7,7 @@
 extern "C" {
 #endif
 
-#define MMA_ABI_VERSION 36
+#define MMA_ABI_VERSION 37
 #define MMA_MAX_K 8
 
 enum {
@@ -78,6 +78,22 @@
     int32_t drop_mode, uint32_t drop_thr, uint64_t seed, const uint64_t* seed_dev, int64_t drop_edge_base, const uint8_t* keep,
     int32_t* sync,
     void* stream);
+
+#define MMA_NC_TAIL_MAX_C 16
+int mma_tail_nc_fused_bwd(
+    const float* x, int64_t ldx, const float* P, int64_t ldp, const float* Q, int64_t ldq,
+    const float* gt, int64_t ldgt,
+    const float* wt, int32_t C,
+    const float* crow, int64_t ldc, const uint8_t* kind_host,
+    const float* T, int64_t ldt, float* gP, int64_t ldgp,
+    const int32_t* t_col, const int32_t* t_eid,
+    const int32_t* items, int64_t n_items, int64_t n_wave_items, const int32_t* hubs, int64_t n_hubs,
+    float* partial, int64_t n_slots,
+    float* gQ, int64_t ldgq, float* gx, int64_t ldgxo, float* row_max,
+    int64_t N, int64_t E, int32_t H, int32_t K,
+    const uint8_t* act_host,
+    int32_t drop_mode, uint32_t drop_thr, uint64_t seed, const uint64_t* seed_dev, int64_t drop_edge_base, const uint8_t* keep,
+    int32_t* sync, void* stream);
 
 int mma_csr_spmm(
     const int32_t* rowptr, const int32_t* col, const float* val,
diff --git a/mma_amd/_abi.py b/mma_amd/_abi.py
--- a/mma_amd/_abi.py
+++ b/mma_amd/_abi.py
@@ -1,4 +1,4 @@
-ABI_VERSION = 36
+ABI_VERSION = 37
 FUNCTIONS = {
     "mma_abi_version": ("int", []),
     "mma_last_error": ("const char*", []),
@@ -7,6 +7,7 @@
     "mma_nc_bwd_node": ("int", [("T", "T", "g"), ("i", "i64", "g_kstride"), ("i", "i64", "ldgr"), ("T", "T", "sel"), ("T", "T", "T"), ("i", "i64", "ldt"), ("T", "T", "rowptr"), ("T", "T", "gs"), ("i", "i64", "ldgs"), ("T", "T", "crow"), ("i", "i64", "ldc"), ("T", "T", "gP"), ("i", "i64", "ldgp"), ("T", "T", "gxs"), ("i", "i64", "ldgx"), ("T", "T", "row_max"), ("i", "i64", "N"), ("i", "i32", "H"), ("i", "i32", "K"), ("H", "H", "kind_host"), ("S", "S", "stream")]),
     "mma_nc_crow_floats": ("int64_t", [("i", "i32", "H"), ("i", "i32", "K"), ("H", "H", "kind_host")]),
     "mma_nc_fused_bwd": ("int", [("T", "T", "x"), ("i", "i64", "ldx"), ("T", "T", "P"), ("i", "i64", "ldp"), ("T", "T", "Q"), ("i", "i64", "ldq"), ("T", "T", "gs"), ("i", "i64", "ldg"), ("T", "T", "g"), ("i", "i64", "ldgg"), ("T", "T", "crow"), ("i", "i64", "ldc"), ("H", "H", "kind_host"), ("T", "T", "gxs"), ("i", "i64", "ldgx"), ("T", "T", "T"), ("i", "i64", "ldt"), ("T", "T", "gP"), ("i", "i64", "ldgp"), ("i", "i64", "n_targets"), ("T", "T", "t_col"), ("T", "T", "t_eid"), ("T", "T", "items"), ("i", "i64", "n_items"), ("i", "i64", "n_wave_items"), ("T", "T", "hubs"), ("i", "i64", "n_hubs"), ("T", "T", "partial"), ("i", "i64", "n_slots"), ("T", "T", "gQ"), ("i", "i64", "ldgq"), ("T", "T", "gx"), ("i", "i64", "ldgxo"), ("T", "T", "row_max"), ("i", "i64", "N"), ("i", "i64", "E"), ("i", "i32", "H"), ("i", "i32", "K"), ("H", "H", "act_host"), ("i", "i32", "drop_mode"), ("i", "u32", "drop_thr"), ("i", "u64", "seed"), ("T", "T", "seed_dev"), ("i", "i64", "drop_edge_base"), ("T", "T", "keep"), ("T", "T", "sync"), ("S", "S", "stream")]),
+    "mma_tail_nc_fused_bwd": ("int", [("T", "T", "x"), ("i", "i64", "ldx"), ("T", "T", "P"), ("i", "i64", "ldp"), ("T", "T", "Q"), ("i", "i64", "ldq"), ("T", "T", "gt"), ("i", "i64", "ldgt"), ("T", "T", "wt"), ("i", "i32", "C"), ("T", "T", "crow"), ("i", "i64", "ldc"), ("H", "H", "kind_host"), ("T", "T", "T"), ("i", "i64", "ldt"), ("T", "T", "gP"), ("i", "i64", "ldgp"), ("T", "T", "t_col"), ("T", "T", "t_eid"), ("T", "T", "items"), ("i", "i64", "n_items"), ("i", "i64", "n_wave_items"), ("T", "T", "hubs"), ("i", "i64", "n_hubs"), ("T", "T", "partial"), ("i", "i64", "n_slots"), ("T", "T", "gQ"), ("i", "i64", "ldgq"), ("T", "T", "gx"), ("i", "i64", "ldgxo"), ("T", "T", "row_max"), ("i", "i64", "N"), ("i", "i64", "E"), ("i", "i32", "H"), ("i", "i32", "K"), ("H", "H", "act_host"), ("i", "i32", "drop_mode"), ("i", "u32", "drop_thr"), ("i", "u64", "seed"), ("T", "T", "seed_dev"), ("i", "i64", "drop_edge_base"), ("T", "T", "keep"), ("T", "T", "sync"), ("S", "S", "stream")]),
     "mma_csr_spmm": ("int", [("T", "T", "rowptr"), ("T", "T", "col"), ("T", "T", "val"), ("T", "T", "B"), ("i", "i64", "ldb"), ("i", "i64", "rows_per_block"), ("i", "i32", "K"), ("T", "T", "bias"), ("T", "T", "out"), ("i", "i64", "ldo"), ("i", "i64", "n_rows"), ("i", "i32", "C"), ("S", "S", "stream")]),
     "mma_csr_spmm_rm": ("int", [("T", "T", "rowptr"), ("T", "T", "col"), ("T", "T", "val"), ("T", "T", "B"), ("i", "i64", "ldb"), ("i", "i64", "rows_per_block"), ("i", "i32", "K"), ("T", "T", "bias"), ("T", "T", "out"), ("i", "i64", "ldo"), ("i", "i64", "n_rows"), ("i", "i32", "C"), ("T", "T", "row_max"), ("S", "S", "stream")]),
     "mma_csr_spmm_items": ("int", [("T", "T", "col"), ("T", "T", "val"), ("T", "T", "B"), ("i", "i64", "ldb"), ("T", "T", "bias"), ("T", "T", "out"), ("i", "i64", "ldo"), ("T", "T", "items"), ("i", "i64", "n_items"), ("i", "i64", "n_wave_items"), ("T", "T", "hubs"), ("i", "i64", "n_hubs"), ("T", "T", "partial"), ("i", "i64", "n_slots"), ("i", "i32", "C"), ("S", "S", "stream")]),
diff --git a/mma_amd/csrc/nc_fused.hip b/mma_amd/csrc/nc_fused.hip
--- a/mma_amd/csrc/nc_fused.hip
+++ b/mma_amd/csrc/nc_fused.hip
@@ -412,11 +412,77 @@
   int first_pass;
   uint32_t* rowmax;
   const int4* hubs; int64_t n_hubs; unsigned* sync; unsigned n_slots;
+  const float* gt; int64_t ldgt; const float* wt;
 };
 
+typedef float mma_f32x2 __attribute__((ext_vector_type(2)));
+template <int TQ> struct TailRow { float v[TQ > 0 ? 4 * TQ : 1]; };
+template <int TQ> struct TailWLds {
+  const float4* t; int lpr, li;
+  __device__ __forceinline__ float4 piece(int pr, int c2) const { return t[(pr * 2 * TQ + c2) * lpr + li]; }
+};
+template <int TQ> struct TailWGlobal {
+  const float* wt; int c;
+  __device__ __forceinline__ float4 piece(int pr, int c2) const {
+    const float* r0 = wt + (size_t)(c + 2 * pr) * (4 * TQ) + 2 * c2;
+    const float* r1 = r0 + 4 * TQ;
+    return make_float4(r0[0], r1[0], r0[1], r1[1]);
+  }
+};
+template <int TQ>
+__device__ __forceinline__ float4* tail_w_tile() {
+  __shared__ float4 tile[4 * TQ * kWave];
+  return tile;
+}
+template <int TQ>
+__device__ __forceinline__ TailWLds<TQ> tail_fill_w(const float* wt, int H, int lpr, int lane) {
+  float4* tile = tail_w_tile<TQ>();
+  for (int e = threadIdx.x; e < 4 * TQ * lpr; e += kBlock) {
+    const int li = e & (lpr - 1), piece = e / lpr;
+    const int col = ((int)blockIdx.y * lpr + li) * 4;
+    tile[e] = col < H ? TailWGlobal<TQ>{wt, col}.piece(piece / (2 * TQ), piece % (2 * TQ)) : make_float4(0.f, 0.f, 0.f, 0.f);
+  }
+  __syncthreads();
+  return TailWLds<TQ>{tile, lpr, lane & (lpr - 1)};
+}
+template <int TQ>
+__device__ __forceinline__ TailRow<TQ> tail_load_gt(const float* gt, int64_t ldgt, int node) {
+  TailRow<TQ> r;
+  const float* row = gt + row_off(node, ldgt);
+#pragma unroll
+  for (int q = 0; q < TQ; ++q) {
+    const Vec<4> t = ldv<4>(row + 4 * q);
+#pragma unroll
+    for (int j = 0; j < 4; ++j) r.v[4 * q + j] = t.v[j];
+  }
+  return r;
+}
+template <int TQ, typename W>
+__device__ __forceinline__ Vec<4> tail_rebuild(const TailRow<TQ>& t, const W& w) {
+  Vec<4> g;
+#pragma unroll
+  for (int pr = 0; pr < 2; ++pr) {
+    mma_f32x2 a;
+#pragma unroll
+    for (int c2 = 0; c2 < 2 * TQ; ++c2) {
+      const float4 p = w.piece(pr, c2);
+      const mma_f32x2 t0 = {t.v[2 * c2], t.v[2 * c2]}, t1 = {t.v[2 * c2 + 1], t.v[2 * c2 + 1]};
+      const mma_f32x2 w0 = {p.x, p.y}, w1 = {p.z, p.w};
+      a = c2 == 0 ? t0 * w0 : __builtin_elementwise_fma(t0, w0, a);
+      a = __builtin_elementwise_fma(t1, w1, a);
+    }
+    g.v[2 * pr] = a.x; g.v[2 * pr + 1] = a.y;
+  }
+  return g;
+}
+template <int VEC, int TQ, typename W>
+__device__ __forceinline__ Vec<VEC> nc_bwd_target_g(const NcBwdParams& p, int node, int c, const W& w) {
+  if constexpr (TQ > 0) return tail_rebuild<TQ>(tail_load_gt<TQ>(p.gt, p.ldgt, node), w);
+  else return ldv_nt<VEC>(p.g + row_off(node, p.ldgg) + c);
+}
+
 template <int VEC>
-__device__ __forceinline__ Vec<VEC> nc_bwd_epilogue(const NcBwdParams& p, int node, int c, int k0, int nk, float& mx) {
-  const Vec<VEC> g = ldv_nt<VEC>(p.g + row_off(node, p.ldgg) + c);
+__device__ __forceinline__ Vec<VEC> nc_bwd_epilogue(const NcBwdParams& p, const Vec<VEC>& g, int node, int c, int k0, int nk, float& mx) {
   const float* crow = p.crow + row_off(node, p.ldc);
   const float inv_deg = crow[0];
   Vec<VEC> gxd = vzero<VEC>();
@@ -448,10 +514,10 @@
   return gxd;
 }
 
-template <int VEC>
+template <int VEC, int TQ>
 __device__ __forceinline__ void nc_bwd_finalize_body(const NcBwdParams& p, const int4* hubs, int64_t n_hubs, const int64_t first, const int64_t step);
 
-template <int K, int VEC, int DM, bool SHARED, bool MULTI, bool EPI, bool ONE = false>
+template <int K, int VEC, int DM, bool SHARED, bool MULTI, bool EPI, bool ONE = false, int TQ = 0>
 __device__ __forceinline__ void nc_bwd_body(const NcBwdParams& p, const int bx, const int nbx) {
   constexpr bool DROP = DM != MMA_DROP_NONE;
   const DropParams dp = (DM == MMA_DROP_HASH || DM == MMA_DROP_HASH16) ? drop_resolve(p.drop) : p.drop;
@@ -474,6 +540,8 @@
   const int waves_per_block = kBlock / kWave;
   const int64_t stride = (int64_t)nbx * waves_per_block;
   const int64_t n_witems = (p.n_items + gpw - 1) / gpw;
+  TailWLds<TQ> tw{};
+  if constexpr (TQ > 0) tw = tail_fill_w<TQ>(p.wt, p.H, lpr, lane);
 
   for (int64_t it0 = (int64_t)bx * waves_per_block + (threadIdx.x >> 6); it0 < n_witems; it0 += stride) {
     int node, ebeg, eend, slot;
@@ -513,7 +581,7 @@
       const int mye = (DROP && gl < cnt) ? p.t_eid[ebeg + base + gl] : 0;
       for (int t0 = 0; t0 < ucnt; t0 += U * epg) {
         int tt[U]; bool ev[U]; uint32_t eid[U]; Vec<VEC> gv[U][SHARED ? 1 : K]; Vec<VEC> pv[U][K];
-        uint32_t codes[U][K]; float idg[U];
+        uint32_t codes[U][K]; float idg[U]; TailRow<TQ> gtv[U];
 #pragma unroll
         for (int u = 0; u < U; ++u) {
           tt[u] = t0 + u * epg + sub;
@@ -522,7 +590,8 @@
           const int ii = __shfl(myi, gbase + (tl & (G - 1)), kWave);
           eid[u] = DROP ? (uint32_t)__shfl(mye, gbase + (tl & (G - 1)), kWave) : 0u;
           if (SHARED) {
-            gv[u][0] = ldv<VEC>(p.g + row_off(ii, p.ldgg) + cc);
+            if constexpr (TQ > 0) gtv[u] = tail_load_gt<TQ>(p.gt, p.ldgt, ii);
+            else gv[u][0] = ldv<VEC>(p.g + row_off(ii, p.ldgg) + cc);
             const float* crow = p.crow + row_off(ii, p.ldc);
             idg[u] = crow[0];
 #pragma unroll
@@ -544,6 +613,7 @@
 #pragma unroll
         for (int u = 0; u < U; ++u) {
           const bool live = ev[u];
+          if constexpr (TQ > 0) gv[u][0] = tail_rebuild<TQ>(gtv[u], tw);
 #pragma unroll
           for (int kk = 0; kk < (SHARED ? 1 : K); ++kk)
 #pragma unroll
@@ -593,7 +663,7 @@
     const bool tgt = EPI && writer && slot < 0 && (int64_t)node < p.n_targets;
     Vec<VEC> gxd = vzero<VEC>();
     float mxp = 0.f;
-    if (EPI) { if (tgt) gxd = nc_bwd_epilogue<VEC>(p, node, c, p.k_base, K, mxp); }
+    if (EPI) { if (tgt) gxd = nc_bwd_epilogue<VEC>(p, nc_bwd_target_g<VEC, TQ>(p, node, c, tw), node, c, p.k_base, K, mxp); }
 
     for (int off = G / 2; off >= lpr; off >>= 1) {
 #pragma unroll
@@ -667,7 +737,7 @@
         if (wrote && gl == 0) ticket = atomicAdd(p.sync, 1u) + 1u;
         if (__builtin_amdgcn_ballot_w64(ticket == p.n_slots) != 0) {
           __builtin_amdgcn_fence(__ATOMIC_ACQUIRE, "agent");
-          nc_bwd_finalize_body<VEC>(p, p.hubs, p.n_hubs, lane, kWave);
+          nc_bwd_finalize_body<VEC, TQ>(p, p.hubs, p.n_hubs, lane, kWave);
           if (lane == 0) *p.sync = 0u;
         }
       }
@@ -675,12 +745,12 @@
   }
 }
 
-template <int K, int VEC, int DM, bool SHARED, bool MULTI, bool EPI>
+template <int K, int VEC, int DM, bool SHARED, bool MULTI, bool EPI, int TQ = 0>
 __global__ __launch_bounds__(kBlock, (K <= 4 ? MMA_MIN_WAVES : 1)) void nc_bwd_kernel(const NcBwdParams p) {
-  nc_bwd_body<K, VEC, DM, SHARED, MULTI, EPI>(p, (int)blockIdx.x, (int)gridDim.x);
-}
-
-template <int VEC>
+  nc_bwd_body<K, VEC, DM, SHARED, MULTI, EPI, false, TQ>(p, (int)blockIdx.x, (int)gridDim.x);
+}
+
+template <int VEC, int TQ>
 __device__ __forceinline__ void nc_bwd_finalize_body(const NcBwdParams& p, const int4* hubs, int64_t n_hubs, const int64_t first, const int64_t step) {
   const int per_row = (p.H + VEC - 1) / VEC;
   const bool epi = p.T != nullptr;
@@ -705,11 +775,12 @@
     }
     const int node = hub.x;
     const bool tgt = epi && (int64_t)node < p.n_targets;
+    const TailWGlobal<TQ> tw{p.wt, c};
     Vec<VEC> o;
     if (k < p.K_total) {
       const Vec<VEC> xj = ldv<VEC>(p.x + (size_t)node * p.ldx + c);
       float mxq = 0.f;
-      if (tgt) nc_bwd_epilogue<VEC>(p, node, c, k, 1, mxq);
+      if (tgt) nc_bwd_epilogue<VEC>(p, nc_bwd_target_g<VEC, TQ>(p, node, c, tw), node, c, k, 1, mxq);
 #pragma unroll
       for (int i = 0; i < VEC; ++i) o.v[i] = xj.v[i] * s.v[i];
       stv_nt<VEC>(p.gQ + (size_t)node * p.ldgq + (size_t)k * p.H + c, o);
@@ -721,7 +792,9 @@
     } else {
       Vec<VEC> g0 = vzero<VEC>();
       if (tgt) {
-        const Vec<VEC> g = ldv<VEC>(p.g + row_off(node, p.ldgg) + c);
+        Vec<VEC> g;
+        if constexpr (TQ > 0) g = nc_bwd_target_g<VEC, TQ>(p, node, c, tw);
+        else g = ldv<VEC>(p.g + row_off(node, p.ldgg) + c);
         const float* crow = p.crow + row_off(node, p.ldc);
         const float inv_deg = crow[0];
         for (int kk = 0; kk < p.K_total; ++kk) {
@@ -743,21 +816,21 @@
     }
   }
 }
-template <int VEC>
+template <int VEC, int TQ = 0>
 __global__ __launch_bounds__(kBlock) void nc_bwd_finalize_kernel(const NcBwdParams p, const int4* hubs, int64_t n_hubs) {
-  nc_bwd_finalize_body<VEC>(p, hubs, n_hubs, (int64_t)blockIdx.x * blockDim.x + threadIdx.x, (int64_t)gridDim.x * blockDim.x);
-}
-
-template <int K, int VEC, int DM, bool EPI>
+  nc_bwd_finalize_body<VEC, TQ>(p, hubs, n_hubs, (int64_t)blockIdx.x * blockDim.x + threadIdx.x, (int64_t)gridDim.x * blockDim.x);
+}
+
+template <int K, int VEC, int DM, bool EPI, int TQ = 0>
 __global__ __launch_bounds__(kBlock, (K <= 4 ? MMA_MIN_WAVES : 1)) void nc_bwd_small_kernel(const NcBwdParams p, const NcSmallPlan sp) {
   if ((int)blockIdx.x < sp.blocks_a) {
     NcBwdParams q = p;
     q.n_items = sp.n_wave_items;
-    nc_bwd_body<K, VEC, DM, true, false, EPI, true>(q, (int)blockIdx.x, sp.blocks_a);
+    nc_bwd_body<K, VEC, DM, true, false, EPI, true, TQ>(q, (int)blockIdx.x, sp.blocks_a);
   } else {
     NcBwdParams q = p;
     q.items = p.items + sp.n_wave_items; q.n_items = p.n_items - sp.n_wave_items;
-    nc_bwd_body<K, VEC, DM, true, true, EPI, true>(q, (int)blockIdx.x - sp.blocks_a, (int)gridDim.x - sp.blocks_a);
+    nc_bwd_body<K, VEC, DM, true, true, EPI, true, TQ>(q, (int)blockIdx.x - sp.blocks_a, (int)gridDim.x - sp.blocks_a);
   }
 }
 
@@ -837,27 +910,37 @@
     default: launch_fwd<8, VEC, MULTI>(p, grid, save, dm, st); break;
   }
 }
-template <int K, int VEC, bool MULTI>
+template <int K, int VEC, bool MULTI, int TQ = 0>
 static void launch_bwd(const NcBwdParams& p, dim3 grid, int dm, hipStream_t st) {
   const bool shared = p.gs == nullptr;
   const bool epi = p.T != nullptr;
-#define MMA_BWD(DM, SHARED, EPI) hipLaunchKernelGGL((nc_bwd_kernel<K, VEC, DM, SHARED, MULTI, EPI>), grid, dim3(kBlock), 0, st, p)
-#define MMA_BWD_DM(SHARED, EPI) \
-  do { if (dm == MMA_DROP_HASH) MMA_BWD(MMA_DROP_HASH, SHARED, EPI); else if (dm == MMA_DROP_HASH16) MMA_BWD(MMA_DROP_HASH16, SHARED, EPI); else if (dm == MMA_DROP_EXPLICIT) MMA_BWD(MMA_DROP_EXPLICIT, SHARED, EPI); \
-       else MMA_BWD(MMA_DROP_NONE, SHARED, EPI); } while (0)
-  if (shared) { if (epi) MMA_BWD_DM(true, true); else MMA_BWD_DM(true, false); }
-  else MMA_BWD_DM(false, false);
+#define MMA_BWD(DM, SHARED, EPI, TQ_) hipLaunchKernelGGL((nc_bwd_kernel<K, VEC, DM, SHARED, MULTI, EPI, TQ_>), grid, dim3(kBlock), 0, st, p)
+#define MMA_BWD_DM(SHARED, EPI, TQ_) \
+  do { if (dm == MMA_DROP_HASH) MMA_BWD(MMA_DROP_HASH, SHARED, EPI, TQ_); else if (dm == MMA_DROP_HASH16) MMA_BWD(MMA_DROP_HASH16, SHARED, EPI, TQ_); else if (dm == MMA_DROP_EXPLICIT) MMA_BWD(MMA_DROP_EXPLICIT, SHARED, EPI, TQ_); \
+       else MMA_BWD(MMA_DROP_NONE, SHARED, EPI, TQ_); } while (0)
+  if (TQ > 0) MMA_BWD_DM(true, true, TQ);
+  else if (shared) { if (epi) MMA_BWD_DM(true, true, 0); else MMA_BWD_DM(true, false, 0); }
+  else MMA_BWD_DM(false, false, 0);
 #undef MMA_BWD_DM
 #undef MMA_BWD
 }
-template <int VEC, bool MULTI>
+template <int VEC, bool MULTI, int TQ = 0>
 static void launch_bwd_k(int Ks, const NcBwdParams& p, dim3 grid, int dm, hipStream_t st) {
   switch (Ks) {
-    case 1: launch_bwd<1, VEC, MULTI>(p, grid, dm, st); break;
-    case 2: launch_bwd<2, VEC, MULTI>(p, grid, dm, st); break;
-    case 3: launch_bwd<3, VEC, MULTI>(p, grid, dm, st); break;
-    case 4: launch_bwd<4, VEC, MULTI>(p, grid, dm, st); break;
-    default: launch_bwd<8, VEC, MULTI>(p, grid, dm, st); break;
+    case 1: launch_bwd<1, VEC, MULTI, TQ>(p, grid, dm, st); break;
+    case 2: launch_bwd<2, VEC, MULTI, TQ>(p, grid, dm, st); break;
+    case 3: launch_bwd<3, VEC, MULTI, TQ>(p, grid, dm, st); break;
+    case 4: launch_bwd<4, VEC, MULTI, TQ>(p, grid, dm, st); break;
+    default: launch_bwd<8, VEC, MULTI, TQ>(p, grid, dm, st); break;
+  }
+}
+template <bool MULTI>
+static void launch_bwd_tail(int tq, int Ks, const NcBwdParams& p, dim3 grid, int dm, hipStream_t st) {
+  switch (tq) {
+    case 1: launch_bwd_k<4, MULTI, 1>(Ks, p, grid, dm, st); break;
+    case 2: launch_bwd_k<4, MULTI, 2>(Ks, p, grid, dm, st); break;
+    case 3: launch_bwd_k<4, MULTI, 3>(Ks, p, grid, dm, st); break;
+    default: launch_bwd_k<4, MULTI, 4>(Ks, p, grid, dm, st); break;
   }
 }
 
@@ -868,13 +951,24 @@
   else { if (dm == MMA_DROP_HASH) MMA_FWD_S(false, MMA_DROP_HASH); else if (dm == MMA_DROP_HASH16) MMA_FWD_S(false, MMA_DROP_HASH16); else MMA_FWD_S(false, MMA_DROP_NONE); }
 #undef MMA_FWD_S
 }
-template <int K>
+template <int K, int TQ = 0>
 static void launch_bwd_small(const NcBwdParams& p, const NcSmallPlan& sp, dim3 grid, int dm, hipStream_t st) {
   const bool epi = p.T != nullptr;
-#define MMA_BWD_S(DM, EPI) hipLaunchKernelGGL((nc_bwd_small_kernel<K, 4, DM, EPI>), grid, dim3(kBlock), 0, st, p, sp)
-  if (epi) { if (dm == MMA_DROP_HASH) MMA_BWD_S(MMA_DROP_HASH, true); else if (dm == MMA_DROP_HASH16) MMA_BWD_S(MMA_DROP_HASH16, true); else MMA_BWD_S(MMA_DROP_NONE, true); }
+#define MMA_BWD_S(DM, EPI) hipLaunchKernelGGL((nc_bwd_small_kernel<K, 4, DM, EPI, TQ>), grid, dim3(kBlock), 0, st, p, sp)
+  if (TQ > 0) { if (dm == MMA_DROP_HASH) MMA_BWD_S(MMA_DROP_HASH, true); else if (dm == MMA_DROP_HASH16) MMA_BWD_S(MMA_DROP_HASH16, true); else MMA_BWD_S(MMA_DROP_NONE, true); }
+  else if (epi) { if (dm == MMA_DROP_HASH) MMA_BWD_S(MMA_DROP_HASH, true); else if (dm == MMA_DROP_HASH16) MMA_BWD_S(MMA_DROP_HASH16, true); else MMA_BWD_S(MMA_DROP_NONE, true); }
   else { if (dm == MMA_DROP_HASH) MMA_BWD_S(MMA_DROP_HASH, false); else if (dm == MMA_DROP_HASH16) MMA_BWD_S(MMA_DROP_HASH16, false); else MMA_BWD_S(MMA_DROP_NONE, false); }
 #undef MMA_BWD_S
+}
+template <int TQ>
+static void launch_bwd_small_k(int K, const NcBwdParams& p, const NcSmallPlan& sp, dim3 grid, int dm, hipStream_t st) {
+  switch (K) {
+    case 1: launch_bwd_small<1, TQ>(p, sp, grid, dm, st); break;
+    case 2: launch_bwd_small<2, TQ>(p, sp, grid, dm, st); break;
+    case 3: launch_bwd_small<3, TQ>(p, sp, grid, dm, st); break;
+    case 4: launch_bwd_small<4, TQ>(p, sp, grid, dm, st); break;
+    default: launch_bwd_small<8, TQ>(p, sp, grid, dm, st); break;
+  }
 }
 static bool small_plan(int32_t* sync, int K, const Geometry& g, int dm, int64_t n_items, int64_t n_wave_items, int64_t n_hubs, int64_t n_slots,
                        int64_t finalize_elems, NcSmallPlan* sp, dim3* grid) {
@@ -1036,7 +1130,7 @@
   return check_launch("nc_bwd_node_kernel");
 }
 
-extern "C" int mma_nc_fused_bwd(
+static int nc_fused_bwd_impl(
     const float* x, int64_t ldx, const float* P, int64_t ldp, const float* Q, int64_t ldq,
     const float* gs, int64_t ldg, const float* g, int64_t ldgg, const float* crow, int64_t ldc, const uint8_t* kind_host,
     const float* gxs, int64_t ldgx, const float* T, int64_t ldt, float* gP, int64_t ldgp, int64_t n_targets,
@@ -1045,7 +1139,8 @@
     float* partial, int64_t n_slots, float* gQ, int64_t ldgq, float* gx, int64_t ldgxo, float* row_max,
     int64_t N, int64_t E, int32_t H, int32_t K, const uint8_t* act_host,
     int32_t drop_mode, uint32_t drop_thr, uint64_t seed, const uint64_t* seed_dev, int64_t drop_edge_base, const uint8_t* keep,
-    int32_t* sync, void* stream) {
+    int32_t* sync, void* stream, const float* gt, int64_t ldgt, const float* wt, int tq) {
+  const bool tail = tq > 0;
   MMA_REQUIRE(N >= 0 && E >= 0 && N < (1LL << 31) && E < (1LL << 31), "N=%lld E=%lld out of int32 range", (long long)N, (long long)E);
   MMA_REQUIRE(H >= 1 && K >= 1 && K <= MMA_MAX_K, "H=%d K=%d unsupported (1<=K<=%d)", H, K, MMA_MAX_K);
   MMA_REQUIRE(ldx >= H && ldp >= (int64_t)K * H && ldq >= (int64_t)K * H && (!gs || ldg >= (int64_t)K * H) && ldgq >= (int64_t)K * H &&
@@ -1057,7 +1152,7 @@
   if (N == 0 || n_items == 0) return 0;
   const bool shared = gs == nullptr;
   const bool epi = T != nullptr;
-  MMA_REQUIRE(!shared || (g && crow && kind_host && ldgg >= H),
+  MMA_REQUIRE(!shared || ((tail || (g && ldgg >= H)) && crow && kind_host),
               "give gs (n_targets,K*H), or the shared-gradient form: g (n_targets,H), the code rows crow K1 wrote, and kinds");
   MMA_REQUIRE(!epi || (shared && gP && ldt >= (int64_t)K * H && ldgp >= (int64_t)K * H && n_targets >= 0 && n_targets <= N),
               "the fused node-level epilogue (T given) needs the shared-gradient form, gP and 0 <= n_targets <= N");
@@ -1071,11 +1166,13 @@
   if (int rc = make_drop(drop_mode, drop_thr, seed, seed_dev, drop_edge_base, keep, E, &p.drop)) return rc;
   const int dm = (drop_mode == MMA_DROP_HASH && drop_thr == 0) ? MMA_DROP_NONE : p.drop.mode;
   const bool v4 = (H % 4 == 0) && (ldx % 4 == 0) && (ldp % 4 == 0) && (ldq % 4 == 0) && (epi || (ldgx % 4 == 0 && aligned16(gxs))) && (ldgq % 4 == 0) &&
-                  (shared ? (ldgg % 4 == 0 && aligned16(g) && ldc % 4 == 0 && aligned16(crow)) : (ldg % 4 == 0 && aligned16(gs))) &&
+                  (shared ? ((tail || (ldgg % 4 == 0 && aligned16(g))) && ldc % 4 == 0 && aligned16(crow)) : (ldg % 4 == 0 && aligned16(gs))) &&
                   (!epi || (ldt % 4 == 0 && aligned16(T) && ldgp % 4 == 0 && aligned16(gP))) &&
                   (ldgxo % 4 == 0) && aligned16(x) && aligned16(P) && aligned16(Q) &&
                   aligned16(gQ) && aligned16(gx) && (partial == nullptr || aligned16(partial));
+  MMA_REQUIRE(!tail || v4, "the tail form runs on the vector path only: H %% 4 == 0, 16-byte aligned buffers and row pitches");
   const Geometry geo = geometry(H, v4);
+  p.gt = gt; p.ldgt = ldgt; p.wt = wt;
   p.x = x; p.ldx = ldx; p.P = P; p.ldp = ldp; p.Q = Q; p.ldq = ldq; p.gs = gs; p.ldg = ldg; p.gxs = gxs; p.ldgx = ldgx;
   p.g = g; p.ldgg = ldgg; p.crow = crow; p.ldc = ldc; p.kinds = kinds;
   p.T = T; p.ldt = ldt; p.gP = gP; p.ldgp = ldgp; p.n_targets = n_targets;
@@ -1096,12 +1193,12 @@
     if (shared && small_plan(sync, K, geo, dm, n_items, n_wave_items, n_hubs, n_slots, n_hubs * (K + 1) * ((H + 3) / 4), &sp, &sgrid)) {
       p.k_base = 0; p.first_pass = 1;
       p.hubs = reinterpret_cast<const int4*>(hubs); p.n_hubs = n_hubs; p.sync = reinterpret_cast<unsigned*>(sync); p.n_slots = (unsigned)n_slots;
-      switch (K) {
-        case 1: launch_bwd_small<1>(p, sp, sgrid, dm, st); break;
-        case 2: launch_bwd_small<2>(p, sp, sgrid, dm, st); break;
-        case 3: launch_bwd_small<3>(p, sp, sgrid, dm, st); break;
-        case 4: launch_bwd_small<4>(p, sp, sgrid, dm, st); break;
-        default: launch_bwd_small<8>(p, sp, sgrid, dm, st); break;
+      switch (tq) {
+        case 0: launch_bwd_small_k<0>(K, p, sp, sgrid, dm, st); break;
+        case 1: launch_bwd_small_k<1>(K, p, sp, sgrid, dm, st); break;
+        case 2: launch_bwd_small_k<2>(K, p, sp, sgrid, dm, st); break;
+        case 3: launch_bwd_small_k<3>(K, p, sp, sgrid, dm, st); break;
+        default: launch_bwd_small_k<4>(K, p, sp, sgrid, dm, st); break;
       }
       return check_launch("nc_bwd_small_kernel");
     }
@@ -1115,7 +1212,8 @@
     for (int k0 = 0; k0 < K;) {
       const int ks = next_slice(K - k0);
       p.k_base = k0; p.first_pass = (k0 == 0);
-      if (geo.vec == 4) { if (part == 0) launch_bwd_k<4, false>(ks, p, grid, dm, st); else launch_bwd_k<4, true>(ks, p, grid, dm, st); }
+      if (tail) { if (part == 0) launch_bwd_tail<false>(tq, ks, p, grid, dm, st); else launch_bwd_tail<true>(tq, ks, p, grid, dm, st); }
+      else if (geo.vec == 4) { if (part == 0) launch_bwd_k<4, false>(ks, p, grid, dm, st); else launch_bwd_k<4, true>(ks, p, grid, dm, st); }
       else { if (part == 0) launch_bwd_k<1, false>(ks, p, grid, dm, st); else launch_bwd_k<1, true>(ks, p, grid, dm, st); }
       k0 += ks;
     }
@@ -1125,9 +1223,49 @@
     const int per_row = (H + geo.vec - 1) / geo.vec;
     const dim3 fg((unsigned)elementwise_grid(n_hubs * (K + 1) * per_row));
     const int4* hb = reinterpret_cast<const int4*>(hubs);
-    if (geo.vec == 4) hipLaunchKernelGGL((nc_bwd_finalize_kernel<4>), fg, dim3(kBlock), 0, st, p, hb, n_hubs);
+    if (tq == 1) hipLaunchKernelGGL((nc_bwd_finalize_kernel<4, 1>), fg, dim3(kBlock), 0, st, p, hb, n_hubs);
+    else if (tq == 2) hipLaunchKernelGGL((nc_bwd_finalize_kernel<4, 2>), fg, dim3(kBlock), 0, st, p, hb, n_hubs);
+    else if (tq == 3) hipLaunchKernelGGL((nc_bwd_finalize_kernel<4, 3>), fg, dim3(kBlock), 0, st, p, hb, n_hubs);
+    else if (tq == 4) hipLaunchKernelGGL((nc_bwd_finalize_kernel<4, 4>), fg, dim3(kBlock), 0, st, p, hb, n_hubs);
+    else if (geo.vec == 4) hipLaunchKernelGGL((nc_bwd_finalize_kernel<4>), fg, dim3(kBlock), 0, st, p, hb, n_hubs);
     else hipLaunchKernelGGL((nc_bwd_finalize_kernel<1>), fg, dim3(kBlock), 0, st, p, hb, n_hubs);
     if (int rc = check_launch("nc_bwd_finalize_kernel")) return rc;
   }
   return 0;
 }
+
+extern "C" int mma_nc_fused_bwd(
+    const float* x, int64_t ldx, const float* P, int64_t ldp, const float* Q, int64_t ldq,
+    const float* gs, int64_t ldg, const float* g, int64_t ldgg, const float* crow, int64_t ldc, const uint8_t* kind_host,
+    const float* gxs, int64_t ldgx, const float* T, int64_t ldt, float* gP, int64_t ldgp, int64_t n_targets,
+    const int32_t* t_col, const int32_t* t_eid,
+    const int32_t* items, int64_t n_items, int64_t n_wave_items, const int32_t* hubs, int64_t n_hubs,
+    float* partial, int64_t n_slots, float* gQ, int64_t ldgq, float* gx, int64_t ldgxo, float* row_max,
+    int64_t N, int64_t E, int32_t H, int32_t K, const uint8_t* act_host,
+    int32_t drop_mode, uint32_t drop_thr, uint64_t seed, const uint64_t* seed_dev, int64_t drop_edge_base, const uint8_t* keep,
+    int32_t* sync, void* stream) {
+  return nc_fused_bwd_impl(x, ldx, P, ldp, Q, ldq, gs, ldg, g, ldgg, crow, ldc, kind_host, gxs, ldgx, T, ldt, gP, ldgp, n_targets, t_col, t_eid,
+                           items, n_items, n_wave_items, hubs, n_hubs, partial, n_slots, gQ, ldgq, gx, ldgxo, row_max, N, E, H, K, act_host,
+                           drop_mode, drop_thr, seed, seed_dev, drop_edge_base, keep, sync, stream, nullptr, 0, nullptr, 0);
+}
+
+extern "C" int mma_tail_nc_fused_bwd(
+    const float* x, int64_t ldx, const float* P, int64_t ldp, const float* Q, int64_t ldq,
+    const float* gt, int64_t ldgt, const float* wt, int32_t C, const float* crow, int64_t ldc, const uint8_t* kind_host,
+    const float* T, int64_t ldt, float* gP, int64_t ldgp,
+    const int32_t* t_col, const int32_t* t_eid,
+    const int32_t* items, int64_t n_items, int64_t n_wave_items, const int32_t* hubs, int64_t n_hubs,
+    float* partial, int64_t n_slots, float* gQ, int64_t ldgq, float* gx, int64_t ldgxo, float* row_max,
+    int64_t N, int64_t E, int32_t H, int32_t K, const uint8_t* act_host,
+    int32_t drop_mode, uint32_t drop_thr, uint64_t seed, const uint64_t* seed_dev, int64_t drop_edge_base, const uint8_t* keep,
+    int32_t* sync, void* stream) {
+  MMA_REQUIRE(C >= 4 && C <= MMA_NC_TAIL_MAX_C && C % 4 == 0, "C=%d unsupported by the tail form (a multiple of 4, 4..%d)", C, MMA_NC_TAIL_MAX_C);
+  MMA_REQUIRE(H >= 1 && H % 4 == 0, "H=%d: the tail form runs on the vector path only (H %% 4 == 0)", H);
+  MMA_REQUIRE(ldgt >= C && ldgt % 4 == 0 && ldgt < (1LL << 31), "ldgt=%lld: the gt rows need a pitch >= C that is a multiple of 4 floats", (long long)ldgt);
+  if (N == 0 || n_items == 0) return 0;
+  MMA_REQUIRE(gt != nullptr && wt != nullptr && T != nullptr, "NULL argument: the tail form needs gt (N,C), wt (H,C) and K1's saved T");
+  MMA_REQUIRE(aligned16(gt) && aligned16(wt), "gt and wt must be 16-byte aligned");
+  return nc_fused_bwd_impl(x, ldx, P, ldp, Q, ldq, nullptr, 0, nullptr, 0, crow, ldc, kind_host, nullptr, 0, T, ldt, gP, ldgp, N, t_col, t_eid,
+                           items, n_items, n_wave_items, hubs, n_hubs, partial, n_slots, gQ, ldgq, gx, ldgxo, row_max, N, E, H, K, act_host,
+                           drop_mode, drop_thr, seed, seed_dev, drop_edge_base, keep, sync, stream, gt, ldgt, wt, C / 4);
+}
diff --git a/mma_amd/csrc/torch_ops.cpp b/mma_amd/csrc/torch_ops.cpp
--- a/mma_amd/csrc/torch_ops.cpp
+++ b/mma_amd/csrc/torch_ops.cpp
@@ -40,6 +40,12 @@
   check(mma_nc_fused_bwd(dptr<float>(x), static_cast<int64_t>(ldx), dptr<float>(P), static_cast<int64_t>(ldp), dptr<float>(Q), static_cast<int64_t>(ldq), dptr<float>(gs), static_cast<int64_t>(ldg), dptr<float>(g), static_cast<int64_t>(ldgg), dptr<float>(crow), static_cast<int64_t>(ldc), (c_kind_host.has ? c_kind_host.v.data() : nullptr), dptr<float>(gxs), static_cast<int64_t>(ldgx), dptr<float>(T), static_cast<int64_t>(ldt), dptr<float>(gP), static_cast<int64_t>(ldgp), static_cast<int64_t>(n_targets), dptr<int32_t>(t_col), dptr<int32_t>(t_eid), dptr<int32_t>(items), static_cast<int64_t>(n_items), static_cast<int64_t>(n_wave_items), dptr<int32_t>(hubs), static_cast<int64_t>(n_hubs), dptr<float>(partial), static_cast<int64_t>(n_slots), dptr<float>(gQ), static_cast<int64_t>(ldgq), dptr<float>(gx), static_cast<int64_t>(ldgxo), dptr<float>(row_max), static_cast<int64_t>(N), static_cast<int64_t>(E), static_cast<int32_t>(H), static_cast<int32_t>(K), (c_act_host.has ? c_act_host.v.data() : nullptr), static_cast<int32_t>(drop_mode), static_cast<uint32_t>(drop_thr), static_cast<uint64_t>(seed), dptr<uint64_t>(seed_dev), static_cast<int64_t>(drop_edge_base), dptr<uint8_t>(keep), dptr<int32_t>(sync), stream()), "mma_nc_fused_bwd");
 }
 
+void op_mma_tail_nc_fused_bwd(const OptT& x, int64_t ldx, const OptT& P, int64_t ldp, const OptT& Q, int64_t ldq, const OptT& gt, int64_t ldgt, const OptT& wt, int64_t C, const OptT& crow, int64_t ldc, std::optional<at::IntArrayRef> kind_host, const OptT& T, int64_t ldt, const OptT& gP, int64_t ldgp, const OptT& t_col, const OptT& t_eid, const OptT& items, int64_t n_items, int64_t n_wave_items, const OptT& hubs, int64_t n_hubs, const OptT& partial, int64_t n_slots, const OptT& gQ, int64_t ldgq, const OptT& gx, int64_t ldgxo, const OptT& row_max, int64_t N, int64_t E, int64_t H, int64_t K, std::optional<at::IntArrayRef> act_host, int64_t drop_mode, int64_t drop_thr, int64_t seed, const OptT& seed_dev, int64_t drop_edge_base, const OptT& keep, const OptT& sync) {
+  const Codes c_kind_host = codes(kind_host, static_cast<int64_t>(K), "kind_host");
+  const Codes c_act_host = codes(act_host, static_cast<int64_t>(K), "act_host");
+  check(mma_tail_nc_fused_bwd(dptr<float>(x), static_cast<int64_t>(ldx), dptr<float>(P), static_cast<int64_t>(ldp), dptr<float>(Q), static_cast<int64_t>(ldq), dptr<float>(gt), static_cast<int64_t>(ldgt), dptr<float>(wt), static_cast<int32_t>(C), dptr<float>(crow), static_cast<int64_t>(ldc), (c_kind_host.has ? c_kind_host.v.data() : nullptr), dptr<float>(T), static_cast<int64_t>(ldt), dptr<float>(gP), static_cast<int64_t>(ldgp), dptr<int32_t>(t_col), dptr<int32_t>(t_eid), dptr<int32_t>(items), static_cast<int64_t>(n_items), static_cast<int64_t>(n_wave_items), dptr<int32_t>(hubs), static_cast<int64_t>(n_hubs), dptr<float>(partial), static_cast<int64_t>(n_slots), dptr<float>(gQ), static_cast<int64_t>(ldgq), dptr<float>(gx), static_cast<int64_t>(ldgxo), dptr<float>(row_max), static_cast<int64_t>(N), static_cast<int64_t>(E), static_cast<int32_t>(H), static_cast<int32_t>(K), (c_act_host.has ? c_act_host.v.data() : nullptr), static_cast<int32_t>(drop_mode), static_cast<uint32_t>(drop_thr), static_cast<uint64_t>(seed), dptr<uint64_t>(seed_dev), static_cast<int64_t>(drop_edge_base), dptr<uint8_t>(keep), dptr<int32_t>(sync), stream()), "mma_tail_nc_fused_bwd");
+}
+
 void op_mma_csr_spmm(const OptT& rowptr, const OptT& col, const OptT& val, const OptT& B, int64_t ldb, int64_t rows_per_block, int64_t K, const OptT& bias, const OptT& out, int64_t ldo, int64_t n_rows, int64_t C) {
   check(mma_csr_spmm(dptr<int32_t>(rowptr), dptr<int32_t>(col), dptr<float>(val), dptr<float>(B), static_cast<int64_t>(ldb), static_cast<int64_t>(rows_per_block), static_cast<int32_t>(K), dptr<float>(bias), dptr<float>(out), static_cast<int64_t>(ldo), static_cast<int64_t>(n_rows), static_cast<int32_t>(C), stream()), "mma_csr_spmm");
 }
@@ -247,6 +253,7 @@
   m.def("mma_nc_fused_fwd(Tensor? x, int ldx, Tensor? P, int ldp, Tensor? Q, int ldq, Tensor? rowptr, Tensor? col, Tensor? items, int n_items, int n_wave_items, Tensor? hubs, int n_hubs, Tensor(a!)? partial, int n_slots, Tensor(b!)? m, Tensor(c!)? m_sum, int ldms, Tensor(d!)? T, Tensor(e!)? sel, int ldt, Tensor(f!)? crow, int ldc, int N, int E, int H, int K, int[]? kind_host, int[]? act_host, int drop_mode, int drop_thr, int seed, Tensor? seed_dev, int drop_edge_base, Tensor? keep, Tensor(g!)? sync) -> ()");
   m.def("mma_nc_bwd_node(Tensor? g, int g_kstride, int ldgr, Tensor? sel, Tensor? T, int ldt, Tensor? rowptr, Tensor(a!)? gs, int ldgs, Tensor? crow, int ldc, Tensor(b!)? gP, int ldgp, Tensor(c!)? gxs, int ldgx, Tensor(d!)? row_max, int N, int H, int K, int[]? kind_host) -> ()");
   m.def("mma_nc_fused_bwd(Tensor? x, int ldx, Tensor? P, int ldp, Tensor? Q, int ldq, Tensor? gs, int ldg, Tensor? g, int ldgg, Tensor? crow, int ldc, int[]? kind_host, Tensor? gxs, int ldgx, Tensor? T, int ldt, Tensor(a!)? gP, int ldgp, int n_targets, Tensor? t_col, Tensor? t_eid, Tensor? items, int n_items, int n_wave_items, Tensor? hubs, int n_hubs, Tensor(b!)? partial, int n_slots, Tensor(c!)? gQ, int ldgq, Tensor(d!)? gx, int ldgxo, Tensor(e!)? row_max, int N, int E, int H, int K, int[]? act_host, int drop_mode, int drop_thr, int seed, Tensor? seed_dev, int drop_edge_base, Tensor? keep, Tensor(f!)? sync) -> ()");
+  m.def("mma_tail_nc_fused_bwd(Tensor? x, int ldx, Tensor? P, int ldp, Tensor? Q, int ldq, Tensor? gt, int ldgt, Tensor? wt, int C, Tensor? crow, int ldc, int[]? kind_host, Tensor? T, int ldt, Tensor(a!)? gP, int ldgp, Tensor? t_col, Tensor? t_eid, Tensor? items, int n_items, int n_wave_items, Tensor? hubs, int n_hubs, Tensor(b!)? partial, int n_slots, Tensor(c!)? gQ, int ldgq, Tensor(d!)? gx, int ldgxo, Tensor(e!)? row_max, int N, int E, int H, int K, int[]? act_host, int drop_mode, int drop_thr, int seed, Tensor? seed_dev, int drop_edge_base, Tensor? keep, Tensor(f!)? sync) -> ()");
   m.def("mma_csr_spmm(Tensor? rowptr, Tensor? col, Tensor? val, Tensor? B, int ldb, int rows_per_block, int K, Tensor? bias, Tensor(a!)? out, int ldo, int n_rows, int C) -> ()");
   m.def("mma_csr_spmm_rm(Tensor? rowptr, Tensor? col, Tensor? val, Tensor? B, int ldb, int rows_per_block, int K, Tensor? bias, Tensor(a!)? out, int ldo, int n_rows, int C, Tensor(b!)? row_max) -> ()");
   m.def("mma_csr_spmm_items(Tensor? col, Tensor? val, Tensor? B, int ldb, Tensor? bias, Tensor(a!)? out, int ldo, Tensor? items, int n_items, int n_wave_items, Tensor? hubs, int n_hubs, Tensor(b!)? partial, int n_slots, int C) -> ()");
@@ -301,6 +308,7 @@
   m.impl("mma_nc_fused_fwd", &op_mma_nc_fused_fwd);
   m.impl("mma_nc_bwd_node", &op_mma_nc_bwd_node);
   m.impl("mma_nc_fused_bwd", &op_mma_nc_fused_bwd);
+  m.impl("mma_tail_nc_fused_bwd", &op_mma_tail_nc_fused_bwd);
   m.impl("mma_csr_spmm", &op_mma_csr_spmm);
   m.impl("mma_csr_spmm_rm", &op_mma_csr_spmm_rm);
   m.impl("mma_csr_spmm_items", &op_mma_csr_spmm_items);
diff --git a/mma_amd/functional.py b/mma_amd/functional.py
--- a/mma_amd/functional.py
+++ b/mma_amd/functional.py
@@ -105,12 +105,32 @@
     return gs, gP, gxs
 
 
-def nc_bwd_edges_launch(x_src, P, Q, gs, g, crow, gxs, graph, kinds, acts, drop, gQ, gx, partial, part=None, row_max=None, T=None, gP=None):
+TAIL_MAX_C = 16
+
+
+def tail_form_ok(H, K, C, graph):
+    return H % 4 == 0 and C % 4 == 0 and 4 <= C <= TAIL_MAX_C and 1 <= K <= 8 and graph.n_src == graph.N
+
+
+def nc_bwd_edges_launch(x_src, P, Q, gs, g, crow, gxs, graph, kinds, acts, drop, gQ, gx, partial, part=None, row_max=None, T=None, gP=None,
+                        *, gt=None, wt=None):
     K = len(acts)
     S, H = x_src.shape
     items, n_wave, hubs = part if part is not None else (graph.t_items, graph.t_n_wave_items, graph.t_hubs)
     shared = gs is None
     mode, thr, seed, seed_dev, keep = drop.args()
+    if gt is not None:
+        assert g is None and gs is None and T is not None and gP is not None and wt is not None and part is None
+        C = gt.shape[1]
+        assert tail_form_ok(H, K, C, graph) and gt.shape[0] == graph.N and gt.stride(1) == 1 and wt.shape == (H, C) and wt.is_contiguous()
+        with _span("nc_fused_bwd"):
+            call("mma_tail_nc_fused_bwd", ptr(x_src), x_src.stride(0), ptr(P), P.stride(0), ptr(Q), Q.stride(0),
+                 ptr(gt), gt.stride(0), ptr(wt), C, ptr(crow), crow.stride(0), host_codes(kinds),
+                 ptr(T), K * H, ptr(gP), gP.stride(0), ptr(graph.t_col), ptr(graph.t_eid), ptr(items), items.shape[0], n_wave,
+                 ptr(hubs) if hubs.shape[0] else None, hubs.shape[0], ptr(partial), graph.t_n_slots if hubs.shape[0] else 0,
+                 ptr(gQ), gQ.stride(0), ptr(gx), H, ptr(row_max), S, graph.E, H, K, host_codes(acts), mode, thr, seed, seed_dev,
+                 graph.edge_base, keep, ptr(graph.sync(1)), stream_ptr())
+        return
     with _span("nc_fused_bwd"):
         call("mma_nc_fused_bwd", ptr(x_src), x_src.stride(0), ptr(P), P.stride(0), ptr(Q), Q.stride(0),
              ptr(gs), K * H, ptr(g) if shared else None, g.stride(0) if shared else 0,
@@ -159,54 +179,99 @@
         return gx, gP, gQ, None, None, None, None, None
 
 
+def _local_layer_fwd(ctx, x, wtop, wbot, graph, kinds, acts, drop, need):
+    from .dense import mm_into
+    require_gpu(x)
+    x = x.contiguous()
+    N, H = x.shape
+    K = len(kinds)
+    KH = K * H
+    PQ = torch.empty((N, 2 * KH), device=x.device, dtype=torch.float32)
+    ctx.cat_given = wbot is None
+    wcat = wtop if ctx.cat_given else torch.cat([wtop, wbot], 1)
+    box = [] if need else None
+    mm_into(x, wcat, PQ, row_max_box=box)
+    msum, T, sel, crow = nc_fwd_launch(x, PQ[:, :KH], PQ[:, KH:], graph, kinds, acts, drop, True, need)
+    ctx.graph, ctx.kinds, ctx.acts, ctx.drop = graph, kinds, acts, drop
+    return msum, (x, PQ, T, sel, crow, wcat, box[0] if box else None)
+
+
+def _local_layer_bwd(ctx, saved, need_w, row_max, g=None, gt=None, wt=None):
+    from .dense import rows_mm_add_, xt_g
+    graph, kinds, acts, drop = ctx.graph, ctx.kinds, ctx.acts, ctx.drop
+    x, PQ, T, sel, crow, wcat, x_row_max = saved
+    N, H = x.shape
+    K = len(kinds)
+    KH = K * H
+    dev = x.device
+    gPQ = torch.empty((N, 2 * KH), device=dev, dtype=torch.float32)
+    gx = torch.empty((N, H), device=dev, dtype=torch.float32)
+    partial = (torch.empty((graph.t_n_slots, (K + 1) * H), device=dev, dtype=torch.float32)
+               if graph.t_n_slots else None)
+    shared = crow is not None
+    if gt is not None:
+        nc_bwd_edges_launch(x, PQ[:, :KH], PQ[:, KH:], None, None, crow, None, graph, kinds, acts, drop, gPQ[:, KH:], gx, partial,
+                            row_max=row_max, T=T, gP=gPQ[:, :KH], gt=gt, wt=wt)
+    elif shared and FUSE_NODE_BWD:
+        nc_bwd_edges_launch(x, PQ[:, :KH], PQ[:, KH:], None, g, crow, None, graph, kinds, acts, drop, gPQ[:, KH:], gx, partial,
+                            row_max=row_max, T=T, gP=gPQ[:, :KH])
+    else:
+        gs, gP, gxs = nc_bwd_node_launch(g, True, sel, crow, T, graph, kinds, H, shared, gP=gPQ[:, :KH], row_max=row_max)
+        nc_bwd_edges_launch(x, PQ[:, :KH], PQ[:, KH:], gs, g, crow, gxs, graph, kinds, acts, drop, gPQ[:, KH:], gx, partial,
+                            row_max=row_max)
+    rows_mm_add_(gx, gPQ, wcat.t(), row_max)
+    gw = xt_g(x, gPQ, x_row_max, row_max) if need_w else None
+    if ctx.cat_given:
+        return gx, gw, None
+    return gx, (gw[:, :KH] if gw is not None else None), (gw[:, KH:] if gw is not None else None)
+
+
 class _NCLocalLayer(torch.autograd.Function):
 
     @staticmethod
     def forward(ctx, x, wtop, wbot, graph, kinds, acts, drop):
-        from .dense import mm_into
-        require_gpu(x)
-        x = x.contiguous()
-        N, H = x.shape
-        K = len(kinds)
-        KH = K * H
-        PQ = torch.empty((N, 2 * KH), device=x.device, dtype=torch.float32)
-        ctx.cat_given = wbot is None
-        wcat = wtop if ctx.cat_given else torch.cat([wtop, wbot], 1)
+        msum, saved = _local_layer_fwd(ctx, x, wtop, wbot, graph, kinds, acts, drop, any(ctx.needs_input_grad[:3]))
+        ctx.save_for_backward(*saved)
+        return msum
+
+    @staticmethod
+    def backward(ctx, g):
+        from .dense import f16x2_n128_ok
+        need_w = ctx.needs_input_grad[1] or ctx.needs_input_grad[2]
+        (N, H), K = ctx.saved_tensors[0].shape, len(ctx.kinds)
+        row_max = torch.zeros((N,), device=g.device, dtype=torch.float32) if f16x2_n128_ok(N, 2 * K * H, H) and K <= 8 else None
+        return _local_layer_bwd(ctx, ctx.saved_tensors, need_w, row_max, g=g.contiguous()) + (None, None, None, None)
+
+
+class _NCLocalLayerTail(torch.autograd.Function):
+
+    @staticmethod
+    def forward(ctx, x, wtop, wbot, w_tail, graph, kinds, acts, drop):
+        from .dense import _nn
         need = any(ctx.needs_input_grad[:3])
-        box = [] if need else None
-        mm_into(x, wcat, PQ, row_max_box=box)
-        msum, T, sel, crow = nc_fwd_launch(x, PQ[:, :KH], PQ[:, KH:], graph, kinds, acts, drop, True, need)
-        ctx.graph, ctx.kinds, ctx.acts, ctx.drop = graph, kinds, acts, drop
-        ctx.save_for_backward(x, PQ, T, sel, crow, wcat, box[0] if box else None)
-        return msum
-
-    @staticmethod
-    def backward(ctx, g):
-        from .dense import f16x2_n128_ok, rows_mm_add_, xt_g
-        graph, kinds, acts, drop = ctx.graph, ctx.kinds, ctx.acts, ctx.drop
-        x, PQ, T, sel, crow, wcat, x_row_max = ctx.saved_tensors
-        N, H = x.shape
-        K = len(kinds)
-        KH = K * H
-        g = g.contiguous()
-        gPQ = torch.empty((N, 2 * KH), device=g.device, dtype=torch.float32)
-        row_max = torch.zeros((N,), device=g.device, dtype=torch.float32) if f16x2_n128_ok(N, 2 * KH, H) and K <= 8 else None
-        gx = torch.empty((N, H), device=g.device, dtype=torch.float32)
-        partial = (torch.empty((graph.t_n_slots, (K + 1) * H), device=g.device, dtype=torch.float32)
-                   if graph.t_n_slots else None)
-        shared = crow is not None
-        if shared and FUSE_NODE_BWD:
-            nc_bwd_edges_launch(x, PQ[:, :KH], PQ[:, KH:], None, g, crow, None, graph, kinds, acts, drop, gPQ[:, KH:], gx, partial,
-                                row_max=row_max, T=T, gP=gPQ[:, :KH])
-        else:
-            gs, gP, gxs = nc_bwd_node_launch(g, True, sel, crow, T, graph, kinds, H, shared, gP=gPQ[:, :KH], row_max=row_max)
-            nc_bwd_edges_launch(x, PQ[:, :KH], PQ[:, KH:], gs, g, crow, gxs, graph, kinds, acts, drop, gPQ[:, KH:], gx, partial,
-                                row_max=row_max)
-        rows_mm_add_(gx, gPQ, wcat.t(), row_max)
-        gw = xt_g(x, gPQ, x_row_max, row_max) if (ctx.needs_input_grad[1] or ctx.needs_input_grad[2]) else None
-        if ctx.cat_given:
-            return gx, gw, None, None, None, None, None
-        return gx, (gw[:, :KH] if gw is not None else None), (gw[:, KH:] if gw is not None else None), None, None, None, None
+        msum, saved = _local_layer_fwd(ctx, x, wtop, wbot, graph, kinds, acts, drop, need)
+        require_gpu(w_tail)
+        ctx.save_for_backward(*saved, msum, w_tail)
+        return _nn(msum, w_tail)
+
+    @staticmethod
+    def backward(ctx, gt):
+        from .dense import f16x2_n128_ok, xt_g
+        *saved, msum, w_tail = ctx.saved_tensors
+        gt = gt.contiguous()
+        gw_tail = xt_g(msum, gt) if ctx.needs_input_grad[3] else None
+        gx = gwt = gwb = None
+        if any(ctx.needs_input_grad[:3]):
+            need_w = ctx.needs_input_grad[1] or ctx.needs_input_grad[2]
+            (N, H), K = msum.shape, len(ctx.kinds)
+            row_max = torch.zeros((N,), device=gt.device, dtype=torch.float32) if f16x2_n128_ok(N, 2 * K * H, H) and K <= 8 else None
+            gx, gwt, gwb = _local_layer_bwd(ctx, saved, need_w, row_max, gt=gt, wt=w_tail.contiguous())
+        return gx, gwt, gwb, gw_tail, None, None, None, None
+
+
+def nc_local_layer_tail(x, wtop, wbot, w_tail, graph, kinds, acts, drop=None):
+    assert tail_form_ok(x.shape[1], len(kinds), w_tail.shape[1], graph) and FUSE_NODE_BWD and SHARED_GRAD_BWD
+    return _NCLocalLayerTail.apply(x, wtop, wbot, w_tail, graph, tuple(kinds), tuple(acts), drop or DropoutSpec(0.0))
 
 
 def nc_local_layer(x, wtop, wbot, graph, kinds, acts, drop=None):
diff --git a/mma_amd/layers.py b/mma_amd/layers.py
--- a/mma_amd/layers.py
+++ b/mma_amd/layers.py
@@ -171,12 +171,14 @@
             return Fn.DropoutSpec(self.dropout, seed_tensor=self._seeds.advance())
         return Fn.DropoutSpec(self.dropout)
 
-    def _aggregate(self, names, input, drop=None, reduce_k=False):
+    def _aggregate(self, names, input, drop=None, reduce_k=False, tail=None):
         require_gpu(input)
         H = input.shape[1]
         kinds, acts = self._codes(names)
         masks = [getattr(self, "mask_" + n) for n in names]
         graph = self.graph(input.device)
+        if reduce_k and tail is not None:
+            return Fn.nc_local_layer_tail(input, Fn.mask_weights(masks), None, tail, graph, kinds, acts, drop or self._drop(names, input.device))
         if reduce_k:
             return Fn.nc_local_layer(input, Fn.mask_weights(masks), None, graph, kinds, acts, drop or self._drop(names, input.device))
         wtop, wbot = torch.cat([w[:H] for w in masks], 1), torch.cat([w[H:] for w in masks], 1)
@@ -202,13 +204,17 @@
 
     def forward(self, input, adj):
         N = input.shape[0]
-        msum = self._aggregate_all(self.aggregator_names, input, reduce_k=True)
+        names = self.aggregator_names
+        tail = (Fn.FUSE_NODE_BWD and Fn.SHARED_GRAD_BWD and len(names) <= 8 and self.weight.dim() == 2 and
+                Fn.tail_form_ok(input.shape[1], len(names), self.weight.shape[1], self.graph(input.device)))
+        support = (self._aggregate(names, input, reduce_k=True, tail=self.weight) if tail
+                   else mm(self._aggregate_all(names, input, reduce_k=True), self.weight))
         if self._sg is None or self._sg[0] is not adj:
             self._sg = (adj, adj if isinstance(adj, SpmmGraph) else SpmmGraph.from_torch_sparse(adj, input.device))
         factor = self._scaler_factor(N, input.device)
         if self._sg_scaled is None or self._sg_scaled[0] is not self._sg[1] or self._sg_scaled[1] is not factor:
             self._sg_scaled = (self._sg[1], factor, self._sg[1].scaled_by_source(factor))
-        return Fn.csr_spmm(mm(msum, self.weight), self.bias, self._sg_scaled[2], 1)
+        return Fn.csr_spmm(support, self.bias, self._sg_scaled[2], 1)
 
     def __repr__(self):
         return self.__class__.__name__ + ' (' + str(self.in_features) + ' -> ' + str(self.out_features) + ')'
```

Measured after the change: 735.7 million. 2.2% lower.
